# CMB-BNU/PloidyFrost

Measured on AMD Instinct MI355X. Metric: unitigs/s through superbubble+SeqAlign (k=25, z=8), higher is better.
Workload: dtype u64

## Files before the change

### include/ploidyfrost_hip.h

```cpp
#ifndef PLOIDYFROST_HIP_H_
#define PLOIDYFROST_HIP_H_

#include <stddef.h>
#include <stdint.h>

#ifdef __cplusplus
extern "C" {
#endif

#define PF_NONE 0xFFFFFFFFu

enum pf_status {
    PF_OK = 0,
    PF_ERR_ARG = 1,
    PF_ERR_HIP = 2,
    PF_ERR_NO_DEVICE = 3,
    PF_ERR_OVERFLOW = 4,
    PF_ERR_MISSING_KMER = 5
};

typedef struct pf_ctx pf_ctx;

int pf_create(int device, pf_ctx **out);
int pf_warmup(int device);
// ... 271 lines not shown
    uint32_t n_cols;
    uint32_t n_sites;
    uint32_t n_indel_len;
} pf_bubble_result;

int pf_align_bubbles(pf_ctx *, const char *text, uint64_t text_len, const pf_bubble_path *paths, uint64_t n_paths,
                     const pf_bubble_task *tasks, uint32_t n_tasks, double match, double mismatch, double gap,
                     pf_bubble_result *results, char *out_text, uint64_t text_cap, pf_bubble_site *out_sites,
                     uint64_t site_cap, uint8_t *out_groups, uint64_t group_cap, uint32_t *out_ilen, uint64_t ilen_cap,
                     uint64_t used[4]);

int pf_string_cov(pf_ctx *, const char *text, const uint64_t *str_off, uint32_t n_str, uint32_t low, uint32_t up,
                  uint64_t *sum, uint8_t *ok, uint8_t *miss);


int pf_call_set_colours(pf_ctx *, uint32_t n_colors, const uint64_t *full_mask, const uint64_t *size_total, const uint32_t *part_first,
                        const uint32_t *part_colour, const uint64_t *part_word, const uint64_t *part_bits, uint64_t n_part, uint64_t n_words);
int pf_call_set_cutoffs(pf_ctx *, uint32_t n_colors, const uint32_t *lower, const uint32_t *upper);

int pf_call_set_state(pf_ctx *, const uint8_t *flags, const uint32_t *plus, const uint32_t *minus);
int pf_call_set_format(pf_ctx *, int reference_mt);
int pf_superbubble_rows(pf_ctx *, int colored_rule, uint64_t *n_rows, uint64_t *text_len);
int pf_superbubble_fetch(pf_ctx *, char *dst, uint64_t len);
int pf_call_coverage(pf_ctx *);

typedef struct pf_call_side {
    uint32_t u;
    uint32_t exit_ov;
    uint32_t err_unitig;
    uint8_t plus_side;
    uint8_t kind;
    uint8_t aligned;
    uint8_t err;
} pf_call_side;
int pf_call_scan(pf_ctx *, uint32_t lower, uint32_t upper, uint64_t *n_sides);
int pf_call_sides(pf_ctx *, pf_call_side *out, uint64_t cap);
int pf_call_resolve(pf_ctx *, uint64_t *n_bubbles, uint32_t *err, uint32_t *err_unitig);
int pf_call_select(pf_ctx *, const uint32_t *side_index, uint64_t n_bubbles);

#define PF_CALL_STREAMS 10
enum pf_call_stream {
    PF_OUT_ALLELE_FREQUENCY = 0, PF_OUT_ALIGNSEQ = 1, PF_OUT_BIFRE = 2, PF_OUT_TRIFRE = 3, PF_OUT_TETRAFRE = 4, PF_OUT_PENTAFRE = 5,
    PF_OUT_BICOV = 6, PF_OUT_TRICOV = 7, PF_OUT_TETRACOV = 8, PF_OUT_PENTACOV = 9
};
typedef struct pf_call_result {
    uint64_t text_len[PF_CALL_STREAMS];
    uint64_t allele[4];
    uint64_t core_cov, core_num;
    uint64_t n_called;
    uint64_t align_jobs, site_strings, n_branching;
    uint64_t snp_jobs, pair_jobs, wave_jobs;
    uint64_t stack_jobs;
    uint64_t alignseq_packed_len;
    uint64_t numeric_packed;
} pf_call_result;
#define PF_CALL_SLABS 4
#define PF_CALL_LANES 4
int pf_call_run(pf_ctx *, int slab, uint64_t t0, uint64_t t1, uint64_t var_count_base, uint32_t complex_size, double match,
                double mismatch, double gap, pf_call_result *out);
int pf_call_align(pf_ctx *, uint64_t t0, uint64_t t1, uint32_t complex_size, double match, double mismatch, double gap,
                  pf_call_result *out);
int pf_call_text(pf_ctx *, int slab, uint64_t var_count_base, pf_call_result *out);
int pf_call_set_alignseq_packed(pf_ctx *, int on);
#define PF_NUMERIC_PACKED_LEN(text_len) (((((uint64_t)(text_len)) + 1) / 2 + 15) & ~15ull)
int pf_call_set_numeric_packed(pf_ctx *, int on);
int pf_call_fetch_text(pf_ctx *, int slab, int stream, char *dst, uint64_t len);
int pf_call_reserve(pf_ctx *, uint64_t n_bubbles, uint32_t complex_size);
int pf_call_reserve_lanes(pf_ctx *, uint64_t n_bubbles, uint32_t complex_size, int n_lanes);
int pf_call_reserve_text(pf_ctx *, uint64_t piece_bubbles);
typedef struct pf_call_bubble {
    uint32_t entrance_ov, exit_ov;
    uint32_t strict, n_inner;
    uint32_t inner[4];
    double cov[4], core_mean, cov_sum;
} pf_call_bubble;
int pf_call_peek(pf_ctx *, int lane, pf_call_bubble *bubbles, pf_bubble_result *results, uint64_t *sv_off, uint64_t bubble_cap, char *text,
                 pf_bubble_site *sites, uint8_t *groups, uint32_t *ilen, double *sv, const uint64_t cap[5], uint64_t used[6]);
int pf_call_text_range(pf_ctx *, int slab, uint64_t first, uint64_t count, uint64_t var_count_base, pf_call_result *out);
int pf_call_align_lane(pf_ctx *, int lane, uint64_t t0, uint64_t t1, uint32_t complex_size, double match, double mismatch,
                       double gap, pf_call_result *out);
int pf_call_text_range_lane(pf_ctx *, int lane, int slab, uint64_t first, uint64_t count, uint64_t var_count_base,
                            pf_call_result *out);
int pf_call_text_sizes(pf_ctx *, int lane, uint64_t first, uint64_t count, uint64_t var_count_base, pf_call_result *out);
int pf_call_fetch(pf_ctx *, int slab, int stream, char *dst, uint64_t len);
int pf_call_fetch_slab(pf_ctx *, int slab, char *dst, const uint64_t *len);
int pf_call_fetch_range(pf_ctx *, int slab, uint64_t first_byte, char *dst, uint64_t len, int slot);
int pf_call_fetch_wait(pf_ctx *, int slot);
int pf_format_doubles(pf_ctx *, const double *values, uint64_t n, char *text, uint8_t *len);

int pf_side_components(pf_ctx *, int reset, const pf_bfs_record *records, uint64_t n_records, const uint32_t *pool, uint64_t pool_len,
                       const pf_bfs_record *extra, uint64_t n_extra, const uint32_t *extra_pool, uint64_t extra_pool_len);
int pf_replay_order(pf_ctx *, uint32_t n_classes, uint32_t *order, uint32_t *class_off, uint32_t *labels);

int pf_bfs_live_deferred(pf_ctx *, uint64_t cap, volatile uint64_t **list);
int pf_bfs_live_count(pf_ctx *, uint64_t *n);
int pf_bfs_candidates_resident(pf_ctx *, uint32_t u0, uint32_t u1, uint64_t *n_records, uint64_t *pool_used, uint32_t *deferred,
                               uint32_t *deferred_entrance, uint64_t deferred_cap, uint64_t *n_deferred);
int pf_find_reserve(pf_ctx *, uint64_t n_records);
int pf_replay_device(pf_ctx *, uint32_t complex_size, uint32_t small_limit, uint64_t *n_big, uint64_t *big_entries);
int pf_replay_set_colours(pf_ctx *, uint32_t n_colors, const uint64_t *full_mask, const uint64_t *size_total, const uint32_t *n_full_enc);
int pf_replay_big_fetch(pf_ctx *, uint32_t *index, pf_bfs_record *records, uint32_t *pool);
int pf_replay_finish(pf_ctx *, const uint32_t *sides, const uint32_t *links, const uint8_t *side_flags, uint64_t n_patch);
int pf_call_get_state(pf_ctx *, uint8_t *flags, uint32_t *plus, uint32_t *minus);

#define PF_MAX_COLORS_TABLE 1024
#define PF_MAX_COLORS PF_MAX_COLORS_TABLE
int pf_upload_counts_colored(pf_ctx *, uint32_t n_colors, const uint64_t *const *kmers, const uint32_t *const *counts,
                             const uint64_t *n, const uint64_t *min_count, const uint64_t *max_count, const int *both_strands);
uint32_t pf_num_colors(const pf_ctx *);
int pf_unitig_cov_colored(pf_ctx *, uint32_t u0, uint32_t u1, uint64_t *sum, uint32_t *min_count, uint32_t *max_count,
                          uint8_t *miss);
int pf_unitig_cov_colored_probe(pf_ctx *, uint32_t u0, uint32_t u1, uint64_t *sum, uint32_t *min_count, uint32_t *max_count,
                          uint8_t *miss);
int pf_string_cov_colored(pf_ctx *, const char *text, const uint64_t *str_off, uint32_t n_str, const uint32_t *low,
                          const uint32_t *up, uint64_t *sum, uint8_t *ok);

#define PF_COMM_ID_BYTES 128
int pf_comm_unique_id(unsigned char id[PF_COMM_ID_BYTES]);
int pf_comm_init(pf_ctx *, const unsigned char id[PF_COMM_ID_BYTES], int rank, int world);
int pf_gather(pf_ctx *, const uint64_t *mine, uint32_t n, uint64_t *all);
void pf_comm_destroy(pf_ctx *);

#define PF_GMM_MAX_GAUSS 16
int pf_gmm_upload(pf_ctx *, const double *values, uint64_t n);
uint64_t pf_gmm_count(const pf_ctx *);
int pf_gmm_fit(pf_ctx *, uint32_t gauss, double m_thre, double n_thre, int32_t max_iter, double max_delta, double *weights,
               double *means, double *vars, double *loglik, uint32_t *iterations);
int pf_gmm_values(pf_ctx *, double *dst, uint64_t cap);
#define PF_DENSITY_MIN_POINTS 2
#define PF_DENSITY_MAX_POINTS 4096
typedef struct pf_density_info {
    uint64_t n;
    double min, max, sd, q1, q3, bw;
    double order[4];
} pf_density_info;
int pf_gmm_density(pf_ctx *, uint32_t points, double adjust, double *x, double *density, pf_density_info *info);

enum pf_model_source { PF_MODEL_COV = 0, PF_MODEL_FRE = 1 };
int pf_call_model_begin(pf_ctx *, int source, double q);
int pf_call_model_take(pf_ctx *, int slab);
int pf_call_model_finish(pf_ctx *, uint64_t *n_values);
typedef struct pf_filter_opts {
    int simple, indel, snp;
    long long low, up;
    long long num, distance, size;
    double frequency;
} pf_filter_opts;
int pf_call_model_filter(pf_ctx *, const pf_filter_opts *);
int pf_call_model_take_text(pf_ctx *, int stream_ord, const char *host_text, uint64_t len);
typedef struct pf_filter_multi_opts {
    int simple, indel, snp;
    long long low, up;
    long long num, distance, size;
    double frequency;
    long long color;
    double cramer;
} pf_filter_multi_opts;
#define PF_MODEL_NO_ROW 0xFFFFFFFFFFFFFFFFull
int pf_call_model_filter_multi(pf_ctx *, const pf_filter_multi_opts *, int each_color);
uint32_t pf_call_model_color_count(const pf_ctx *);
int pf_call_model_color_select(pf_ctx *, int color, uint64_t *n_values);
uint64_t pf_call_fetched_bytes(const pf_ctx *);

int pf_host_alloc(pf_ctx *, size_t bytes, void **out);
int pf_fetch(pf_ctx *, void *dst_host, const void *src_dev, uint64_t bytes);
void pf_host_free(pf_ctx *, void *p);
// ... 13 lines not shown
```

### ploidyfrost_amd/csrc/host/pf_cdbg_call.cpp

```cpp
#include <fcntl.h>
#include <sys/stat.h>
#include <unistd.h>

#include <algorithm>
#include <atomic>
#include <condition_variable>
#include <cstdio>
#include <cstring>
#include <ctime>
#include <deque>
#include <memory>
#include <mutex>
#include <sstream>
#include <thread>

#include "../pf_alnpack.hpp"
#include "../pf_nibble.hpp"
#include "pf_cdbg_impl.hpp"
#include "pf_parallel.hpp"

namespace pfh {

namespace {
const char *kStreamSuffix[PF_CALL_STREAMS] = {"_allele_frequency.txt", "_alignseq.txt", "_bifre.txt",    "_trifre.txt",   "_tetrafre.txt",
// ... 202 lines not shown
    model_n_ = 0;
    color_fits_.clear();
    color_none_.clear();
    color_empty_.clear();
    color_no_density_.clear();
    density_done_ = false;
    pooled_values_.clear();
    last_each_ = false;
    const uint64_t fetched_before = pf_call_fetched_bytes(ctx_);
    const unsigned T = threads_ ? threads_ : (unsigned)std::max<size_t>(thr, 1);
    times_.cov_device_s = times_.tasks_s = times_.align_s = times_.sites_s = times_.format_s = times_.write_s = 0;
    times_.tasks = times_.align_jobs = times_.site_strings = 0;
    times_.snp_jobs = times_.pair_jobs = times_.wave_jobs = times_.stack_jobs = 0;
    times_.align_build_s = times_.align_device_s = times_.align_post_s = times_.align_choose_s = times_.scan_s = 0;
    allele_[0] = allele_[1] = allele_[2] = allele_[3] = 0;
    core_cov_ = core_num_ = 0;
    const bool trace = getenv("PF_TRACE_PLOIDY") != nullptr;
    auto tp = [&](const char *what) { if (trace) fprintf(stderr, "[ploidy] %-28s %.2f ms\n", what, since(t_all) * 1e3); };

    struct OutFile {
        std::string name;
        uint64_t bytes = 0;
        int rc = 0;
    };
    std::vector<OutFile> files(PF_CALL_STREAMS);
    for (int s = 0; s < PF_CALL_STREAMS; ++s) files[(size_t)s].name = outpre + kStreamSuffix[s];
    MappedOut *maps = out_maps_.get();
    int open_failed = -1;
    std::thread opener;
    if (write_ten)
        opener = std::thread([&] {
            for (size_t i = 0; i < files.size(); ++i)
                if (maps[i].open_for(outdir_ + "/" + files[i].name)) { open_failed = (int)i; return; }
        });
    struct OpenerGuard {
        std::thread &t;
        ~OpenerGuard() { if (t.joinable()) t.join(); }
    } opener_guard{opener};

    uint64_t n_tasks = 0;
    if (call_select(cutoff, n_tasks)) return status_;
    tp("scan + selection done");
    if (opener.joinable()) opener.join();
    if (open_failed >= 0) return fail(PF_ERR_ARG, "CDBG:: Open " + files[(size_t)open_failed].name + " file error");
    last_allfre_.clear();
    last_allfre_file_.clear();
    std::thread prefault0;
    std::atomic<bool> prefault0_stop{false};
    struct Prefault0Guard {
        std::thread &t;
        std::atomic<bool> &stop;
        ~Prefault0Guard() { stop.store(true); if (t.joinable()) t.join(); }
    } prefault0_guard{prefault0, prefault0_stop};
    if (write_ten && n_tasks) {
        const double nbub = 1.1 * (double)n_tasks;
        const double per_bubble[PF_CALL_STREAMS] = {20, 2.0 * (2 * g_.k + 26), 20, 0.5, 0.25, 0, 34, 0.75, 0.25, 0};
        std::vector<std::pair<int, uint64_t>> fresh;
        for (int s = 0; s < PF_CALL_STREAMS; ++s) {
            const uint64_t est = (uint64_t)(per_bubble[s] * nbub);
            if (est >= (1u << 20) && maps[s].reserve(est) == 0) fresh.push_back({s, est});
        }
        if (!fresh.empty())
            prefault0 = std::thread([maps, fresh, T, &prefault0_stop] {
                constexpr uint64_t STEP = 4u << 20;
                std::vector<std::pair<int, uint64_t>> spans;
                uint64_t longest = 0;
                for (auto &f : fresh) longest = std::max(longest, f.second);
                for (uint64_t at = 0; at < longest; at += STEP)
                    for (auto &f : fresh)
                        if (at < f.second) spans.push_back({f.first, at});
                parallel_chunks(spans.size(), 1, std::max(2u, T), [&](size_t i, size_t, size_t) {
                    if (prefault0_stop.load(std::memory_order_relaxed)) return;
                    const int s = spans[i].first;
                    uint64_t end = spans[i].second + STEP;
                    for (auto &f : fresh) if (f.first == s) end = std::min(end, f.second);
                    maps[s].populate(spans[i].second, end);
                });
            });
    }

    const bool aln_packed = !getenv("PF_ALIGNSEQ_ASCII");
    if (pf_call_set_alignseq_packed(ctx_, aln_packed ? 1 : 0) != PF_OK) return fail(PF_ERR_HIP, std::string(tag_) + "::PloidyEstimation(): " + pf_last_error(ctx_));
    const bool num_packed = !getenv("PF_NUMERIC_ASCII");
    if (pf_call_set_numeric_packed(ctx_, num_packed ? 1 : 0) != PF_OK) return fail(PF_ERR_HIP, std::string(tag_) + "::PloidyEstimation(): " + pf_last_error(ctx_));
    if (model_.on && (pf_call_model_begin(ctx_, model_.source, model_.q) != PF_OK || (filter_on_ && pf_call_model_filter(ctx_, &filter_) != PF_OK) ||
                      (multi_on_ && pf_call_model_filter_multi(ctx_, &multi_, multi_each_ ? 1 : 0) != PF_OK)))
        return fail(PF_ERR_ARG, std::string(tag_) + "::PloidyEstimation(): " + pf_last_error(ctx_));
    struct PackGuard {
        pf_ctx *c;
        ~PackGuard() { (void)pf_call_set_alignseq_packed(c, 0); (void)pf_call_set_numeric_packed(c, 0); }
    } pack_guard{ctx_};
    auto slab_len = [](const pf_call_result &r, int s) -> uint64_t {
        const uint64_t aln = (s == PF_OUT_ALIGNSEQ && r.alignseq_packed_len) ? r.alignseq_packed_len : r.text_len[s];
        if (!r.numeric_packed) return aln;
        return s == PF_OUT_ALIGNSEQ ? ((aln + 15) & ~15ull) : PF_NUMERIC_PACKED_LEN(r.text_len[s]);
    };

    const size_t batch_env = [] { const char *e = getenv("PF_BATCH_BUBBLES"); return e ? (size_t)std::max(1, atoi(e)) : (size_t)0; }();
    const size_t batch_now = batch_env ? batch_env : batch_bubbles_;
    const size_t CHUNK = std::min<size_t>(std::max<size_t>(batch_now ? batch_now * 4 : 1, 1), (size_t)1 << 24);
    struct Done {
        pf_call_result res;
        int slab;
        int hslab;
        std::shared_ptr<std::vector<std::vector<char>>> plain;
    };
    std::mutex mu;
    std::condition_variable cv;
    std::deque<Done> ready, towrite;
    size_t fetched = 0;
    size_t written = 0;
    bool fetcher_done = false;
    bool stop = false, producer_done = false;
    int wst = PF_OK;
    std::string werr;
    double write_s = 0;
    auto thread_failed = [&](const char *who, const std::exception &e) {
        {
            std::lock_guard<std::mutex> lk(mu);
            wst = PF_ERR_HIP;
            werr = std::string(who) + ": " + e.what();
            stop = true;
            fetcher_done = true;
        }
        cv.notify_all();
    };
    std::thread fetcher([&] {
        try {
        size_t b = 0;
        for (;;) {
            Done d;
            {
                std::unique_lock<std::mutex> lk(mu);
                cv.wait(lk, [&] { return stop || !ready.empty() || producer_done; });
                if (stop || ready.empty()) { fetcher_done = true; lk.unlock(); cv.notify_all(); return; }
                d = ready.front();
                ready.pop_front();
                cv.wait(lk, [&] { return stop || b < written + 2; });
                if (stop) { fetcher_done = true; lk.unlock(); cv.notify_all(); return; }
            }
            uint64_t total = 0, fetch_len[PF_CALL_STREAMS];
            for (int s = 0; s < PF_CALL_STREAMS; ++s) { fetch_len[s] = slab_len(d.res, s); total += fetch_len[s]; }
            PinnedBuf<char> &hb = cx_.slab[d.hslab];
            hb.ensure(ctx_, std::max<uint64_t>(total, 1) + 16);
            int st = pf_call_fetch_slab(ctx_, d.slab, hb.p, fetch_len);
            if (st == PF_OK && d.res.numeric_packed) {
                uint32_t flagged = 0;
                memcpy(&flagged, hb.p + total, 4);
                if (flagged) {
                    d.plain = std::make_shared<std::vector<std::vector<char>>>((size_t)PF_CALL_STREAMS);
                    for (int s = 0; s < PF_CALL_STREAMS && st == PF_OK; ++s)
                        if (((flagged >> s) & 1) && d.res.text_len[s]) {
                            (*d.plain)[(size_t)s].resize(d.res.text_len[s]);
                            st = pf_call_fetch_text(ctx_, d.slab, s, (*d.plain)[(size_t)s].data(), d.res.text_len[s]);
                        }
                }
            }
            {
                std::lock_guard<std::mutex> lk(mu);
                fetched = b + 1;
                if (st != PF_OK) { wst = st; werr = "copy of a text slab failed"; stop = true; fetcher_done = true; }
                else towrite.push_back(d);
            }
            cv.notify_all();
            if (st != PF_OK) return;
            if (trace) fprintf(stderr, "[ploidy]   batch %zu fetched (%.1f MB) %.2f ms\n", b, total / 1e6, since(t_all) * 1e3);
            ++b;
        }
        } catch (const std::exception &e) { thread_failed("copy of a text slab", e); }
    });
    std::thread writer([&] {
        try {
        size_t b = 0;
        for (;;) {
            Done d;
            {
                std::unique_lock<std::mutex> lk(mu);
                cv.wait(lk, [&] { return stop || !towrite.empty() || fetcher_done; });
                if (stop || towrite.empty()) return;
                d = towrite.front();
                towrite.pop_front();
            }
            const auto tw = clk::now();
            uint64_t total = 0, off[PF_CALL_STREAMS + 1];
            for (int s = 0; s < PF_CALL_STREAMS; ++s) { off[s] = total; total += slab_len(d.res, s); }
            PinnedBuf<char> &hb = cx_.slab[d.hslab];
            if (write_ten) {
                CopySpan spans[PF_CALL_STREAMS];
                bool nib_span[PF_CALL_STREAMS] = {};
                size_t n_spans = 0;
                pf::AlnPackPiece packed;
                char *packed_dst = nullptr;
                std::vector<char> packed_tmp;
                for (int s = 0; s < PF_CALL_STREAMS; ++s) {
                    if (!d.res.text_len[s]) continue;
                    char *dst = maps[s].prepare(files[(size_t)s].bytes, d.res.text_len[s]);
                    if (s == PF_OUT_ALIGNSEQ && d.res.alignseq_packed_len) {
                        if (!packed.parse(reinterpret_cast<const uint8_t *>(hb.p + off[s]), d.res.alignseq_packed_len)) { files[(size_t)s].rc = 1; continue; }
                        if (!dst) { packed_tmp.resize(d.res.text_len[s]); dst = packed_tmp.data(); }
                        packed_dst = dst;
                        continue;
                    }
                    const char *src = hb.p + off[s];
                    bool nib = d.res.numeric_packed != 0 && s != PF_OUT_ALIGNSEQ;
                    if (nib && d.plain && !(*d.plain)[(size_t)s].empty()) { src = (*d.plain)[(size_t)s].data(); nib = false; }
                    if (dst) {
                        nib_span[n_spans] = nib;
                        spans[n_spans++] = CopySpan{dst, src, d.res.text_len[s]};
                    } else if (nib) {
                        std::vector<char> tmp(d.res.text_len[s]);
                        pf::nibble_expand(tmp.data(), reinterpret_cast<const uint8_t *>(src), d.res.text_len[s]);
                        if (maps[s].write(files[(size_t)s].bytes, tmp.data(), tmp.size(), T)) files[(size_t)s].rc = 1;
                    } else if (maps[s].write(files[(size_t)s].bytes, src, d.res.text_len[s], T)) files[(size_t)s].rc = 1;
                }
                constexpr uint64_t PIECE = 1u << 20;
                std::vector<CopySpan> cut;
                std::vector<char> cut_nib;
                constexpr uint64_t NIB_PIECE = 128u << 10;
                for (size_t i = 0; i < n_spans; ++i) {
                    const uint64_t step = nib_span[i] ? NIB_PIECE : PIECE;
                    for (uint64_t at = 0; at < spans[i].len; at += step) {
                        cut.push_back(CopySpan{spans[i].dst + at, spans[i].src + (nib_span[i] ? at / 2 : at), std::min<uint64_t>(step, spans[i].len - at)});
                        cut_nib.push_back(nib_span[i] ? 1 : 0);
                    }
                }
                constexpr uint64_t GROUPS_PER_TASK = 16;
                const size_t n_aln = packed_dst ? (size_t)((packed.n_groups + GROUPS_PER_TASK - 1) / GROUPS_PER_TASK) : 0;
                std::atomic<int> bad{0};
                parallel_chunks(n_aln + cut.size(), 1, T, [&](size_t i, size_t, size_t) {
                    if (i >= n_aln) {
                        const CopySpan &c = cut[i - n_aln];
                        if (cut_nib[i - n_aln]) pf::nibble_expand(c.dst, reinterpret_cast<const uint8_t *>(c.src), c.len);
                        else memcpy(c.dst, c.src, (size_t)c.len);
                        return;
                    }
                    const uint64_t g0 = (uint64_t)i * GROUPS_PER_TASK, g1 = std::min<uint64_t>(packed.n_groups, g0 + GROUPS_PER_TASK);
                    uint64_t t0_, r0_, t1_, r1_;
                    packed.entry(g0, t0_, r0_);
                    packed.entry(g1, t1_, r1_);
                    if (t1_ > d.res.text_len[PF_OUT_ALIGNSEQ] || t0_ > t1_ || r0_ > r1_ ||
                        (uint64_t)(packed.records - packed.base) + r1_ > d.res.alignseq_packed_len) { bad = 1; return; }
                    char *end = pf::alnpack_expand(packed.records + r0_, packed.records + r1_, packed_dst + t0_, packed_dst + t1_);
                    if (end != packed_dst + t1_) bad = 1;
                });
                if (bad) files[PF_OUT_ALIGNSEQ].rc = 1;
                if (!packed_tmp.empty() && maps[PF_OUT_ALIGNSEQ].write(files[PF_OUT_ALIGNSEQ].bytes, packed_tmp.data(), packed_tmp.size(), T)) files[PF_OUT_ALIGNSEQ].rc = 1;
            }
            if (!write_files_) {
                if (d.plain && !(*d.plain)[0].empty()) last_allfre_.append((*d.plain)[0].data(), d.res.text_len[0]);
                else if (d.res.numeric_packed) {
                    const size_t at0 = last_allfre_.size();
                    last_allfre_.resize(at0 + d.res.text_len[0]);
                    pf::nibble_expand(&last_allfre_[at0], reinterpret_cast<const uint8_t *>(hb.p + off[0]), d.res.text_len[0]);
                } else last_allfre_.append(hb.p + off[0], d.res.text_len[0]);
            }
            for (int s = 0; s < PF_CALL_STREAMS; ++s) files[(size_t)s].bytes += d.res.text_len[s];
            write_s += since(tw);
            if (trace) fprintf(stderr, "[ploidy]   batch %zu written %.2f ms\n", b, since(t_all) * 1e3);
            ++b;
            { std::lock_guard<std::mutex> lk(mu); written = b; }
            cv.notify_all();
        }
        } catch (const std::exception &e) { thread_failed("writing the result files", e); }
    });
    struct WriterGuard {
        std::thread &t, &t2;
        std::mutex &mu;
        std::condition_variable &cv;
        bool &stop;
        ~WriterGuard() {
            if (!t.joinable() && !t2.joinable()) return;
            { std::lock_guard<std::mutex> lk(mu); stop = true; }
            cv.notify_all();
            if (t.joinable()) t.join();
            if (t2.joinable()) t2.join();
        }
    } writer_guard{fetcher, writer, mu, cv, stop};

    int rc = PF_OK;
    std::string rc_err;
    std::thread prefault;
    struct PrefaultGuard {
        std::thread &t;
        ~PrefaultGuard() { if (t.joinable()) t.join(); }
    } prefault_guard{prefault};
    const auto t_dev = clk::now();
    uint64_t ALIGN = std::min<uint64_t>((uint64_t)CHUNK * std::max<size_t>(align_pieces_, 1), (uint64_t)1 << 24);
    {
        const int ranges_env = [] { const char *e = getenv("PF_ALIGN_RANGES"); return e ? atoi(e) : 0; }();
        const uint64_t pieces = (n_tasks + CHUNK - 1) / CHUNK;
        const uint64_t n_ranges = ranges_env > 0 ? (uint64_t)ranges_env : (pieces >= 4 ? 2 : 1);
        if (n_ranges > 1) ALIGN = std::min<uint64_t>(ALIGN, std::max<uint64_t>(1, (pieces + n_ranges - 1) / n_ranges) * CHUNK);
    }
    int first_env = 0;
    constexpr int LANES = PF_CALL_LANES;
    const int aligners_wanted = [&] { const char *e = getenv("PF_ALIGN_THREADS"); return e ? std::max(1, std::min(LANES, atoi(e))) : std::min(2, LANES); }();
    {
        const uint64_t pieces = (n_tasks + CHUNK - 1) / CHUNK;
        if (first_env <= 0 && !getenv("PF_ALIGN_RANGES") && pieces >= 4)
            first_env = (int)std::min<uint64_t>(aligners_wanted >= 2 ? (pieces + 1) / 2 : (pieces * 5 + 7) / 8, ((uint64_t)1 << 24) / CHUNK);
    }
    struct Range {
        uint64_t a0 = 0, a1 = 0;
        int lane = 0;
        bool aligned = false;
        uint64_t n_called = 0;
    };
    std::vector<Range> ranges;
    for (uint64_t a0 = 0, a1 = 0; a0 < n_tasks; a0 = a1) {
        a1 = std::min<uint64_t>(n_tasks, a0 + (first_env > 0 && ranges.empty() ? (uint64_t)first_env * CHUNK : ALIGN));
        Range r;
        r.a0 = a0; r.a1 = a1; r.lane = (int)(ranges.size() % (size_t)LANES);
        ranges.push_back(r);
    }
    const int aligners = (int)std::min<size_t>(ranges.size(), (size_t)aligners_wanted);
    size_t next_range = 0;
    size_t ranges_formatted = 0;
    std::thread formatter([&] {
        struct Last {
            std::mutex &mu;
            std::condition_variable &cv;
            bool &producer_done;
            ~Last() {
                { std::lock_guard<std::mutex> lk(mu); producer_done = true; }
                cv.notify_all();
            }
        } last{mu, cv, producer_done};
        try {
        size_t b = 0;
        uint64_t var_base = 0;
        for (size_t ri = 0; ri < ranges.size(); ++ri) {
            Range r;
            {
                std::unique_lock<std::mutex> lk(mu);
                cv.wait(lk, [&] { return stop || ranges[ri].aligned; });
                if (stop) return;
                r = ranges[ri];
            }
            const uint64_t rn = r.a1 - r.a0;
            for (uint64_t p0 = 0; p0 < rn; p0 += CHUNK, ++b) {
                const uint64_t count = std::min<uint64_t>(CHUNK, rn - p0);
                {
                    std::unique_lock<std::mutex> lk(mu);
                    cv.wait(lk, [&] { return stop || model_.only || b < fetched + PF_CALL_SLABS; });
                    if (stop) return;
                }
                Done d;
                d.slab = (int)(b % PF_CALL_SLABS);
                d.hslab = (int)(b & 1);
                int st = pf_call_text_range_lane(ctx_, r.lane, d.slab, p0, count, var_base, &d.res);
                if (st == PF_OK && model_.on) st = pf_call_model_take(ctx_, d.slab);
                if (st != PF_OK) {
                    { std::lock_guard<std::mutex> lk(mu); if (rc == PF_OK) { rc = st; rc_err = pf_last_error(ctx_); } stop = true; }
                    cv.notify_all();
                    return;
                }
                if (trace) fprintf(stderr, "[ploidy]   piece %zu formatted on the device %.2f ms\n", b, since(t_all) * 1e3);
                if (b == 0 && write_ten) {
                    const double scale = 1.05 * (double)n_tasks / (double)std::max<uint64_t>(1, count);
                    std::vector<std::pair<int, uint64_t>> fresh;
                    for (int s = 0; s < PF_CALL_STREAMS; ++s) {
                        const uint64_t est = (uint64_t)((double)d.res.text_len[s] * scale) + 4096;
                        if (d.res.text_len[s] && maps[s].reserve(est) == 0) fresh.push_back({s, est});
                    }
                    if (!fresh.empty())
                        prefault = std::thread([maps, fresh, T] {
                            constexpr uint64_t STEP = 4u << 20;
                            std::vector<std::pair<int, uint64_t>> spans;
                            uint64_t longest = 0;
                            for (auto &f : fresh) longest = std::max(longest, f.second);
                            for (uint64_t at = 0; at < longest; at += STEP)
                                for (auto &f : fresh)
                                    if (at < f.second) spans.push_back({f.first, at});
                            parallel_chunks(spans.size(), 1, std::max(2u, T / 2), [&](size_t i, size_t, size_t) {
                                const int s = spans[i].first;
                                uint64_t end = spans[i].second + STEP;
                                for (auto &f : fresh) if (f.first == s) end = std::min(end, f.second);
                                maps[s].populate(spans[i].second, end);
                            });
                        });
                }
                for (int a = 0; a < 4; ++a) allele_[a] += d.res.allele[a];
                core_cov_ += d.res.core_cov;
                core_num_ += d.res.core_num;
                if (!model_.only) {
                    { std::lock_guard<std::mutex> lk(mu); ready.push_back(d); }
                    cv.notify_all();
                }
            }
            var_base += r.n_called;
            { std::lock_guard<std::mutex> lk(mu); ++ranges_formatted; }
            cv.notify_all();
        }
        } catch (const std::exception &e) { thread_failed("formatting the result rows", e); }
    });
    struct FormatterGuard {
        std::thread &t;
        std::mutex &mu;
        std::condition_variable &cv;
        bool &stop;
        ~FormatterGuard() {
            if (!t.joinable()) return;
            { std::lock_guard<std::mutex> lk(mu); stop = true; }
            cv.notify_all();
            t.join();
        }
    } formatter_guard{formatter, mu, cv, stop};
    auto aligner = [&] {
        try {
        for (;;) {
            size_t ri;
            {
                std::unique_lock<std::mutex> lk(mu);
                if (stop || next_range >= ranges.size()) return;
                ri = next_range++;
                cv.wait(lk, [&] { return stop || ri < ranges_formatted + (size_t)LANES; });
                if (stop) return;
            }
            const Range r = ranges[ri];
            pf_call_result ar;
            const int st = pf_call_align_lane(ctx_, r.lane, r.a0, r.a1, (uint32_t)std::min<size_t>(complex_size_, 1u << 20), sc_.match, sc_.mismatch, sc_.gap, &ar);
            if (st != PF_OK) {
                { std::lock_guard<std::mutex> lk(mu); if (rc == PF_OK) { rc = st; rc_err = pf_last_error(ctx_); } stop = true; }
                cv.notify_all();
                return;
            }
            if (trace) fprintf(stderr, "[ploidy]   range %zu: %llu bubbles aligned on the device %.2f ms\n", ri, (unsigned long long)(r.a1 - r.a0), since(t_all) * 1e3);
            {
                std::lock_guard<std::mutex> lk(mu);
                times_.tasks += r.a1 - r.a0;
                times_.align_jobs += ar.align_jobs;
                times_.snp_jobs += ar.snp_jobs; times_.pair_jobs += ar.pair_jobs; times_.wave_jobs += ar.wave_jobs; times_.stack_jobs += ar.stack_jobs;
                times_.site_strings += ar.site_strings;
                ranges[ri].n_called = ar.n_called;
                ranges[ri].aligned = true;
            }
            cv.notify_all();
        }
        } catch (const std::exception &e) { thread_failed("aligning the bubbles", e); }
    };
    {
        std::vector<std::thread> extra;
        struct ExtraGuard {
            std::vector<std::thread> &v;
            ~ExtraGuard() { for (auto &t : v) if (t.joinable()) t.join(); }
        } extra_guard{extra};
        for (int a = 1; a < aligners; ++a) extra.emplace_back(aligner);
        aligner();
    }
    formatter.join();
    times_.align_s = since(t_dev);
    fetcher.join();
    writer.join();
    if (prefault.joinable()) prefault.join();
    prefault0_stop.store(true);
    if (prefault0.joinable()) prefault0.join();
    tp("pipeline done");
    if (rc != PF_OK) {
        return fail(rc, rc_err.rfind("CDBG::", 0) == 0 ? rc_err : std::string(tag_) + "::PloidyEstimation(): " + rc_err);
    }
    if (wst != PF_OK) return fail(wst, std::string(tag_) + "::PloidyEstimation(): " + werr);
    auto t0 = clk::now();
    if (join_pending_write() || join_pending_ids()) return status_;
    tp("super_bubble.txt joined");
    for (size_t i = 0; i < files.size(); ++i) {
        OutFile &of = files[i];
        out_bytes_ += of.bytes;
// ... 104 lines not shown
```

### ploidyfrost_amd/csrc/pf_alnpack.hpp

```cpp
#pragma once
#include <cstdint>
#include <cstring>

#ifdef __HIPCC__
#define PF_ALNPACK_HD __host__ __device__
#else
#define PF_ALNPACK_HD
#endif

namespace pf {

constexpr uint32_t ALNPACK_GROUP = 256;
constexpr uint32_t ALNPACK_HEADER = 24;

PF_ALNPACK_HD inline uint32_t alnpack_row_bytes(uint32_t n_cols) { return 3u * ((n_cols + 7u) >> 3); }
PF_ALNPACK_HD inline uint64_t alnpack_index_bytes(uint64_t n_bubbles) { return 16 + ((n_bubbles + ALNPACK_GROUP - 1) / ALNPACK_GROUP + 1) * 16; }
PF_ALNPACK_HD inline uint32_t alnpack_code(char c) { return c == '-' ? 0u : c == 'A' ? 1u : c == 'C' ? 2u : c == 'G' ? 3u : 4u; }

#ifndef __HIP_DEVICE_COMPILE__
struct AlnPackTables {
    uint32_t four[4096];
    AlnPackTables() {
        static const char letter[8] = {'-', 'A', 'C', 'G', 'T', '?', '?', '?'};
        for (uint32_t v = 0; v < 4096; ++v)
            four[v] = (uint32_t)(uint8_t)letter[v & 7] | (uint32_t)(uint8_t)letter[(v >> 3) & 7] << 8 | (uint32_t)(uint8_t)letter[(v >> 6) & 7] << 16 |
                      (uint32_t)(uint8_t)letter[(v >> 9) & 7] << 24;
    }
};
inline const AlnPackTables &alnpack_tables() {
    static const AlnPackTables t;
    return t;
}

inline char *alnpack_put_uint(char *p, uint64_t x) {
    char tmp[24];
    int n = 0;
    do { tmp[n++] = (char)('0' + x % 10); x /= 10; } while (x);
    while (n) *p++ = tmp[--n];
    return p;
}

struct AlnPackPiece {
    const uint8_t *base = nullptr;
    uint64_t n_groups = 0, group_bubbles = 0;
    const uint8_t *index = nullptr, *records = nullptr;
    bool parse(const uint8_t *p, uint64_t len) {
        if (len < 32) return false;
        memcpy(&n_groups, p, 8);
        memcpy(&group_bubbles, p + 8, 8);
        if (n_groups > (len - 16) / 16 - 1) return false;
        base = p;
        index = p + 16;
        records = index + (n_groups + 1) * 16;
        return true;
    }
    void entry(uint64_t g, uint64_t &text_off, uint64_t &rec_off) const {
        memcpy(&text_off, index + g * 16, 8);
        memcpy(&rec_off, index + g * 16 + 8, 8);
    }
};

inline char *alnpack_expand(const uint8_t *rec, const uint8_t *rec_end, char *dst, const char *dst_end) {
    const AlnPackTables &T = alnpack_tables();
    char prefix[96];
    while (rec < rec_end) {
        if ((size_t)(rec_end - rec) < ALNPACK_HEADER) return nullptr;
        uint64_t vc;
        uint32_t ent, ext, L, R;
        memcpy(&vc, rec, 8);
        memcpy(&ent, rec + 8, 4);
        memcpy(&ext, rec + 12, 4);
        memcpy(&L, rec + 16, 4);
        memcpy(&R, rec + 20, 4);
        const bool strict = (R >> 31) != 0;
        R &= 0x7FFFFFFFu;
        rec += ALNPACK_HEADER;
        char *q = alnpack_put_uint(prefix, vc);
        *q++ = '\t'; *q++ = strict ? '1' : '0'; *q++ = '\t';
        q = alnpack_put_uint(q, ent);
        *q++ = '\t';
        q = alnpack_put_uint(q, ext);
        *q++ = '\t';
        const size_t np = (size_t)(q - prefix);
        const uint32_t rb = alnpack_row_bytes(L);
        if ((uint64_t)R * rb > (uint64_t)(rec_end - rec) || (uint64_t)R * (np + L + 1) > (uint64_t)(dst_end - dst)) return nullptr;
        for (uint32_t r = 0; r < R; ++r, rec += rb) {
            memcpy(dst, prefix, np);
            dst += np;
            uint32_t x = 0;
            const uint8_t *s = rec;
            for (; x + 8 <= L; x += 8, s += 3) {
                const uint32_t v = (uint32_t)s[0] | (uint32_t)s[1] << 8 | (uint32_t)s[2] << 16;
                const uint32_t a = T.four[v & 4095], b = T.four[v >> 12];
                memcpy(dst + x, &a, 4);
                memcpy(dst + x + 4, &b, 4);
            }
            if (x < L) {
                const uint32_t v = (uint32_t)s[0] | (uint32_t)s[1] << 8 | (uint32_t)s[2] << 16;
                char tail[8];
                const uint32_t a = T.four[v & 4095], b = T.four[v >> 12];
                memcpy(tail, &a, 4);
                memcpy(tail + 4, &b, 4);
                memcpy(dst + x, tail, L - x);
            }
            dst += L;
            *dst++ = '\n';
        }
    }
    return dst;
}
#endif

}
```

### ploidyfrost_amd/csrc/pf_call.hip

```cpp
#include "pf_call_kernels.hpp"
#include "pf_scan.hpp"

using namespace pf;

#define PF_HIP(call)                                                                         \
    do {                                                                                     \
        hipError_t e_ = (call);                                                              \
        if (e_ != hipSuccess) {                                                              \
            pf::CtxErr{ctx} = std::string(#call) + ": " + hipGetErrorString(e_);                   \
            return PF_ERR_HIP;                                                               \
        }                                                                                    \
    } while (0)

#define PF_TRY(call) do { const int s_ = (call); if (s_ != PF_OK) return s_; } while (0)

using namespace pf_call;

struct Need { DevBuf *buf; size_t bytes; };
static int need(pf_ctx *ctx, const char *who, std::initializer_list<Need> list) {
    for (const Need &n : list)
        if (!n.buf->ensure(n.bytes)) { pf::CtxErr{ctx} = std::string(who) + ": out of device memory"; return PF_ERR_HIP; }
    return PF_OK;
}

namespace pf {

void call_state_create(pf_ctx *ctx) { (void)state_of(ctx); }
void call_destroy(pf_ctx *ctx) {
    if (!ctx->call) return;
    ctx->call->release_all();
    delete ctx->call;
    ctx->call = nullptr;
}
void call_invalidate(pf_ctx *ctx) {
    if (!ctx->call) return;
    ctx->call->have_cov = false;
    ctx->call->have_state = false;
    ctx->call->n_sides = ctx->call->n_tasks = 0;
}

}

namespace pf {
int call_state_arrays(pf_ctx *ctx, uint8_t **flags, uint32_t **plus, uint32_t **minus) {
    if (!ctx->d_seq || !ctx->has_adj) { pf::CtxErr{ctx} = "T1 state: graph and adjacency first"; return PF_ERR_ARG; }
    CallState *S = state_of(ctx);
    const size_t N = ctx->N;
    if (!S->flags.ensure(N + 1) || !S->plus.ensure(N * 4) || !S->minus.ensure(N * 4)) { pf::CtxErr{ctx} = "T1 state: out of device memory"; return PF_ERR_HIP; }
    *flags = S->flags.as<uint8_t>();
    *plus = S->plus.as<uint32_t>();
    *minus = S->minus.as<uint32_t>();
    S->have_state = false;
    return PF_OK;
}
void call_state_resident(pf_ctx *ctx) {
    CallState *S = state_of(ctx);
    S->have_state = true;
    S->n_sides = S->n_tasks = 0;
}
}

extern "C" {

int pf_format_doubles(pf_ctx *ctx, const double *values, uint64_t n, char *text, uint8_t *len) {
    if (!ctx || (n && (!values || !text || !len))) return PF_ERR_ARG;
    if (n == 0) return PF_OK;
    PF_HIP(hipSetDevice(ctx->device));
    DevTmp<double> dx;
    DevTmp<char> dt;
    DevTmp<uint8_t> dl;
    PF_HIP(dx.alloc(n * 8));
    PF_HIP(dt.alloc(n * 32));
    PF_HIP(dl.alloc(n));
    PF_HIP(hipMemcpyAsync(dx.p, values, n * 8, hipMemcpyDefault, ctx->stream));
    k_format_doubles<<<(unsigned)((n + 255) / 256), 256, 0, ctx->stream>>>(dx.p, n, dt.p, dl.p);
    PF_HIP(hipGetLastError());
    PF_HIP(hipMemcpyAsync(text, dt.p, n * 32, hipMemcpyDefault, ctx->stream));
    PF_HIP(hipMemcpyAsync(len, dl.p, n, hipMemcpyDefault, ctx->stream));
    PF_HIP(hipStreamSynchronize(ctx->stream));
    return PF_OK;
}

// ... 632 lines not shown
        PF_HIP(scan_inclusive_u32(W.has.as<uint32_t>(), O.vc.as<uint32_t>(), nb, W.scan_tmp.p, st));
        PF_HIP(hipMemcpyAsync(&n_called, O.vc.as<uint32_t>() + (nb - 1), 4, hipMemcpyDeviceToHost, st));
        return PF_OK;
    }

    SiteArgs site_args(uint32_t ks, uint64_t rows_cap, uint64_t per_wave, uint64_t sv_cap) const {
        SiteArgs sa;
        sa.batch = batch; sa.blist = lists.blist; sa.res = pools.res; sa.otext = pools.otext; sa.osites = pools.osites; sa.ogroups = pools.ogroups;
        sa.k = ctx->k; sa.tab = ctx->d_tab; sa.mask = ctx->tab_cap - 1; sa.one_strand = ctx->tab_one_strand; sa.tab_exact = ctx->tab_exact;
        sa.low = S->low; sa.up = S->up; sa.ks = ks; sa.rows_cap = (uint32_t)rows_cap;
        sa.scratch = W.sites_scr.as<uint8_t>(); sa.scratch_per_wave = per_wave; sa.sv_off = O.sv_off.as<uint64_t>();
        sa.sv = O.sv.as<double>(); sa.sv_cap = sv_cap; sa.cnt = d_cnt; sa.prof = nullptr;
        sa.n_colors = S->n_colors;
        sa.ctab = CTab{ctx->d_ctab, ctx->ctab_cap - 1, ctx->ctab_line_bytes}; sa.c_one_strand = ctx->ctab_one_strand; sa.unread = ctx->d_unread;
        sa.clow = S->col_low.as<uint32_t>(); sa.cup = S->col_up.as<uint32_t>(); sa.full = S->col_full.as<uint64_t>(); sa.cwords = S->col_words;
        sa.part_first = S->part_first.as<uint32_t>(); sa.part_colour = S->part_colour.as<uint32_t>(); sa.part_word = S->part_word.as<uint64_t>();
        sa.part_bits = S->part_bits.as<uint64_t>(); sa.walk_pool = W.walk_pool.as<uint32_t>(); sa.walk_off = W.walk_off.as<uint64_t>();
        sa.graph = graph;
        return sa;
    }

    int launch_sites(SiteArgs &sa, int grid) {
        static const bool sites_stats = getenv("PF_SITES_STATS") != nullptr;
        DevTmp<unsigned long long> prof;
        if (sites_stats) PF_TRY(stats_begin(ctx, prof, (size_t)grid * 6, st, &sa.prof));
        PF_HIP(hipMemsetAsync(&d_cnt->sites_next, 0, 4, st));
        PF_HIP(hipMemsetAsync(&d_cnt->sv_head, 0, 8, st));
        PF_HIP(hipMemsetAsync(&d_cnt->site_strings, 0, 8, st));
        tbegin(PF_K_CALL_SITES, st);
        if (sa.n_colors) k_call_sites<true><<<grid, 64, 0, st>>>(sa);
        else k_call_sites<false><<<grid, 64, 0, st>>>(sa);
        tend(st);
        ctx_units(ctx, PF_K_CALL_SITES, hc.n_branching);
        if (sites_stats) { PF_HIP(hipGetLastError()); PF_TRY(print_sites_stats(ctx, prof, grid, st)); }
        return read_counters();
    }

    int run_sites() {
        uint32_t KS = std::max<uint32_t>(first_site_string(ctx->k), S->sites_ks.load());
        const uint32_t C = S->n_colors;
        const uint64_t rows_cap = sites_rows_cap(hc.max_rows);
        for (int sv_attempt = 0, ks_attempt = 0;;) {
            const uint64_t per_wave = sites_per_wave(rows_cap, KS, C, S->col_words);
            const int grid = call_sites_grid(hc.n_branching, grids, per_wave);
            const uint64_t sv_cap = site_values_cap(C, hc.n_branching, grid, S->sv_pool);
            PF_TRY(need(ctx, who, {{&W.sites_scr, per_wave * grid}, {&O.sv, sv_cap * 8}}));
            SiteArgs sa = site_args(KS, rows_cap, per_wave, sv_cap);
            PF_TRY(launch_sites(sa, grid));
            if (hc.err & ERR_SITE_LONG) {
                if (++ks_attempt > 3 || hc.ks_need <= KS) { pf::CtxErr{ctx} = "pf_call_run: the room for a site string does not converge"; return PF_ERR_OVERFLOW; }
                KS = grown_site_string(hc.ks_need);
                amax(S->sites_ks, KS);
                hc.err = 0; hc.ks_need = 0;
                PF_HIP(hipMemsetAsync(&d_cnt->err, 0, 4, st));
                PF_HIP(hipMemsetAsync(&d_cnt->ks_need, 0, 4, st));
                continue;
            }
            if (hc.err & ERR_MISSING_KMER) { pf::CtxErr{ctx} = "CDBG::readCov(): a kmer of a site string can not found ."; return PF_ERR_MISSING_KMER; }
            if (hc.err & ERR_SITE_ROW) { pf::CtxErr{ctx} = "CDBG::PloidyEstimation(): a site string runs past the end of an aligned row (the reference terminates here: std::out_of_range from substr, src/CDBG.cpp:1478-1590)"; return PF_ERR_ARG; }
            if (hc.err & ERR_SITE_UNITIG) { pf::CtxErr{ctx} = "CCDBG::PloidyEstimation(): a site string does not start on a unitig of its bubble"; return PF_ERR_ARG; }
            if (hc.sv_head > sv_cap) {
                if (sv_attempt++ >= 2) { pf::CtxErr{ctx} = "pf_call_run: site value pool does not converge"; return PF_ERR_OVERFLOW; }
                amax(S->sv_pool, grown(hc.sv_head, 1024));
                continue;
            }
            amax(S->sv_pool, sv_cap);
            return PF_OK;
        }
    }
};

}

extern "C" {

int pf_call_align_lane(pf_ctx *ctx, int lane, uint64_t t0, uint64_t t1, uint32_t complex_size, double match, double mismatch, double gap,
                       pf_call_result *out) {
    if (!ctx || !out || lane < 0 || lane >= PF_CALL_LANES) return PF_ERR_ARG;
    CallState *S = ctx->call;
    if (!S || t0 > t1 || t1 > S->n_tasks) { pf::CtxErr{ctx} = "pf_call_align: range outside the selection"; return PF_ERR_ARG; }
    memset(out, 0, sizeof(*out));
    CallState::AlignOut &O = S->lane[lane];
    O.nb = 0;
    O.t0 = t0;
    O.cur = pf_call_result{};
    if (t1 == t0) return PF_OK;
    if (t1 - t0 > (1u << 24)) { pf::CtxErr{ctx} = "pf_call_align: at most 2^24 bubbles per batch"; return PF_ERR_ARG; }
    PF_HIP(hipSetDevice(ctx->device));
    AlignCall A(ctx, lane, t0, (uint32_t)(t1 - t0), complex_size, match, mismatch, gap);
    PF_TRY(A.prepare());
    for (A.attempt = 0;; ++A.attempt) {
        if (A.attempt > 5) { pf::CtxErr{ctx} = "pf_call_align: pools do not converge"; return PF_ERR_OVERFLOW; }
        bool retry = false;
        PF_TRY(A.size_pools());
        PF_TRY(A.launch_tiers());
        PF_TRY(A.read_counters());
        A.trace.stage("K-PREP .. K-STACK done");
        PF_TRY(A.launch_pair_tier2());
        A.note_units();
        PF_TRY(A.launch_paths_big(&retry));
        if (!retry) PF_TRY(A.accept_walks(&retry));
        if (!retry) PF_TRY(A.run_bubble(&retry));
        if (!retry) break;
    }
    const CallCounters &hc = A.hc;
    out->n_branching = hc.n_branching;
    out->align_jobs = A.n_jobs + hc.n_snp_done + hc.n_pair_done + hc.n_pair2_done + hc.n_stack_done;
    out->snp_jobs = hc.n_snp_done; out->pair_jobs = hc.n_pair_done + hc.n_pair2_done; out->wave_jobs = A.n_jobs; out->stack_jobs = hc.n_stack_done;
    PF_TRY(A.number_called());
    if (hc.n_branching) {
        PF_TRY(A.run_sites());
    } else {
        PF_TRY(need(ctx, A.who, {{&O.sv, 16}}));
        PF_HIP(hipStreamSynchronize(A.st));
    }
    out->site_strings = hc.site_strings;
    A.trace.stage("K-SITES done");
    out->n_called = A.n_called;
    O.nb = A.nb;
    O.cur = *out;
    for (int x = 0; x < 4; ++x) O.used[x] = A.heads[x];
    O.used[4] = hc.n_branching ? hc.sv_head : 0;
    return PF_OK;
}

int pf_call_peek(pf_ctx *ctx, int lane, pf_call_bubble *bubbles, pf_bubble_result *results, uint64_t *sv_off, uint64_t bubble_cap, char *text,
                 pf_bubble_site *sites, uint8_t *groups, uint32_t *ilen, double *sv, const uint64_t cap[5], uint64_t used[6]) {
    if (!ctx || lane < 0 || lane >= PF_CALL_LANES || !used) return PF_ERR_ARG;
    CallState *S = ctx->call;
    if (!S) { pf::CtxErr{ctx} = "pf_call_peek: pf_call_align first"; return PF_ERR_ARG; }
    if (S->n_colors) { pf::CtxErr{ctx} = "pf_call_peek: the single-sample path's view (a colored site holds one value per colour and group)"; return PF_ERR_ARG; }
    const CallState::AlignOut &O = S->lane[lane];
    used[0] = O.nb;
    for (int x = 0; x < 5; ++x) used[x + 1] = O.used[x];
    if (!O.nb) return PF_OK;
    if (!bubbles && !results && !text && !sites && !groups && !ilen && !sv && !sv_off) return PF_OK;
    if (bubble_cap < O.nb || !cap) return PF_ERR_ARG;
    for (int x = 0; x < 5; ++x)
        if (cap[x] < O.used[x]) return PF_ERR_ARG;
    PF_HIP(hipSetDevice(ctx->device));
    if (bubbles) {
        std::vector<uint32_t> kept(O.nb);
        PF_HIP(hipMemcpy(kept.data(), S->kept.as<uint32_t>() + O.t0, (size_t)O.nb * 4, hipMemcpyDeviceToHost));
        std::vector<CallTask> ct(S->n_sides);
        if (S->n_sides) PF_HIP(hipMemcpy(ct.data(), S->ctask.p, (size_t)S->n_sides * sizeof(CallTask), hipMemcpyDeviceToHost));
        for (uint32_t j = 0; j < O.nb; ++j) {
            const CallTask &t = ct[kept[j]];
            pf_call_bubble &b = bubbles[j];
            b.entrance_ov = t.entrance_ov; b.exit_ov = t.exit_ov; b.strict = t.strict; b.n_inner = t.n_inner;
            for (int x = 0; x < 4; ++x) { b.inner[x] = t.inner[x]; b.cov[x] = t.cov[x]; }
            b.core_mean = t.core_mean; b.cov_sum = t.cov_sum;
        }
    }
    if (results) PF_HIP(hipMemcpy(results, O.res.p, (size_t)O.nb * sizeof(pf_bubble_result), hipMemcpyDeviceToHost));
    if (sv_off) PF_HIP(hipMemcpy(sv_off, O.sv_off.p, (size_t)O.nb * 8, hipMemcpyDeviceToHost));
    if (text && O.used[0]) PF_HIP(hipMemcpy(text, O.otext.p, O.used[0], hipMemcpyDeviceToHost));
    if (sites && O.used[1]) PF_HIP(hipMemcpy(sites, O.osites.p, O.used[1] * sizeof(pf_bubble_site), hipMemcpyDeviceToHost));
    if (groups && O.used[2]) PF_HIP(hipMemcpy(groups, O.ogroups.p, O.used[2], hipMemcpyDeviceToHost));
    if (ilen && O.used[3]) PF_HIP(hipMemcpy(ilen, O.oilen.p, O.used[3] * 4, hipMemcpyDeviceToHost));
    if (sv && O.used[4]) PF_HIP(hipMemcpy(sv, O.sv.p, O.used[4] * 8, hipMemcpyDeviceToHost));
    return PF_OK;
}

int pf_call_reserve_lanes(pf_ctx *ctx, uint64_t nb64, uint32_t complex_size, int n_lanes) {
    if (!ctx || nb64 == 0 || n_lanes < 1 || n_lanes > PF_CALL_LANES) return PF_ERR_ARG;
    CallState *S = state_of(ctx);
    PF_HIP(hipSetDevice(ctx->device));
    const uint32_t nb = (uint32_t)std::min<uint64_t>(nb64, 1u << 24);
    const char *who = "pf_call_reserve";
    const CallGrids grids = call_grids(ctx->n_cu);
    DevLoadTrace trace;
    for (int lane = 0; lane < n_lanes; ++lane) {
        CallState::AlignWork &W = S->work[lane];
        CallState::AlignOut &O = S->lane[lane];
        PF_TRY(ensure_batch_buffers(ctx, who, W, O, nb));
        PF_TRY(ensure_wave_scratch(ctx, who, W, grids, depth_cap(complex_size), true, true));
        PF_TRY(ensure_pools(ctx, who, W, O, nb, batch_pools(nb, grids, LearntPools{}, false)));
        PF_TRY(need(ctx, who, {{&W.scan_tmp2, reserve_job_index_bytes(nb)}, {&W.sites_scr, sites_per_wave(256, first_site_string(31), 0, 1) * grids.sites},
                               {&O.sv, reserve_site_values(nb, grids) * 8}}));
        trace.mark("reserve: a lane's buffers");
        PF_TRY(ensure_lane_streams(ctx, W, lane));
        trace.mark("reserve: a lane's streams and events");
        PF_TRY(bubble_reserve(ctx, nb, lane));
        trace.mark("reserve: K-BUBBLE's workspaces and first launches");
    }
    return PF_OK;
}

int pf_call_reserve(pf_ctx *ctx, uint64_t nb64, uint32_t complex_size) { return pf_call_reserve_lanes(ctx, nb64, complex_size, 2); }

int pf_call_align(pf_ctx *ctx, uint64_t t0, uint64_t t1, uint32_t complex_size, double match, double mismatch, double gap,
                  pf_call_result *out) {
    return pf_call_align_lane(ctx, 0, t0, t1, complex_size, match, mismatch, gap, out);
}

static int text_work_of(pf_ctx *ctx, pf::CallState *S, int which, uint32_t nb) {
    pf::CallState::TextWork &T = S->text[which];
    if (!T.stream) {
        int least = 0, greatest = 0;
        PF_HIP(hipDeviceGetStreamPriorityRange(&least, &greatest));
        PF_HIP(hipStreamCreateWithPriority(&T.stream, hipStreamNonBlocking, greatest));
    }
    return need(ctx, "pf_call_text", {{&T.sizes, (size_t)N_INT * (nb + 1) * 4}, {&T.offs, ((size_t)N_INT * (nb + 1) + 1) * 8}, {&T.totals, 16 * 8},
                                      {&T.tcounters, sizeof(CallCounters)}, {&T.tscan, scan_scratch_bytes((uint64_t)N_INT * (nb + 1))}});
}

int pf_call_reserve_text(pf_ctx *ctx, uint64_t piece_bubbles) {
    if (!ctx || piece_bubbles == 0) return PF_ERR_ARG;
    pf::CallState *S = state_of(ctx);
    PF_HIP(hipSetDevice(ctx->device));
    const uint32_t nb = (uint32_t)std::min<uint64_t>(piece_bubbles, 1u << 24);
    for (int which = 0; which < 2; ++which) { const int ts = text_work_of(ctx, S, which, nb); if (ts != PF_OK) return ts; }
    for (int slab = 0; slab < PF_CALL_SLABS; ++slab) PF_TRY(need(ctx, "pf_call_text", {{&S->out[slab], (11ull * 31 + 40) * nb}}));
    for (int which = 0; which < 2; ++which) {
        pf::CallState::TextWork &T = S->text[which];
        FmtArgs fa;
        memset(&fa, 0, sizeof(fa));
        fa.sizes = T.sizes.as<uint32_t>(); fa.offs = T.offs.as<uint64_t>(); fa.cnt = T.tcounters.as<CallCounters>();
        if (S->n_colors) { k_call_format<false, true><<<1, FMT_BLOCK, 0, T.stream>>>(fa); k_call_format<true, true><<<1, FMT_BLOCK, 0, T.stream>>>(fa); }
        else { k_call_format<false, false><<<1, FMT_BLOCK, 0, T.stream>>>(fa); k_call_format<true, false><<<1, FMT_BLOCK, 0, T.stream>>>(fa); }
        PF_HIP(hipGetLastError());
        PF_HIP(hipStreamSynchronize(T.stream));
    }
    return PF_OK;
}

static int call_text_impl(pf_ctx *ctx, int lane, int slab, uint64_t first, uint64_t count, uint64_t var_count_base, pf_call_result *out, bool sizes_only) {
    if (!ctx || !out || slab < 0 || slab >= PF_CALL_SLABS || lane < 0 || lane >= PF_CALL_LANES) return PF_ERR_ARG;
    CallState *S = ctx->call;
    if (!S) return PF_ERR_ARG;
    CallState::AlignOut &O = S->lane[lane];
    if (first + count > O.nb) { pf::CtxErr{ctx} = "pf_call_text_range: range outside the aligned batch"; return PF_ERR_ARG; }
    if (S->n_colors && S->mt_format) { pf::CtxErr{ctx} = "pf_call_text_range: the -t > 1 format is the single-sample path's"; return PF_ERR_ARG; }
    if (!sizes_only)
        for (int s = 0; s < N_STREAMS; ++s) S->out_len[slab][s] = 0;
    *out = O.cur;
    out->n_called = 0;
    if (count == 0) return PF_OK;
    PF_HIP(hipSetDevice(ctx->device));
    const bool trace_stages = getenv("PF_TRACE_ALIGN") != nullptr;
    const auto t_enter = std::chrono::steady_clock::now();
    auto ta = [&](const char *what) {
        if (trace_stages) fprintf(stderr, "[pf_call_text]    %-34s %.2f ms\n", what, std::chrono::duration<double>(std::chrono::steady_clock::now() - t_enter).count() * 1e3);
    };
    const uint32_t nb = (uint32_t)count;
    const int which = sizes_only ? 0 : (slab & 1);
    { const int ts = text_work_of(ctx, S, which, nb); if (ts != PF_OK) return ts; }
    CallState::TextWork &T = S->text[which];
    hipStream_t st = T.stream;
    const uint64_t t0 = O.t0;
    uint32_t vc_edge[2] = {0, 0};
    PF_HIP(hipMemcpyAsync(&vc_edge[1], O.vc.as<uint32_t>() + (first + count - 1), 4, hipMemcpyDeviceToHost, st));
    if (first) PF_HIP(hipMemcpyAsync(&vc_edge[0], O.vc.as<uint32_t>() + (first - 1), 4, hipMemcpyDeviceToHost, st));
    CallCounters *d_cnt = T.tcounters.as<CallCounters>();
    CallCounters hc;
    const size_t n_sizes = (size_t)N_INT * (nb + 1);
    ta("stream and size tables");
    PF_HIP(hipMemsetAsync(&d_cnt->allele[0], 0, 6 * 8, st));
    FmtArgs fa;
    fa.ct = S->ctask.as<CallTask>(); fa.kept = S->kept.as<uint32_t>(); fa.t0 = t0; fa.j0 = (uint32_t)first; fa.nb = nb;
    fa.res = O.res.as<pf_bubble_result>();
    fa.otext = O.otext.as<char>(); fa.osites = O.osites.as<pf_bubble_site>(); fa.ogroups = O.ogroups.as<uint8_t>();
    fa.oilen = O.oilen.as<uint32_t>(); fa.sv_off = O.sv_off.as<uint64_t>(); fa.sv = O.sv.as<double>(); fa.vc = O.vc.as<uint32_t>();
    fa.vc_base = var_count_base; fa.mt = S->mt_format ? 1 : 0; fa.len = ctx->d_len; fa.sizes = T.sizes.as<uint32_t>(); fa.offs = T.offs.as<uint64_t>(); fa.cnt = d_cnt;
    for (int s = 0; s < N_INT; ++s) fa.out[s] = nullptr;
    fa.packed = S->pack_alignseq ? 1 : 0;
    size_t at = 0;
    ctx_begin_at(ctx, PF_K_CALL_FORMAT, st, &at);
    fa.n_colors = S->n_colors; fa.N = ctx->N; fa.k = ctx->k; fa.full = S->col_full.as<uint64_t>(); fa.cwords = S->col_words; fa.ccov_sum = S->ccov_sum.as<uint64_t>();
    if (S->n_colors) k_call_format<false, true><<<(nb + 1 + FMT_BLOCK - 1) / FMT_BLOCK, FMT_BLOCK, 0, st>>>(fa);
    else k_call_format<false, false><<<(nb + 1 + FMT_BLOCK - 1) / FMT_BLOCK, FMT_BLOCK, 0, st>>>(fa);
    ctx_end_at(ctx, at, st);
    PF_HIP(scan_exclusive_u32_u64(T.sizes.as<uint32_t>(), T.offs.as<uint64_t>(), n_sizes, T.tscan.p, st));
    k_call_totals<<<1, 64, 0, st>>>(T.offs.as<uint64_t>(), T.sizes.as<uint32_t>(), nb, T.totals.as<uint64_t>());
    uint64_t totals[N_INT + 1] = {};
    PF_HIP(hipMemcpyAsync(totals, T.totals.p, N_INT * 8, hipMemcpyDeviceToHost, st));
    PF_HIP(hipMemcpyAsync(&hc, d_cnt, sizeof(hc), hipMemcpyDeviceToHost, st));
    PF_HIP(hipStreamSynchronize(st));
    out->n_called = vc_edge[1] - vc_edge[0];
    const uint64_t packed_len = (fa.packed && totals[PF_OUT_ALIGNSEQ]) ? alnpack_index_bytes(nb) + totals[S_PACK] : 0;
    auto slab_len = [&](int s) { return (s == PF_OUT_ALIGNSEQ && fa.packed) ? packed_len : totals[s]; };
    out->alignseq_packed_len = packed_len;
    uint64_t all = 0;
    for (int s = 0; s < N_STREAMS; ++s) all += slab_len(s);
    if (sizes_only) {
        for (int s = 0; s < N_STREAMS; ++s) out->text_len[s] = totals[s];
        for (int x = 0; x < 4; ++x) out->allele[x] = hc.allele[x];
        out->core_cov = hc.core_cov;
        out->core_num = hc.core_num;
        return PF_OK;
    }
    ta("sizes counted");
    PF_TRY(need(ctx, "pf_call_text", {{&S->out[slab], std::max<uint64_t>(all, 16)}}));
    ta("slab taken");
    all = 0;
    for (int s = 0; s < N_STREAMS; ++s) {
        fa.out[s] = S->out[slab].as<char>() + all;
        S->out_off[slab][s] = all;
        S->out_len[slab][s] = slab_len(s);
        out->text_len[s] = totals[s];
        all += slab_len(s);
    }
    if (fa.packed) { fa.out[S_PACK] = fa.out[PF_OUT_ALIGNSEQ]; fa.out[PF_OUT_ALIGNSEQ] = nullptr; }
    if (S->model.read_ev[slab]) PF_HIP(hipStreamWaitEvent(st, S->model.read_ev[slab], 0));
    ctx_begin_at(ctx, PF_K_CALL_FORMAT, st, &at);
    if (S->n_colors) k_call_format<true, true><<<(nb + FMT_BLOCK - 1) / FMT_BLOCK, FMT_BLOCK, 0, st>>>(fa);
    else k_call_format<true, false><<<(nb + FMT_BLOCK - 1) / FMT_BLOCK, FMT_BLOCK, 0, st>>>(fa);
    ctx_end_at(ctx, at, st);
    ctx_units(ctx, PF_K_CALL_FORMAT, nb);
    PF_HIP(hipGetLastError());
    S->fetch_base[slab] = S->out[slab].as<char>();
    S->nib[slab] = false;
    out->numeric_packed = 0;
    for (int s = 0; s < N_STREAMS; ++s) { S->txt_off[slab][s] = S->out_off[slab][s]; S->txt_len[slab][s] = S->out_len[slab][s]; }
    if (S->pack_numeric) {
        uint64_t foff[N_STREAMS], flen[N_STREAMS], fall = 0;
        for (int s = 0; s < N_STREAMS; ++s) {
            flen[s] = s == PF_OUT_ALIGNSEQ ? ((slab_len(s) + 15) & ~15ull) : PF_NUMERIC_PACKED_LEN(totals[s]);
            foff[s] = fall;
            fall += flen[s];
        }
        PF_TRY(need(ctx, "pf_call_text", {{&S->outp[slab], fall + 16}}));
        char *pb = S->outp[slab].as<char>();
        PF_HIP(hipMemsetAsync(pb + fall, 0, 16, st));
        if (slab_len(PF_OUT_ALIGNSEQ))
            PF_HIP(hipMemcpyAsync(pb + foff[PF_OUT_ALIGNSEQ], S->out[slab].as<char>() + S->txt_off[slab][PF_OUT_ALIGNSEQ], (size_t)slab_len(PF_OUT_ALIGNSEQ), hipMemcpyDeviceToDevice, st));
        NibArgs na;
        int x = 0;
        uint64_t units = 0;
        for (int s = 0; s < N_STREAMS; ++s) {
            if (s == PF_OUT_ALIGNSEQ) continue;
            na.src[x] = S->out[slab].as<char>() + S->txt_off[slab][s];
            na.dst[x] = reinterpret_cast<uint8_t *>(pb + foff[s]);
            na.len[x] = totals[s];
            na.unit0[x] = units;
            na.stream[x] = (uint32_t)s;
            units += (totals[s] + 15) / 16;
            ++x;
        }
        na.unit0[NIB_STREAMS] = units;
        na.flag = reinterpret_cast<uint32_t *>(pb + fall);
        if (units) k_text_nibbles<<<(unsigned)((units + 255) / 256), 256, 0, st>>>(na);
        PF_HIP(hipGetLastError());
        for (int s = 0; s < N_STREAMS; ++s) { S->out_off[slab][s] = foff[s]; S->out_len[slab][s] = flen[s]; }
        S->fetch_base[slab] = pb;
        S->nib[slab] = true;
        out->numeric_packed = 1;
    }
    if (!S->text_ev[slab]) PF_HIP(hipEventCreateWithFlags(&S->text_ev[slab], hipEventDisableTiming));
    PF_HIP(hipEventRecord(S->text_ev[slab], st));
    if (!O.read_ev[which]) PF_HIP(hipEventCreateWithFlags(&O.read_ev[which], hipEventDisableTiming));
    PF_HIP(hipEventRecord(O.read_ev[which], st));
    for (int x = 0; x < 4; ++x) out->allele[x] = hc.allele[x];
    out->core_cov = hc.core_cov;
    out->core_num = hc.core_num;
    return PF_OK;
}

int pf_call_set_numeric_packed(pf_ctx *ctx, int on) {
    if (!ctx) return PF_ERR_ARG;
    CallState *S = state_of(ctx);
    if (!S) return PF_ERR_HIP;
    S->pack_numeric = on != 0;
    return PF_OK;
}

int pf_call_fetch_text(pf_ctx *ctx, int slab, int stream, char *dst, uint64_t len) {
    if (!ctx || !ctx->call || slab < 0 || slab >= PF_CALL_SLABS || stream < 0 || stream >= N_STREAMS) return PF_ERR_ARG;
    CallState *S = ctx->call;
    if (len > S->txt_len[slab][stream] || (len && !dst)) return PF_ERR_ARG;
    if (len == 0) return PF_OK;
    if (hipSetDevice(ctx->device) != hipSuccess || !S->copy_stream) return PF_ERR_HIP;
    if (S->text_ev[slab] && hipStreamWaitEvent(S->copy_stream, S->text_ev[slab], 0) != hipSuccess) return PF_ERR_HIP;
    if (hipMemcpyAsync(dst, S->out[slab].as<char>() + S->txt_off[slab][stream], (size_t)len, hipMemcpyDeviceToHost, S->copy_stream) != hipSuccess) return PF_ERR_HIP;
    if (hipStreamSynchronize(S->copy_stream) != hipSuccess) return PF_ERR_HIP;
    S->fetched_bytes.fetch_add(len, std::memory_order_relaxed);
    return PF_OK;
}

int pf_call_set_alignseq_packed(pf_ctx *ctx, int on) {
    if (!ctx) return PF_ERR_ARG;
    CallState *S = state_of(ctx);
    if (!S) return PF_ERR_HIP;
    S->pack_alignseq = on != 0;
    return PF_OK;
}

int pf_call_text_range_lane(pf_ctx *ctx, int lane, int slab, uint64_t first, uint64_t count, uint64_t var_count_base, pf_call_result *out) {
    return call_text_impl(ctx, lane, slab, first, count, var_count_base, out, false);
}

int pf_call_text_sizes(pf_ctx *ctx, int lane, uint64_t first, uint64_t count, uint64_t var_count_base, pf_call_result *out) {
    return call_text_impl(ctx, lane, 0, first, count, var_count_base, out, true);
}

int pf_call_text_range(pf_ctx *ctx, int slab, uint64_t first, uint64_t count, uint64_t var_count_base, pf_call_result *out) {
    return pf_call_text_range_lane(ctx, 0, slab, first, count, var_count_base, out);
}

int pf_call_text(pf_ctx *ctx, int slab, uint64_t var_count_base, pf_call_result *out) {
    if (!ctx || !ctx->call) return PF_ERR_ARG;
    const int st = pf_call_text_range(ctx, slab, 0, ctx->call->lane[0].nb, var_count_base, out);
    if (st == PF_OK) out->n_called = ctx->call->lane[0].cur.n_called;
    return st;
}

int pf_call_run(pf_ctx *ctx, int slab, uint64_t t0, uint64_t t1, uint64_t var_count_base, uint32_t complex_size, double match,
                double mismatch, double gap, pf_call_result *out) {
    const int st = pf_call_align(ctx, t0, t1, complex_size, match, mismatch, gap, out);
    if (st != PF_OK) return st;
    return pf_call_text(ctx, slab, var_count_base, out);
}

int pf_call_fetch(pf_ctx *ctx, int slab, int stream, char *dst, uint64_t len) {
    if (!ctx || !ctx->call || slab < 0 || slab >= PF_CALL_SLABS || stream < 0 || stream >= N_STREAMS) return PF_ERR_ARG;
    CallState *S = ctx->call;
    if (len > S->out_len[slab][stream] || (len && !dst)) return PF_ERR_ARG;
    if (len == 0) return PF_OK;
    if (hipSetDevice(ctx->device) != hipSuccess) return PF_ERR_HIP;
    if (!S->copy_stream) return PF_ERR_HIP;
    if (S->text_ev[slab] && hipStreamWaitEvent(S->copy_stream, S->text_ev[slab], 0) != hipSuccess) return PF_ERR_HIP;
    if (hipMemcpyAsync(dst, S->fetch_base[slab] + S->out_off[slab][stream], (size_t)len, hipMemcpyDeviceToHost, S->copy_stream) != hipSuccess) return PF_ERR_HIP;
    if (hipStreamSynchronize(S->copy_stream) != hipSuccess) return PF_ERR_HIP;
    S->fetched_bytes.fetch_add(len, std::memory_order_relaxed);
    return PF_OK;
}

int pf_call_fetch_slab(pf_ctx *ctx, int slab, char *dst, const uint64_t *len) {
    if (!ctx || !ctx->call || slab < 0 || slab >= PF_CALL_SLABS || !len) return PF_ERR_ARG;
    CallState *S = ctx->call;
    if (hipSetDevice(ctx->device) != hipSuccess) return PF_ERR_HIP;
    if (!S->copy_stream) return PF_ERR_HIP;
    if (S->text_ev[slab] && hipStreamWaitEvent(S->copy_stream, S->text_ev[slab], 0) != hipSuccess) return PF_ERR_HIP;
    uint64_t at = 0;
    bool whole = true;
    for (int s = 0; s < N_STREAMS; ++s) {
        if (len[s] > S->out_len[slab][s] || (len[s] && !dst)) return PF_ERR_ARG;
        whole = whole && len[s] == S->out_len[slab][s];
        at += len[s];
    }
    size_t tl_at = (size_t)-1;
    (void)ctx_begin_at(ctx, PF_K_COPY_TEXT, S->copy_stream, &tl_at);
    if (whole) {
        const uint64_t tail = S->nib[slab] ? 16 : 0;
        if (at + tail && hipMemcpyAsync(dst, S->fetch_base[slab], (size_t)(at + tail), hipMemcpyDeviceToHost, S->copy_stream) != hipSuccess) return PF_ERR_HIP;
    } else {
        at = 0;
        for (int s = 0; s < N_STREAMS; ++s) {
            if (len[s] && hipMemcpyAsync(dst + at, S->fetch_base[slab] + S->out_off[slab][s], (size_t)len[s], hipMemcpyDeviceToHost, S->copy_stream) != hipSuccess)
                return PF_ERR_HIP;
            at += len[s];
        }
    }
    ctx_end_at(ctx, tl_at, S->copy_stream);
    if (hipStreamSynchronize(S->copy_stream) != hipSuccess) return PF_ERR_HIP;
    S->fetched_bytes.fetch_add(at, std::memory_order_relaxed);
    return PF_OK;
// ... 28 lines not shown
```

### ploidyfrost_amd/csrc/pf_call_kernels.hpp

```cpp
#pragma once

#include <hip/hip_runtime.h>

#include <algorithm>
#include <atomic>
#include <chrono>
#include <cmath>
#include <cstddef>
#include <cstdio>
#include <cstdlib>
#include <cstring>
#include <string>
#include <vector>

#include "pf_bubble_launch.hpp"
#include "pf_alnpack.hpp"
#include "pf_call_dev.hpp"
#include "pf_call_plan.hpp"
#include "pf_colored_dev.hpp"
#include "pf_cov_stream.hpp"
#include "pf_ctx.hpp"
#include "pf_device_common.hpp"
#include "pf_filter_rows.hpp"
#include "pf_format_dev.hpp"
// ... 20 lines not shown
    bool ensure(size_t bytes) {
        if (bytes <= cap && p) return true;
        if (p) (void)hipFree(p);
        p = nullptr;
        cap = 0;
        const size_t want = bytes + bytes / 4 + 256;
        if (hipMalloc(&p, want) != hipSuccess) { (void)hipGetLastError(); p = nullptr; return false; }
        cap = want;
        return true;
    }
    void release() {
        if (p) (void)hipFree(p);
        p = nullptr;
        cap = 0;
    }
};

template <typename T, typename V>
inline void amax(std::atomic<T> &a, V v) {
    T cur = a.load(std::memory_order_relaxed);
    while (cur < (T)v && !a.compare_exchange_weak(cur, (T)v, std::memory_order_relaxed)) {}
}

enum CallErr : unsigned int {
    ERR_MANY_PATHS = 1u,
    ERR_MISSING_KMER = 2u,
    ERR_SITE_ROW = 4u,
    ERR_PATH_POOL = 8u,
    ERR_SITE_LONG = 16u,
    ERR_TOO_DEEP = 32u,
    ERR_SITE_UNITIG = 64u,
    ERR_WALK = ERR_MANY_PATHS | ERR_TOO_DEEP,
};

struct CallCounters {
    unsigned int q_n[NQ];
    unsigned int n_branching;
    unsigned int n_snp, n_snp_done;
    unsigned int n_pair, n_pair_done;
    unsigned int n_pair2, n_pair2_done;
    unsigned int n_stack, n_stack_b, n_stack_done;
    unsigned int paths_next, sites_next;
    unsigned int n_many, max_rows;
    unsigned int ks_need;
    unsigned int err;
    unsigned int err_entrance, err_exit;
    unsigned long long path_head, text_head, sv_head, walk_head;
    unsigned long long max_need, retry_need;
    unsigned long long allele[4], core_cov, core_num, n_called, site_strings;
};

static_assert(offsetof(CallCounters, core_cov) == offsetof(CallCounters, allele) + 32 && offsetof(CallCounters, core_num) == offsetof(CallCounters, allele) + 40, "allele[4], core_cov, core_num are contiguous");

}

namespace pf {
using namespace pf_call;

struct CallState {
    DevBuf flags, plus, minus;
    bool have_state = false;
    DevBuf cov_sum, cov_min, cov_miss;
    bool have_cov = false, per_strand = false;
    uint32_t n_colors = 0, col_words = 1;
    DevBuf col_low, col_up, col_full, col_size, part_first, part_colour, part_word, part_bits;
    DevBuf ccov_sum, ccov_min, ccov_max, ccov_miss;
    std::atomic<uint32_t> sites_ks{0};
    bool pack_alignseq = false;
    bool pack_numeric = false;
    DevBuf side_cnt, side_base, sides, ctask, scan_tmp, target, pending, killed, rstate, rflag, rsmall;
    uint64_t n_sides = 0;
    uint32_t low = 0, up = 0;
    DevBuf kept;
    DevBuf sb_cnt, sb_base, sb_sizes, sb_offs, sb_out;
    uint64_t sb_len = 0;
    uint64_t n_tasks = 0;
    struct AlignOut {
        DevBuf res, otext, osites, ogroups, oilen, sv_off, sv, vc;
        uint64_t t0 = 0;
        uint32_t nb = 0;
        pf_call_result cur = {};
        uint64_t used[5] = {};
        hipEvent_t read_ev[2] = {nullptr, nullptr};
    } lane[PF_CALL_LANES];
    struct AlignWork {
        DevBuf counters, btask, bpath, ptext, queues, blist, slist, plist, plist2, klist, klist_b, stack_scr, pair_scr, pair_scr2, has, scan_tmp, scan_tmp2, paths_scr, sites_scr;
        DevBuf mlist, paths_big_scr;
        uint32_t mlist_cap = 0;
        DevBuf walk_off, walk_pool;
        uint64_t walk_cap = 0;
        hipStream_t stream = nullptr;
        bool own_stream = false;
        hipStream_t side_stream = nullptr;
        hipEvent_t ev_prep = nullptr, ev_paths = nullptr;
    } work[PF_CALL_LANES];
    struct TextWork {
        DevBuf sizes, offs, totals, tcounters, tscan;
        hipStream_t stream = nullptr;
    } text[2];
    std::atomic<uint64_t> path_pool{0}, text_pool{0}, sv_pool{0};
    std::atomic<uint64_t> otext_cap{0}, osites_cap{0}, ogroups_cap{0}, oilen_cap{0};
    DevBuf out[PF_CALL_SLABS];
    uint64_t out_len[PF_CALL_SLABS][N_STREAMS] = {}, out_off[PF_CALL_SLABS][N_STREAMS] = {};
    DevBuf outp[PF_CALL_SLABS];
    const char *fetch_base[PF_CALL_SLABS] = {};
    bool nib[PF_CALL_SLABS] = {};
    uint64_t txt_len[PF_CALL_SLABS][N_STREAMS] = {}, txt_off[PF_CALL_SLABS][N_STREAMS] = {};
    hipStream_t copy_stream = nullptr;
    hipEvent_t fetch_ev[2] = {nullptr, nullptr};
    hipEvent_t text_ev[PF_CALL_SLABS] = {};
    bool mt_format = false;
    std::atomic<uint64_t> fetched_bytes{0};
    struct ModelWork {
        bool active = false;
        int source = 0;
        double q = 0;
        hipStream_t stream = nullptr;
        DevBuf state, flags, ends, nvals, voff, n_rows, scan;
        DevBuf vals[14];
        uint64_t bound[14] = {};
        bool filter = false, taken = false;
        pf::FilterRule rule = {};
        DevBuf cflag, coff, upload, tokens;
        bool each = false, each_done = false;
        DevBuf keys[14], tkeys, ctok;
        uint64_t pooled_n = 0;
        uint32_t color_count = 0;
        uint8_t color_kept[1024] = {};
        hipEvent_t read_ev[PF_CALL_SLABS] = {};
    } model;
    void release_all() {
        for (DevBuf *b : {&model.state, &model.flags, &model.ends, &model.nvals, &model.voff, &model.n_rows, &model.scan, &model.cflag, &model.coff, &model.upload, &model.tokens, &model.tkeys, &model.ctok}) b->release();
        for (DevBuf &b : model.vals) b.release();
        for (DevBuf &b : model.keys) b.release();
        model.each_done = false;
        if (model.stream) { (void)hipStreamDestroy(model.stream); model.stream = nullptr; }
        for (hipEvent_t &e : model.read_ev)
            if (e) { (void)hipEventDestroy(e); e = nullptr; }
        model.active = false;
        DevBuf *all[] = {&col_low, &col_up, &col_full, &col_size, &part_first, &part_colour, &part_word, &part_bits, &ccov_sum, &ccov_min, &ccov_max, &ccov_miss,
                         &flags, &plus, &minus, &cov_sum, &cov_min, &cov_miss, &side_cnt, &side_base, &sides, &ctask, &scan_tmp, &target, &pending, &killed, &rstate, &rflag, &rsmall, &kept, &sb_cnt, &sb_base, &sb_sizes, &sb_offs, &sb_out,
                         };
        for (DevBuf *b : all) b->release();
        for (TextWork &t : text) {
            for (DevBuf *b : {&t.sizes, &t.offs, &t.totals, &t.tcounters, &t.tscan}) b->release();
            if (t.stream) { (void)hipStreamDestroy(t.stream); t.stream = nullptr; }
        }
        for (AlignOut &o : lane) {
            for (DevBuf *b : {&o.res, &o.otext, &o.osites, &o.ogroups, &o.oilen, &o.sv_off, &o.sv, &o.vc}) b->release();
            for (hipEvent_t &e : o.read_ev) if (e) { (void)hipEventDestroy(e); e = nullptr; }
        }
        for (AlignWork &w : work) {
            for (DevBuf *b : {&w.counters, &w.btask, &w.bpath, &w.ptext, &w.queues, &w.blist, &w.slist, &w.plist, &w.plist2, &w.klist, &w.klist_b, &w.stack_scr,
                              &w.pair_scr, &w.pair_scr2, &w.has, &w.scan_tmp, &w.scan_tmp2, &w.paths_scr, &w.sites_scr, &w.mlist, &w.paths_big_scr, &w.walk_off, &w.walk_pool})
                b->release();
            if (w.own_stream && w.stream) (void)hipStreamDestroy(w.stream);
            w.stream = nullptr; w.own_stream = false;
            if (w.side_stream) { (void)hipStreamDestroy(w.side_stream); w.side_stream = nullptr; }
            if (w.ev_prep) { (void)hipEventDestroy(w.ev_prep); w.ev_prep = nullptr; }
            if (w.ev_paths) { (void)hipEventDestroy(w.ev_paths); w.ev_paths = nullptr; }
        }
        for (DevBuf &b : out) b.release();
        for (DevBuf &b : outp) b.release();
        if (copy_stream) { (void)hipStreamDestroy(copy_stream); copy_stream = nullptr; }
        for (hipEvent_t &e : fetch_ev)
            if (e) { (void)hipEventDestroy(e); e = nullptr; }
        for (hipEvent_t &e : text_ev)
            if (e) { (void)hipEventDestroy(e); e = nullptr; }
    }
};
}

namespace pf_call {

__device__ inline bool colour_in(const uint64_t *__restrict__ full, uint32_t words, uint32_t u, uint32_t c) {
    return (full[(size_t)u * words + (c >> 6)] >> (c & 63)) & 1;
}

inline CallState *state_of(pf_ctx *ctx) {
    if (!ctx->call) {
        ctx->call = new CallState();
        if (hipStreamCreateWithFlags(&ctx->call->copy_stream, hipStreamNonBlocking) != hipSuccess) { (void)hipGetLastError(); ctx->call->copy_stream = nullptr; }
    }
    return ctx->call;
}

struct ScanArgs {
    const uint8_t *flags;
    const uint32_t *plus, *minus, *succ, *pred;
    const uint64_t *seq, *off;
    const uint32_t *len;
    uint32_t N;
    int k;
    const uint64_t *cov_sum;
    const uint32_t *cov_min;
    const uint8_t *cov_miss;
    int per_strand;
    uint32_t low, up;
    const uint32_t *side_base;
    pf_call_side *sides;
    CallTask *tasks;
    uint32_t *target;
    uint32_t n_colors;
    const uint64_t *ccov_sum;
    const uint32_t *ccov_min, *ccov_max;
    const uint8_t *ccov_miss;
    const uint32_t *clow, *cup;
    const uint64_t *full, *size_total;
    uint32_t cwords;
};

struct ResolveArgs {
    const pf_call_side *sides;
    const uint32_t *target;
    uint32_t n;
    int *pending;
    uint8_t *killed;
    uint8_t *state;
    uint32_t *flag;
    unsigned int *undecided;
    unsigned int *first_err;
};

struct CallLists {
    uint32_t *queues;
    uint32_t *blist, *slist, *plist, *plist2, *klist, *klist_b;
    uint32_t nb;
};
__device__ inline void wave_append(int key, uint32_t val, const CallLists &L, CallCounters *cnt) {
    unsigned long long todo = __ballot(key != KEY_NONE);
    while (todo) {
        const int x = __shfl(key, __ffsll((long long)todo) - 1, WAVE);
        const unsigned long long m = __ballot(key == x);
// ... 132 lines not shown
    const uint32_t *blist;
    const uint32_t *succ;
    GraphSeq graph;
    int k;
    uint32_t depth_cap;
    uint8_t *scratch;
    uint64_t scratch_per_wave;
    int force_scratch;
    uint32_t max_paths;
    const unsigned int *n_list;
    uint32_t *mlist;
    uint32_t mlist_cap;
    uint32_t *walk_pool;
    uint64_t *walk_off;
    uint64_t walk_cap;
    pf_bubble_task *btask;
    pf_bubble_path *bpath;
    uint64_t path_cap;
    char *text;
    uint64_t text_cap;
    uint32_t *queues;
    uint32_t *klist;
    int stack_ok;
    CallCounters *cnt;
};

constexpr uint32_t MAX_PATHS = 255;
constexpr uint32_t PATHS_BIG = 65535;

struct SiteArgs {
    BatchRef batch;
    const uint32_t *blist;
    const pf_bubble_result *res;
    const char *otext;
    pf_bubble_site *osites;
    const uint8_t *ogroups;
    int k;
    const CountLine *tab;
    uint64_t mask;
    int one_strand, tab_exact;
    uint32_t low, up;
    uint32_t ks;
    uint32_t rows_cap;
    uint8_t *scratch;
    uint64_t scratch_per_wave;
    uint64_t *sv_off;
    double *sv;
    uint64_t sv_cap;
    CallCounters *cnt;
    unsigned long long *prof;
    uint32_t n_colors;
    CTab ctab;
    int c_one_strand;
    const uint8_t *unread;
    const uint32_t *clow, *cup;
    const uint64_t *full;
    uint32_t cwords;
    const uint32_t *part_first, *part_colour;
    const uint64_t *part_word, *part_bits;
    const uint32_t *walk_pool;
    const uint64_t *walk_off;
    GraphSeq graph;
};

struct FmtArgs {
    const CallTask *ct;
    const uint32_t *kept;
    uint64_t t0;
    uint32_t j0;
    uint32_t nb;
    const pf_bubble_result *res;
    const char *otext;
    const pf_bubble_site *osites;
    const uint8_t *ogroups;
    const uint32_t *oilen;
    const uint64_t *sv_off;
    const double *sv;
    const uint32_t *vc;
    uint64_t vc_base;
    int mt;
    const uint32_t *len;
    uint32_t *sizes;
    const uint64_t *offs;
    char *out[N_INT];
    int packed;
    CallCounters *cnt;
    uint32_t n_colors, N, cwords;
    int k;
    const uint64_t *full, *ccov_sum;
};

constexpr uint32_t FMT_BLOCK = 64;

constexpr int NIB_STREAMS = N_STREAMS - 1;
struct NibArgs {
    const char *src[NIB_STREAMS];
    uint8_t *dst[NIB_STREAMS];
    uint64_t len[NIB_STREAMS];
    uint64_t unit0[NIB_STREAMS + 1];
    uint32_t stream[NIB_STREAMS];
    uint32_t *flag;
};

struct SbArgs {
    const uint8_t *flags;
    const uint32_t *plus, *minus;
    uint32_t N;
    int colored;
    uint32_t first_id;
    const uint32_t *row_base;
    uint32_t *sizes;
    const uint64_t *offs;
    char *out;
};

__global__ void k_call_count_sides(const uint8_t *, uint32_t, uint32_t *);
template <bool COLORED> __global__ void k_call_sides(ScanArgs);
__global__ void k_call_pending(ResolveArgs);
__global__ void k_call_resolve(ResolveArgs);
__global__ void k_call_prep(PrepArgs);
__global__ void k_call_snp(SnpArgs);
__global__ void k_call_pair2_reroute(PairArgs);
template <int NMAX, bool INTEGRAL> __global__ void k_call_pair(PairArgs);
__global__ void k_call_stack(StackArgs);
template <bool BIG> __global__ void k_call_paths(PathArgs);
template <bool COLORED> __global__ void k_call_sites(SiteArgs);
__global__ void k_call_has(const pf_bubble_result *, uint32_t, uint32_t *);
template <bool W, bool COLORED> __global__ void k_call_format(FmtArgs);
__global__ void k_call_totals(const uint64_t *, const uint32_t *, uint32_t, uint64_t *);
__global__ void k_sb_count(SbArgs, uint32_t *);
template <bool W> __global__ void k_sb_format(SbArgs);
__global__ void k_format_doubles(const double *, uint64_t, char *, uint8_t *);
__global__ void k_text_nibbles(NibArgs);

}
```

### ploidyfrost_amd/csrc/pf_call_plan.hpp

```cpp
#pragma once

#include <algorithm>
#include <cstdint>

namespace pf_call {

constexpr uint32_t FIRST_ROW_TEXT = 384, FIRST_SITES = 4, FIRST_GROUPS = 12, FIRST_ILEN = 2, FIRST_PATH_TEXT = 64;

constexpr int paths_per_cu = 16, sites_per_cu = 16, pair_per_cu = 12, pair2_per_cu = 4, stack_per_cu = 8;

struct CallGrids {
    int paths, sites, pair, pair2, stack;
};
inline CallGrids call_grids(int n_cu) { return {n_cu * paths_per_cu, n_cu * sites_per_cu, n_cu * pair_per_cu, n_cu * pair2_per_cu, n_cu * stack_per_cu}; }

inline uint64_t round_up(uint64_t x, uint64_t to) { return (x + to - 1) & ~(to - 1); }
inline uint64_t grown(uint64_t need, uint64_t slack) { return need + need / 8 + slack; }

inline uint32_t depth_cap(uint32_t complex_size) { return std::max<uint32_t>(complex_size + 4, 16); }
inline uint64_t paths_stack_bytes(uint32_t depth) { return (10ull * depth + 4) * 4; }
inline uint64_t paths_per_wave(uint32_t depth) { return round_up(256 * 8 + 256 * 4 + paths_stack_bytes(depth), 256); }
inline uint64_t paths_big_per_wave(uint32_t depth, uint32_t max_paths) { return round_up(round_up(paths_stack_bytes(depth), 8) + ((uint64_t)max_paths + 1) * 12, 256); }
inline int paths_big_grid(uint32_t n_many) { return (int)std::min<uint32_t>(n_many, 32); }
constexpr uint32_t MANY_LIST_MIN = 4096;
inline uint32_t grown_many(uint32_t n_many) { return n_many + n_many / 8 + 64; }

inline int call_pair2_grid(uint32_t n_pair2, const CallGrids &g) { return (int)std::min<uint32_t>((n_pair2 + 63) / 64, (uint32_t)g.pair2); }
inline uint32_t pair2_min(int n_cu) { return (uint32_t)n_cu * 32u; }

inline uint32_t first_site_string(int k) { return (uint32_t)(2 * k + 64); }
inline uint32_t grown_site_string(uint32_t ks_need) { return (ks_need + 63u) & ~63u; }
inline uint64_t sites_rows_cap(uint32_t max_rows) { return std::max<uint64_t>(256, round_up(max_rows, 64)); }
inline uint64_t sites_per_wave(uint64_t rows_cap, uint64_t ks, uint32_t n_colors, uint32_t col_words) {
    return round_up(2 * rows_cap * ks + rows_cap * (4 + 4 + 4 + 1 + 1 + 8) + (n_colors ? rows_cap * (16ull * col_words + 8ull * n_colors + 1) : 0), 256);
}
inline int call_sites_grid(uint32_t n_branching, const CallGrids &g, uint64_t per_wave) {
    return (int)std::max<uint64_t>(1, std::min<uint64_t>(std::min<uint32_t>(n_branching, (uint32_t)g.sites), (2ull << 30) / per_wave));
}
inline uint64_t site_values_cap(uint32_t n_colors, uint32_t n_branching, int sites_grid, uint64_t learnt) {
    return std::max<uint64_t>(learnt, 8ull * std::max<uint32_t>(n_colors, 1) * n_branching + 1024ull * sites_grid + 1024);
}

struct LearntPools {
    uint64_t path_pool = 0, path_text = 0, row_text = 0, sites = 0, groups = 0, ilen = 0, walk = 0;
};
struct BatchPools {
    uint64_t path_pool;
    uint64_t path_text;
    uint64_t row_text, sites, groups, ilen;
    uint64_t walk;
    uint64_t path_entries(uint32_t nb) const { return 4ull * nb + path_pool; }
};
inline BatchPools batch_pools(uint32_t nb, const CallGrids &g, const LearntPools &l, bool colored) {
    BatchPools p;
    p.path_pool = std::max<uint64_t>(l.path_pool, (uint64_t)nb / 2 + 128ull * g.paths + 1024);
    p.path_text = std::max<uint64_t>(l.path_text, (uint64_t)nb * FIRST_PATH_TEXT + (1u << 16));
    p.row_text = std::max<uint64_t>(l.row_text, (uint64_t)FIRST_ROW_TEXT * nb + (1u << 16));
    p.sites = std::max<uint64_t>(l.sites, (uint64_t)FIRST_SITES * nb + 64);
    p.groups = std::max<uint64_t>(l.groups, (uint64_t)FIRST_GROUPS * nb + 64);
    p.ilen = std::max<uint64_t>(l.ilen, (uint64_t)FIRST_ILEN * nb + 64);
    p.walk = colored ? std::max<uint64_t>(l.walk, (uint64_t)nb * 2 + 256ull * g.paths + 1024) : 0;
    return p;
}
inline uint64_t row_text_need(uint64_t path_text_used, uint32_t n_branching, uint32_t nb) { return 3 * path_text_used + 128ull * n_branching + 160ull * nb; }

inline uint64_t reserve_job_index_bytes(uint32_t nb) { return (uint64_t)nb / 4 * 4 + 4096; }
inline uint64_t reserve_site_values(uint32_t nb, const CallGrids &g) { return (uint64_t)nb / 4 + 1024ull * g.sites + 1024; }

}
```

### ploidyfrost_amd/csrc/pf_call_text.hip

```cpp
#include "pf_call_kernels.hpp"

namespace pf_call {

__device__ __forceinline__ uint32_t open_run_len(const uint32_t *ilen, uint32_t i, uint32_t n_ilen, uint32_t n_cols, uint32_t col) {
    return i < n_ilen ? ilen[i] : n_cols - col;
}


template <class Val>
__device__ inline double cramer_v_dev(const Val &val, uint32_t ca, uint32_t cb, uint32_t n_alleles) {
#pragma clang fp contract(off)
    double n = 0, nA = 0, nB = 0, chi = 0;
    uint32_t count = 0;
    for (uint32_t i = 0; i < n_alleles; ++i) {
        const double A = val(ca, i), B = val(cb, i), p = A + B;
        nA += A;
        nB += B;
        n = n + p;
        if (p != 0) ++count;
    }
    if ((count & 255u) < 2) return 0;
    for (uint32_t i = 0; i < n_alleles; ++i) {
        const double A = val(ca, i), B = val(cb, i), p = A + B;
        if (p == 0) continue;
        const double exA = nA * p / n, exB = nB * p / n;
        const double dA = A - exA, dB = B - exB;
        chi += dA * dA / exA;
        chi += dB * dB / exB;
    }
    return sqrt(chi / n);
}
template <class Val>
__device__ inline double max_cramer_v_dev(const Val &val, uint32_t n_colors, uint32_t n_alleles) {
    double c = 0;
    for (uint32_t ci = 0; ci + 1 < n_colors; ++ci)
        for (uint32_t cj = ci + 1; cj < n_colors; ++cj) {
            const double v = cramer_v_dev(val, ci, cj, n_alleles);
            c = c < v ? v : c;
        }
    return c;
}

template <bool W>
struct Row {
    char *p;
    uint32_t n;
    __device__ inline void put(char c) { if (W) *p++ = c; else ++n; }
};

template <bool W>
struct Tee {
    Row<W> &a, &b;
    __device__ inline void put(char c) { a.put(c); b.put(c); }
};

__global__ void k_call_has(const pf_bubble_result *__restrict__ res, uint32_t nb, uint32_t *__restrict__ has) {
    const uint32_t j = blockIdx.x * blockDim.x + threadIdx.x;
    if (j < nb) has[j] = (res[j].n_rows != 0 && res[j].n_rows != 0xFFFFFFFFu) ? 1u : 0u;
}

constexpr uint32_t FMT_STAGE[4] = {8192, 1536, 1536, 2048};
constexpr int FMT_STAGED_STREAM[4] = {1, 0, 2, 6};

template <bool W, bool COLORED>
__global__ __launch_bounds__(FMT_BLOCK, W ? 3 : 4) void k_call_format(FmtArgs a) {
    const uint32_t jj = blockIdx.x * blockDim.x + threadIdx.x;
    const uint32_t j = a.j0 + jj;
    unsigned long long allele[4] = {0, 0, 0, 0}, core_cov = 0, core_num = 0;
    __shared__ __attribute__((aligned(16))) char s_stage[W ? (FMT_BLOCK / 64) * (FMT_STAGE[0] + FMT_STAGE[1] + FMT_STAGE[2] + FMT_STAGE[3]) : 4];
    bool staged[4] = {false, false, false, false};
    uint64_t span0[4] = {0, 0, 0, 0};
    uint32_t span_len[4] = {0, 0, 0, 0};
    char *stage[4] = {nullptr, nullptr, nullptr, nullptr};
    char *cp_dst = nullptr;
    const char *cp_src = nullptr;
    uint32_t cp_L = 0, cp_R = 0, cp_step = 0;
    if (W) {
        const size_t stride = (size_t)a.nb + 1;
        const uint32_t w_first = jj & ~63u;
        if (w_first < a.nb) {
            const uint32_t w_end = w_first + 64 < a.nb ? w_first + 64 : a.nb;
            char *base = s_stage + (threadIdx.x >> 6) * (FMT_STAGE[0] + FMT_STAGE[1] + FMT_STAGE[2] + FMT_STAGE[3]);
            uint32_t acc = 0;
#pragma unroll
            for (int q = 0; q < 4; ++q) {
                const int st_ = (q == 0 && a.packed) ? S_PACK : FMT_STAGED_STREAM[q];
                span0[q] = a.offs[st_ * stride + w_first];
                span_len[q] = (uint32_t)(a.offs[st_ * stride + w_end] - span0[q]);
                staged[q] = span_len[q] <= FMT_STAGE[q];
                stage[q] = base + acc;
                acc += FMT_STAGE[q];
            }
        }
    }
    if (jj < a.nb) {
        const size_t stride = (size_t)a.nb + 1;
        Row<W> s_all{nullptr, 0}, s_aln{nullptr, 0}, s_fre[4], s_cov[4];
        for (int x = 0; x < 4; ++x) { s_fre[x] = Row<W>{nullptr, 0}; s_cov[x] = Row<W>{nullptr, 0}; }
        if (W) {
            s_all.p = a.out[0] + (a.offs[0 * stride + jj] - a.offs[0 * stride]);
            if (!a.packed) s_aln.p = a.out[1] + (a.offs[1 * stride + jj] - a.offs[1 * stride]);
#pragma unroll
            for (int x = 0; x < 4; ++x) {
                s_fre[x].p = a.out[2 + x] + (a.offs[(2 + x) * stride + jj] - a.offs[(2 + x) * stride]);
                s_cov[x].p = a.out[6 + x] + (a.offs[(6 + x) * stride + jj] - a.offs[(6 + x) * stride]);
            }
            if (staged[0] && !a.packed) s_aln.p = stage[0] + (a.offs[1 * stride + jj] - span0[0]);
            if (staged[1]) s_all.p = stage[1] + (a.offs[0 * stride + jj] - span0[1]);
            if (staged[2]) s_fre[0].p = stage[2] + (a.offs[2 * stride + jj] - span0[2]);
            if (staged[3]) s_cov[0].p = stage[3] + (a.offs[6 * stride + jj] - span0[3]);
        }
        const pf_bubble_result r = a.res[j];
        if (r.n_rows != 0 && r.n_rows != 0xFFFFFFFFu) {
            const CallTask &t = a.ct[a.kept[a.t0 + j]];
            const uint32_t R = r.n_rows, L = r.n_cols;
            const char *rows = a.otext + r.rows_off;
            const uint64_t my_vc = a.vc_base + a.vc[j] - (a.mt ? 1 : 0);
            char *fre_start[4] = {s_fre[0].p, s_fre[1].p, s_fre[2].p, s_fre[3].p};
            const uint32_t fre_n0[4] = {s_fre[0].n, s_fre[1].n, s_fre[2].n, s_fre[3].n};
            if (W && a.packed) {
                char *rec = staged[0] ? stage[0] + (a.offs[(size_t)S_PACK * stride + jj] - span0[0])
                                      : a.out[S_PACK] + alnpack_index_bytes(a.nb) + (a.offs[(size_t)S_PACK * stride + jj] - a.offs[(size_t)S_PACK * stride]);
                const uint64_t vc64 = my_vc;
                const uint32_t h[4] = {t.u + 1, (t.exit_ov >> 1) + 1, L, R | (t.strict ? 0x80000000u : 0u)};
                __builtin_memcpy(rec, &vc64, 8);
                __builtin_memcpy(rec + 8, h, 16);
                cp_dst = rec + ALNPACK_HEADER; cp_src = rows; cp_L = L; cp_R = R;
            }
            for (uint32_t p = 0; p < R && !(W && a.packed); ++p) {
                char *const row_start = s_aln.p;
                put_uint(s_aln, my_vc);
                s_aln.put('\t'); s_aln.put(t.strict ? '1' : '0'); s_aln.put('\t');
                put_uint(s_aln, (uint64_t)t.u + 1);
                s_aln.put('\t');
                put_uint(s_aln, (uint64_t)(t.exit_ov >> 1) + 1);
                s_aln.put('\t');
                if (W) { if (p == 0) { cp_dst = s_aln.p; cp_src = rows; cp_L = L; cp_R = R; } s_aln.p += L; }
                else s_aln.n += L;
                s_aln.put('\n');
                if (W && p == 0) cp_step = (uint32_t)(s_aln.p - row_start);
            }
            core_cov = (unsigned long long)t.core_mean;
            core_num = 1;
            const pf_bubble_site *sites = a.osites + r.site_off;
            const uint32_t *ilen = a.oilen + r.ilen_off;
            const size_t usize = a.len[t.u], esize = a.len[t.exit_ov >> 1];
            const uint32_t ns = r.n_sites;
            uint32_t indel = 0;
            uint64_t vcur = t.strict ? 0 : a.sv_off[j];
            for (uint32_t i = 0; i < ns; ++i) {
                const pf_bubble_site sr = sites[i];
                const uint8_t *grp = a.ogroups + r.group_off + (uint64_t)i * R;
                uint32_t vd;
                if (i == 0) {
                    if (ns != 1) vd = (uint32_t)std::min((size_t)(uint32_t)(sites[1].col - sites[0].col - 1), usize);
                    else vd = (uint32_t)std::min(usize, esize);
                } else if (i == ns - 1) {
                    vd = (uint32_t)std::min((size_t)(uint32_t)(sites[i].col - sites[i - 1].col - 1), esize);
                } else {
                    vd = std::min((uint32_t)(sites[i].col - sites[i - 1].col - 1), (uint32_t)(sites[i + 1].col - sites[i].col - 1));
                }
                const uint32_t maxnum = sr.maxnum;
                if (sr.is_indel) ++indel;
                if (COLORED) {
                    const uint32_t C = a.n_colors;
                    const double *cvals = nullptr;
                    if (!t.strict) {
                        cvals = a.sv + vcur;
                        vcur += (uint64_t)C * maxnum + 1;
                        if (!sr.pad_) continue;
                    }
                    uint32_t wu[4] = {0, 0, 0, 0}, lk[4] = {1, 1, 1, 1};
                    if (t.strict)
                        for (uint32_t p = 0; p < R && p < 4; ++p) {
                            wu[p] = t.inner[p] >> 1;
                            lk[p] = a.len[wu[p]] - (uint32_t)a.k + 1;
                        }
                    auto m_at = [&](uint32_t c, uint32_t p) -> double {
                        const uint32_t q = p < 4 ? p : 3;
                        return colour_in(a.full, a.cwords, wu[q], c) ? (double)a.ccov_sum[(size_t)c * a.N + wu[q]] / (double)lk[q] : 0.0;
                    };
                    auto gc_at = [&](uint32_t c, uint32_t x) -> double {
                        if (!t.strict) return cvals[(size_t)c * maxnum + x];
                        double tc = 0.0;
                        for (uint32_t p = 0; p < R; ++p)
                            if ((uint32_t)grp[p] - 1 == x) tc += m_at(c, p);
                        return tc;
                    };
                    const double coefficient = t.strict ? max_cramer_v_dev(m_at, C, R) : max_cramer_v_dev(gc_at, C, maxnum);
                    for (uint32_t c = 0; c < C; ++c) {
                        uint32_t n_res = 0;
                        double sum = 0;
                        for (uint32_t x = 0; x < maxnum; ++x) {
                            const double v = gc_at(c, x);
                            if (v > 0.0) { ++n_res; sum += v; }
                        }
                        if (n_res < 2) continue;
                        const int ar = (int)n_res - 2;
                        Row<W> cov = ar == 0 ? s_cov[0] : ar == 1 ? s_cov[1] : ar == 2 ? s_cov[2] : s_cov[3];
                        Row<W> fre = ar == 0 ? s_fre[0] : ar == 1 ? s_fre[1] : ar == 2 ? s_fre[2] : s_fre[3];
                        const bool filed = ar <= 3;
                        for (uint32_t x = 0; x < maxnum; ++x) {
                            const double v = gc_at(c, x);
                            if (!(v > 0.0)) continue;
                            if (filed) { put_double(cov, v); cov.put('\t'); }
// ... 17 lines not shown
                            put_uint(cov, my_vc);
                            cov.put('\t');
                            put_uint(cov, ns);
                            cov.put('\t');
                            put_double(cov, coefficient);
                            cov.put('\t');
                            put_uint(cov, vd);
                            cov.put('\t'); cov.put('\n');
                            ++allele[ar];
                            if (ar == 0) { s_cov[0] = cov; s_fre[0] = fre; }
                            else if (ar == 1) { s_cov[1] = cov; s_fre[1] = fre; }
                            else if (ar == 2) { s_cov[2] = cov; s_fre[2] = fre; }
                            else { s_cov[3] = cov; s_fre[3] = fre; }
                        }
                    }
                    continue;
                }
                double denom;
                const double *vals = nullptr;
                if (t.strict) {
                    denom = t.cov_sum;
                } else {
                    vals = a.sv + vcur;
                    vcur += maxnum + 1;
                    if (!sr.pad_) continue;
                    denom = vals[maxnum];
                }
                const int ar = (int)maxnum - 2;
                Row<W> cov = ar == 0 ? s_cov[0] : ar == 1 ? s_cov[1] : ar == 2 ? s_cov[2] : s_cov[3];
                Row<W> fre = ar == 0 ? s_fre[0] : ar == 1 ? s_fre[1] : ar == 2 ? s_fre[2] : s_fre[3];
                const bool filed = ar >= 0 && ar <= 3;
                for (uint32_t x = 0; x < maxnum; ++x) {
                    double tc;
                    if (t.strict) {
                        tc = 0.0;
                        for (uint32_t p = 0; p < R; ++p)
                            if ((uint32_t)grp[p] - 1 == x) tc += t.cov[p < 4 ? p : 3];
                    } else {
                        tc = vals[x];
                    }
                    if (filed) { put_double(cov, tc); cov.put('\t'); }
                    const double fr = tc / denom;
                    if (filed) {
                        if (!a.mt) {
                            Tee<W> both{fre, s_all};
                            put_double(both, fr);
                            both.put('\n');
                        } else {
                            put_double(fre, fr);
                            fre.put('\n');
                        }
                    } else if (!a.mt) {
                        put_double(s_all, fr);
                        s_all.put('\n');
                    }
                }
                if (filed) {
                    cov.put(t.strict ? '1' : '0'); cov.put('\t');
                    if (sr.is_indel) put_uint(cov, open_run_len(ilen, indel - 1, r.n_indel_len, r.n_cols, sr.col));
                    else cov.put('0');
                    cov.put('\t');
                    put_uint(cov, my_vc);
                    cov.put('\t');
                    put_uint(cov, ns);
                    cov.put('\t');
                    put_uint(cov, vd);
                    cov.put('\t'); cov.put('\n');
                    ++allele[ar];
                    if (ar == 0) { s_cov[0] = cov; s_fre[0] = fre; }
                    else if (ar == 1) { s_cov[1] = cov; s_fre[1] = fre; }
                    else if (ar == 2) { s_cov[2] = cov; s_fre[2] = fre; }
                    else { s_cov[3] = cov; s_fre[3] = fre; }
                }
            }
            if (a.mt) {
                const int n_ar = t.strict ? 4 : 3;
                for (int x = 0; x < n_ar; ++x) {
                    if (W) { for (char *c = fre_start[x]; c < s_fre[x].p; ++c) *s_all.p++ = *c; }
                    else s_all.n += s_fre[x].n - fre_n0[x];
                }
            }
        }
        if (!W) {
            a.sizes[0 * stride + jj] = s_all.n;
            a.sizes[1 * stride + jj] = s_aln.n;
            a.sizes[(size_t)S_PACK * stride + jj] = (a.packed && s_aln.n) ? ALNPACK_HEADER + r.n_rows * alnpack_row_bytes(r.n_cols) : 0u;
#pragma unroll
            for (int x = 0; x < 4; ++x) {
                a.sizes[(2 + x) * stride + jj] = s_fre[x].n;
                a.sizes[(6 + x) * stride + jj] = s_cov[x].n;
            }
        }
    }
    if (W) {
        {
            unsigned long long todo = __ballot(cp_R != 0);
            const int lane = lane_id();
            while (todo) {
                const int b = __ffsll((long long)todo) - 1;
                todo &= todo - 1;
                const uint32_t Lb = read_lane(cp_L, b), Rb = read_lane(cp_R, b), step = read_lane(cp_step, b);
                const uint64_t d64 = (uint64_t)(uintptr_t)cp_dst, s64 = (uint64_t)(uintptr_t)cp_src;
                char *dst = reinterpret_cast<char *>((uintptr_t)(((uint64_t)read_lane((uint32_t)(d64 >> 32), b) << 32) | read_lane((uint32_t)d64, b)));
                const char *src = reinterpret_cast<const char *>((uintptr_t)(((uint64_t)read_lane((uint32_t)(s64 >> 32), b) << 32) | read_lane((uint32_t)s64, b)));
                if (a.packed) {
                    const uint32_t rb = alnpack_row_bytes(Lb);
                    for (uint32_t p = 0; p < Rb; ++p)
                        for (uint32_t x0 = 0; x0 < Lb; x0 += WAVE) {
                            const uint32_t x = x0 + (uint32_t)lane;
                            uint32_t v = x < Lb ? alnpack_code(src[(size_t)p * Lb + x]) << (3 * (lane & 7)) : 0u;
                            v |= (uint32_t)__shfl_xor((int)v, 1, WAVE);
                            v |= (uint32_t)__shfl_xor((int)v, 2, WAVE);
                            v |= (uint32_t)__shfl_xor((int)v, 4, WAVE);
                            const uint32_t g = x >> 3, byte = (uint32_t)lane & 7;
                            if (byte < 3 && (g << 3) < Lb) dst[(size_t)p * rb + 3 * (size_t)g + byte] = (char)(v >> (8 * byte));
                        }
                    continue;
                }
                for (uint32_t p = 0; p < Rb; ++p)
                    for (uint32_t x = (uint32_t)lane; x < Lb; x += WAVE) dst[(size_t)p * step + x] = src[(size_t)p * Lb + x];
            }
        }
        if (a.packed && jj < a.nb && (jj % ALNPACK_GROUP == 0 || jj + 1 == a.nb)) {
            const size_t stride = (size_t)a.nb + 1;
            char *idx = a.out[S_PACK];
            auto entry = [&](uint64_t g, uint32_t at) {
                const uint64_t e[2] = {a.offs[1 * stride + at] - a.offs[1 * stride], a.offs[(size_t)S_PACK * stride + at] - a.offs[(size_t)S_PACK * stride]};
                __builtin_memcpy(idx + 16 + 16 * g, e, 16);
            };
            if (jj % ALNPACK_GROUP == 0) entry(jj / ALNPACK_GROUP, jj);
            if (jj + 1 == a.nb) {
                const uint64_t n_groups = ((uint64_t)a.nb + ALNPACK_GROUP - 1) / ALNPACK_GROUP;
                const uint64_t head[2] = {n_groups, ALNPACK_GROUP};
                __builtin_memcpy(idx, head, 16);
                entry(n_groups, a.nb);
            }
        }
        __builtin_amdgcn_fence(__ATOMIC_SEQ_CST, "workgroup");
        __builtin_amdgcn_wave_barrier();
        const size_t stride = (size_t)a.nb + 1;
#pragma unroll
        for (int q = 0; q < 4; ++q) {
            if (!staged[q]) continue;
            const bool pk = q == 0 && a.packed;
            const int st_ = pk ? S_PACK : FMT_STAGED_STREAM[q];
            char *dst = a.out[st_] + (pk ? alnpack_index_bytes(a.nb) : 0) + (span0[q] - a.offs[st_ * stride]);
            const uint32_t n_words = span_len[q] >> 2;
            for (uint32_t x = lane_id(); x < n_words; x += WAVE) {
                const uint32_t w = reinterpret_cast<const uint32_t *>(stage[q])[x];
                __builtin_memcpy(dst + 4 * (size_t)x, &w, 4);
            }
            for (uint32_t x = (n_words << 2) + lane_id(); x < span_len[q]; x += WAVE) dst[x] = stage[q][x];
        }
    }
    if (!W) {
        unsigned long long v[7] = {allele[0], allele[1], allele[2], allele[3], core_cov, core_num, 0};
        for (int x = 0; x < 6; ++x) {
            const unsigned long long s = wave_sum_u64(v[x]);
            if (lane_id() == 0 && s) atomicAdd(reinterpret_cast<unsigned long long *>(reinterpret_cast<char *>(a.cnt) + offsetof(CallCounters, allele)) + x, s);
        }
        if (jj == a.nb) {
            const size_t stride = (size_t)a.nb + 1;
            for (int s = 0; s < N_INT; ++s) a.sizes[s * stride + a.nb] = 0;
        }
    }
}

__global__ void k_call_totals(const uint64_t *__restrict__ offs, const uint32_t *__restrict__ sizes, uint32_t nb, uint64_t *__restrict__ totals) {
    const int s = threadIdx.x;
    const size_t stride = (size_t)nb + 1;
    if (s < N_INT) totals[s] = offs[s * stride + nb] - offs[s * stride];
    (void)sizes;
}


__device__ inline uint32_t sb_rows_of(const SbArgs &a, uint32_t u, bool &p_row, bool &m_row) {
    const uint8_t f = a.flags[u];
    p_row = m_row = false;
    if ((f & 3) == 0) return 0;
    if (a.colored) { p_row = a.plus[u] != 0; m_row = a.minus[u] != 0; }
    else { p_row = (f & B_PLUS) != 0; m_row = (f & B_MINUS) != 0; }
    return (uint32_t)p_row + (uint32_t)m_row;
}

__global__ void k_sb_count(SbArgs a, uint32_t *cnt) {
    const uint32_t u = blockIdx.x * blockDim.x + threadIdx.x;
    if (u > a.N) return;
    bool p, m;
    cnt[u] = u < a.N ? sb_rows_of(a, u, p, m) : 0u;
}

constexpr uint32_t SB_STAGE = 4096;

template <bool W>
__global__ __launch_bounds__(256) void k_sb_format(SbArgs a) {
    const uint32_t u = blockIdx.x * blockDim.x + threadIdx.x;
    __shared__ __attribute__((aligned(16))) char s_stage[W ? 4 * SB_STAGE : 4];
    char *stage = s_stage + (threadIdx.x >> 6) * SB_STAGE;
    uint64_t span0 = 0;
    uint32_t span_len = 0;
    bool staged = false;
    if (W) {
        const uint32_t w_first = u & ~63u;
        if (w_first < a.N) {
            const uint32_t w_end = w_first + 64 < a.N ? w_first + 64 : a.N;
            span0 = a.offs[w_first];
            span_len = (uint32_t)(a.offs[w_end] - span0);
            staged = span_len <= SB_STAGE;
        }
    }
    if (u < a.N) {
        bool rows[2];
        const uint32_t n = sb_rows_of(a, u, rows[0], rows[1]);
        Row<W> o{W ? (staged ? stage + (a.offs[u] - span0) : a.out + a.offs[u]) : nullptr, 0};
        if (n) {
            const uint8_t f = a.flags[u];
            uint64_t nb = (uint64_t)a.row_base[u] + a.first_id;
            for (int side = 0; side < 2; ++side) {
                if (!rows[side]) continue;
                const bool ps = side == 0;
                put_uint(o, nb++);
                o.put('\t');
                put_uint(o, (uint64_t)u + 1);
                o.put('\t'); o.put(ps ? '+' : '-'); o.put('\t');
                put_uint(o, ps ? a.plus[u] : a.minus[u]);
                o.put('\t'); o.put((f & (ps ? B_STRICT_P : B_STRICT_M)) ? '1' : '0');
                o.put('\t'); o.put((f & (ps ? B_COMPLEX_P : B_COMPLEX_M)) ? '1' : '0');
                o.put('\n');
            }
        }
        if (!W) a.sizes[u] = o.n;
    } else if (u == a.N && !W) {
        a.sizes[u] = 0;
    }
    if (W && staged) {
        __builtin_amdgcn_fence(__ATOMIC_SEQ_CST, "workgroup");
        __builtin_amdgcn_wave_barrier();
        char *dst = a.out + span0;
        const uint32_t n_words = span_len >> 2;
        for (uint32_t x = lane_id(); x < n_words; x += WAVE) {
            const uint32_t w = reinterpret_cast<const uint32_t *>(stage)[x];
            __builtin_memcpy(dst + 4 * (size_t)x, &w, 4);
        }
        for (uint32_t x = (n_words << 2) + lane_id(); x < span_len; x += WAVE) dst[x] = stage[x];
    }
}


__global__ void k_format_doubles(const double *__restrict__ x, uint64_t n, char *__restrict__ out, uint8_t *__restrict__ len) {
    const uint64_t i = (uint64_t)blockIdx.x * blockDim.x + threadIdx.x;
    if (i >= n) return;
    BufSink s{out + i * 32};
    put_double(s, x[i]);
    len[i] = (uint8_t)(s.p - (out + i * 32));
}
// ... 45 lines not shown
```

### ploidyfrost_amd/csrc/pf_nibble.hpp

```cpp
#pragma once
#include <stdint.h>
#include <string.h>

namespace pf {

constexpr char kNibbleAlphabet[17] = "0123456789.\t\n-e+";

inline unsigned nibble_code(char c) {
    for (unsigned i = 0; i < 16; ++i)
        if (kNibbleAlphabet[i] == c) return i;
    return 16;
}

inline void nibble_expand(char *dst, const uint8_t *src, uint64_t n) {
    static const struct Lut {
        uint16_t two[256];
        Lut() {
            for (int b = 0; b < 256; ++b) two[b] = (uint16_t)((uint8_t)kNibbleAlphabet[b & 15] | ((uint16_t)(uint8_t)kNibbleAlphabet[b >> 4] << 8));
        }
    } lut;
    uint64_t i = 0;
    for (; i + 16 <= n; i += 16) {
        uint64_t in;
        memcpy(&in, src + (i >> 1), 8);
        uint16_t w[8];
        for (int x = 0; x < 8; ++x) w[x] = lut.two[(in >> (8 * x)) & 0xFF];
        memcpy(dst + i, w, 16);
    }
    for (; i + 2 <= n; i += 2) {
        const uint16_t w = lut.two[src[i >> 1]];
        memcpy(dst + i, &w, 2);
    }
    if (i < n) dst[i] = (char)(lut.two[src[i >> 1]] & 0xFF);
}

}
```

### ploidyfrost_amd/hipapi.py

```python
from __future__ import annotations

import ctypes as C
import os

import numpy as np

PKG = os.path.dirname(os.path.abspath(__file__))
LIB_PATH = os.path.join(PKG, "csrc", "libploidyfrost_hip.so")

NONE = 0xFFFFFFFF
PF_OK, PF_ERR_ARG, PF_ERR_HIP, PF_ERR_NO_DEVICE, PF_ERR_OVERFLOW, PF_ERR_MISSING_KMER = range(6)
KERNELS = ["k_table_build", "k_adj_insert", "k_adj_probe", "k_cov", "k_bfs", "k_bfs_big", "k_align", "k_align_big",
           "k_strcov", "k_bubble", "k_bubble_big", "k_cov_colored", "k_strcov_colored", "k_gmm", "k_kmc_decode", "k_minz_count", "k_cov_join",
           "k_call_sides", "k_call_prep", "k_call_paths", "k_call_sites", "k_call_format", "k_call_snp", "k_bfs_thread", "k_call_pair", "k_call_stack", "k_cov_join_rest", "copy_text_to_host", "k_call_model"]

K_DENSITY = len(KERNELS)
K_HIST = K_DENSITY + 1
HIST_MAX_BINS = 1 << 20
K_MASK = K_HIST + 1
MASK_STATS = np.dtype([(f, "<u8") for f in ("reads", "reads_changed", "bases", "bases_masked", "kmers", "kmers_bad")])
MASK_NO_UPPER = 0xFFFFFFFF
K_COUNT = K_MASK + 1
COUNT_STATS = np.dtype([(f, "<u8") for f in ("reads", "bases", "kmers", "kmers_bad", "unique", "below_min", "above_max", "written")])
K_TRIM = K_COUNT + 1
# ... 86 lines not shown
        "pf_bfs_candidates_resident": (i, [vp, C.c_uint32, C.c_uint32, C.POINTER(u64), C.POINTER(u64), vp, vp, u64, C.POINTER(u64)]),
        "pf_replay_device": (i, [vp, C.c_uint32, C.c_uint32, C.POINTER(u64), C.POINTER(u64)]),
        "pf_replay_big_fetch": (i, [vp, vp, vp, vp]),
        "pf_replay_set_colours": (i, [vp, C.c_uint32, vp, vp, vp]),
        "pf_replay_finish": (i, [vp, vp, vp, vp, u64]),
        "pf_call_get_state": (i, [vp, vp, vp, vp]),
        "pf_gfa_ingest": (i, [vp, vp, u64, i, i, C.POINTER(C.c_uint32), C.POINTER(C.c_uint32)]),
        "pf_gfa_parse": (i, [vp, vp, u64, i, i, C.POINTER(C.c_uint32), C.POINTER(C.c_uint32)]),
        "pf_gfa_upload": (i, [vp]),
        "pf_gfa_error": (C.c_char_p, [vp]),
        "pf_gfa_segments": (i, [vp, vp, vp, vp, vp, vp, C.POINTER(C.c_int)]),
        "pf_replay_order": (i, [vp, C.c_uint32, vp, vp, vp]),
        "pf_kernel_name": (C.c_char_p, [i]),
        "pf_upload_graph": (i, [vp, vp, vp, vp, u32, i]),
        "pf_build_adjacency": (i, [vp, vp, vp]),
        "pf_upload_counts": (i, [vp, vp, vp, u64, u32, u64, u64, i]),
        "pf_join_counts": (i, [vp]),
        "pf_join_counts_begin": (i, [vp]),
        "pf_join_counts_end": (i, [vp]),
        "pf_lookup_kmers": (i, [vp, vp, u64, vp, vp]),
        "pf_unitig_cov": (i, [vp, u32, u32, vp, vp, vp]),
        "pf_unitig_cov_probe": (i, [vp, u32, u32, vp, vp, vp]),
        "pf_count_candidates": (i, [vp, u32, u32, C.POINTER(u64)]),
        "pf_bfs_candidates": (i, [vp, u32, u32, vp, u64, vp, u64, C.POINTER(u64), C.POINTER(u64)]),
        "pf_align_batch": (i, [vp, vp, u64, vp, u32, C.c_double, C.c_double, C.c_double, vp, vp, vp, u64, vp, u64, vp, u64,
                               C.POINTER(u64)]),
        "pf_align_bubbles": (i, [vp, vp, u64, vp, u64, vp, u32, C.c_double, C.c_double, C.c_double, vp, vp, u64, vp, u64, vp, u64,
                                 vp, u64, C.POINTER(u64)]),
        "pf_string_cov": (i, [vp, vp, vp, u32, u32, u32, vp, vp, vp]),
        "pf_host_alloc": (i, [vp, C.c_size_t, C.POINTER(vp)]),
        "pf_selftest_scan": (i, [vp, u64, C.c_uint32]),
        "pf_call_set_numeric_packed": (i, [vp, i]),
        "pf_call_fetch_text": (i, [vp, i, i, vp, u64]),
        "pf_host_free": (None, [vp, vp]),
        "pf_device_name": (i, [vp, C.c_char_p, C.c_size_t]),
        "pf_device_pci_bus_id": (i, [vp, C.c_char_p, C.c_size_t]),
        "pf_table_capacity": (u64, [vp]),
        "pf_num_kmers": (u64, [vp]),
        "pf_upload_counts_colored": (i, [vp, u32, vp, vp, vp, vp, vp, vp]),
        "pf_num_colors": (u32, [vp]),
        "pf_unitig_cov_colored": (i, [vp, u32, u32, vp, vp, vp, vp]),
        "pf_unitig_cov_colored_probe": (i, [vp, u32, u32, vp, vp, vp, vp]),
        "pf_string_cov_colored": (i, [vp, vp, vp, u32, vp, vp, vp, vp]),
        "pf_unitig_cov_exact": (i, [vp, u32, u32, i, vp, vp, vp]),
        "pf_minimizer_table_slots": (u64, [u64]),
        "pf_minimizer_crowding": (i, [vp, i, u32, vp, vp, vp]),
        "pf_minimizer_replay_inputs": (i, [vp, i, C.c_uint32, vp, vp]),
        "pf_kmc_decode": (i, [vp, vp, u64, u32, u32, vp, u64, u32, u32, vp, vp]),
        "pf_device_free": (None, [vp, vp]),
        "pf_copy_to_host": (i, [vp, vp, vp, C.c_size_t]),
        "pf_gmm_upload": (i, [vp, vp, u64]),
        "pf_gmm_count": (u64, [vp]),
        "pf_gmm_fit": (i, [vp, u32, C.c_double, C.c_double, C.c_int32, C.c_double, vp, vp, vp, vp, vp]),
        "pf_call_set_state": (i, [vp, vp, vp, vp]),
        "pf_call_coverage": (i, [vp]),
        "pf_call_set_format": (i, [vp, i]),
        "pf_superbubble_rows": (i, [vp, i, C.POINTER(u64), C.POINTER(u64)]),
        "pf_superbubble_fetch": (i, [vp, vp, u64]),
        "pf_call_scan": (i, [vp, u32, u32, C.POINTER(u64)]),
        "pf_call_sides": (i, [vp, vp, u64]),
        "pf_call_resolve": (i, [vp, C.POINTER(u64), C.POINTER(u32), C.POINTER(u32)]),
        "pf_call_select": (i, [vp, vp, u64]),
        "pf_call_run": (i, [vp, i, u64, u64, u64, u32, C.c_double, C.c_double, C.c_double, vp]),
        "pf_call_align": (i, [vp, u64, u64, u32, C.c_double, C.c_double, C.c_double, vp]),
        "pf_call_text": (i, [vp, i, u64, vp]),
        "pf_call_set_alignseq_packed": (i, [vp, i]),
        "pf_comm_unique_id": (i, [vp]),
        "pf_comm_init": (i, [vp, vp, i, i]),
        "pf_gather": (i, [vp, vp, C.c_uint32, vp]),
        "pf_comm_destroy": (None, [vp]),
        "pf_call_peek": (i, [vp, i, vp, vp, vp, u64, vp, vp, vp, vp, vp, vp, vp]),
        "pf_call_reserve": (i, [vp, u64, C.c_uint32]),
        "pf_call_reserve_lanes": (i, [vp, u64, C.c_uint32, C.c_int]),
        "pf_timing_select": (i, [vp, u64]),
        "pf_kernel_busy": (i, [vp, u64, C.POINTER(C.c_double)]),
        "pf_call_reserve_text": (i, [vp, u64]),
        "pf_find_reserve": (i, [vp, u64]),
        "pf_call_set_colours": (i, [vp, u32, vp, vp, vp, vp, vp, vp, u64, u64]),
        "pf_call_set_cutoffs": (i, [vp, u32, vp, vp]),
        "pf_call_text_range": (i, [vp, i, u64, u64, u64, vp]),
        "pf_call_align_lane": (i, [vp, i, u64, u64, u32, C.c_double, C.c_double, C.c_double, vp]),
        "pf_call_text_range_lane": (i, [vp, i, i, u64, u64, u64, vp]),
        "pf_call_text_sizes": (i, [vp, i, u64, u64, u64, vp]),
        "pf_bfs_live_deferred": (i, [vp, u64, vp]),
        "pf_bfs_live_count": (i, [vp, vp]),
        "pf_call_fetch": (i, [vp, i, i, vp, u64]),
        "pf_call_fetch_slab": (i, [vp, i, vp, vp]),
        "pf_call_fetch_range": (i, [vp, i, u64, vp, u64, i]),
        "pf_call_fetch_wait": (i, [vp, i]),
        "pf_format_doubles": (i, [vp, vp, u64, vp, vp]),
        "pf_gmm_values": (i, [vp, vp, u64]),
        "pf_call_model_begin": (i, [vp, i, C.c_double]),
        "pf_call_model_take": (i, [vp, i]),
        "pf_call_model_finish": (i, [vp, C.POINTER(u64)]),
        "pf_call_fetched_bytes": (u64, [vp]),
        "pf_call_model_filter": (i, [vp, vp]),
        "pf_call_model_take_text": (i, [vp, i, C.c_char_p, u64]),
        "pf_call_model_filter_multi": (i, [vp, vp, i]),
        "pf_call_model_color_count": (C.c_uint32, [vp]),
        "pf_call_model_color_select": (i, [vp, i, C.POINTER(u64)]),
        "pf_gmm_density": (i, [vp, u32, C.c_double, vp, vp, vp]),
        "pf_count_histogram": (i, [vp, vp, u64, u64, u64, u32, vp]),
        "pf_mask_reads": (i, [vp, vp, u64, vp, vp, u64, u32, u32, vp, vp]),
        "pf_mask_fastq": (i, [vp, vp, u64, i, u32, u32, vp, C.POINTER(u64), vp, C.POINTER(u64)]),
        "pf_count_begin": (i, [vp, u32, i, u64]),
        "pf_count_reads": (i, [vp, vp, u64, vp, vp, u64, vp]),
        "pf_count_fastq": (i, [vp, vp, u64, i, C.POINTER(u64), vp, C.POINTER(u64)]),
        "pf_count_finish": (i, [vp, u64, u64, u64, C.POINTER(vp), C.POINTER(vp), C.POINTER(u64), vp]),
        "pf_count_abort": (i, [vp]),
        "pf_kmc_encode": (i, [vp, vp, vp, u64, u32, u32, u32, vp, vp]),
        "pf_unitig_build": (i, [vp, vp, u64, u32, u32, i, i, vp]),
        "pf_unitig_fetch": (i, [vp, u64, u64, vp]),
        "pf_unitig_release": (i, [vp]),
        "pf_unitig_text": (i, [vp, C.POINTER(vp), C.POINTER(u64)]),
        "pf_maskcount_reads": (i, [vp, vp, u64, vp, vp, u64, u32, u32, vp]),
        "pf_maskcount_fastq": (i, [vp, vp, u64, i, u32, u32, C.POINTER(u64), vp, C.POINTER(u64)]),
        "pf_unitig_build_colored": (i, [vp, vp, u64, u32, u32, i, i, u32, vp, C.POINTER(u64)]),
        "pf_color_begin": (i, [vp, u32]),
        "pf_color_reads": (i, [vp, u32, vp, u64, vp, vp, u64, vp]),
        "pf_color_fastq": (i, [vp, u32, vp, u64, i, C.POINTER(u64), vp, C.POINTER(u64)]),
        "pf_color_finish": (i, [vp, vp]),
        "pf_color_kmers": (i, [vp, u32, vp, u64, vp]),
        "pf_release_counts": (i, [vp]),
        "pf_kmer_union": (i, [vp, u32, vp, vp, C.POINTER(vp), C.POINTER(u64)]),
        "pf_color_fetch": (i, [vp, vp, vp, vp, vp, vp]),
        "pf_trim_fastq": (i, [vp, vp, u64, i, vp, u32, u32, vp, C.POINTER(u64), C.POINTER(u64), vp, vp, C.POINTER(u64), vp, C.POINTER(u64)]),
        "pf_trim_fastq_pair": (i, [vp, vp, u64, vp, u64, i, vp, u32, u32, C.POINTER(vp), C.POINTER(u64), C.POINTER(u64), C.POINTER(vp), C.POINTER(vp),
                                   C.POINTER(u64), vp, C.POINTER(u64)]),
        "pf_trim_table_fastq": (i, [vp, vp, u64, i, vp, vp, vp, C.POINTER(u64), C.POINTER(u64), C.POINTER(u64), vp, C.POINTER(u64)]),
        "pf_trim_table_fastq_pair": (i, [vp, vp, u64, vp, u64, i, vp, C.POINTER(vp), C.POINTER(vp), C.POINTER(u64), C.POINTER(u64), C.POINTER(u64), vp,
                                         C.POINTER(u64)]),
        "pf_count_fastq_trimmed": (i, [vp, vp, u64, i, vp, C.POINTER(u64), vp, vp, C.POINTER(u64)]),
        "pf_count_fastq_pair_trimmed": (i, [vp, vp, u64, vp, u64, i, vp, C.POINTER(u64), vp, vp, C.POINTER(u64)]),
        "pf_maskcount_fastq_trimmed": (i, [vp, vp, u64, i, vp, u32, u32, C.POINTER(u64), vp, vp, C.POINTER(u64)]),
        "pf_maskcount_fastq_pair_trimmed": (i, [vp, vp, u64, vp, u64, i, vp, u32, u32, C.POINTER(u64), vp, vp, C.POINTER(u64)]),
    }
    for name, (res, args) in sig.items():
        fn = getattr(L, name)
        fn.restype = res
        fn.argtypes = args
    _lib = L
    return L


DECLARED_SYMBOLS = ["pf_create", "pf_warmup", "pf_destroy", "pf_last_error", "pf_set_stream", "pf_synchronize", "pf_enable_timing",
                    "pf_kernel_time", "pf_reset_timing", "pf_device_busy", "pf_kernel_units", "pf_side_components", "pf_replay_order", "pf_bfs_candidates_begin", "pf_bfs_candidates_end", "pf_fetch", "pf_bfs_candidates_resident", "pf_bfs_live_deferred", "pf_bfs_live_count", "pf_replay_device", "pf_replay_big_fetch", "pf_replay_set_colours", "pf_replay_finish", "pf_call_get_state", "pf_gfa_ingest", "pf_gfa_segments", "pf_gfa_parse", "pf_gfa_upload", "pf_gfa_error", "pf_kernel_name", "pf_upload_graph", "pf_build_adjacency",
                    "pf_upload_counts", "pf_join_counts", "pf_join_counts_begin", "pf_join_counts_end", "pf_lookup_kmers", "pf_unitig_cov", "pf_count_candidates", "pf_bfs_candidates",
                    "pf_align_batch", "pf_align_bubbles", "pf_string_cov", "pf_host_alloc", "pf_host_free", "pf_device_name", "pf_device_pci_bus_id", "pf_table_capacity", "pf_num_kmers",
                    "pf_upload_counts_colored", "pf_num_colors", "pf_unitig_cov_colored", "pf_string_cov_colored",
                    "pf_gmm_upload", "pf_gmm_count", "pf_gmm_fit", "pf_kmc_decode", "pf_device_free", "pf_copy_to_host",
                    "pf_minimizer_table_slots", "pf_minimizer_crowding", "pf_minimizer_replay_inputs", "pf_bfs_candidates_split", "pf_unitig_cov_exact", "pf_unitig_cov_probe", "pf_unitig_cov_colored_probe",
                    "pf_call_set_state", "pf_call_set_format", "pf_superbubble_rows", "pf_superbubble_fetch", "pf_call_coverage", "pf_call_scan", "pf_call_sides", "pf_call_resolve", "pf_call_select", "pf_call_run", "pf_call_align",
                    "pf_call_text", "pf_call_set_alignseq_packed", "pf_comm_unique_id", "pf_comm_init", "pf_gather", "pf_comm_destroy", "pf_call_reserve", "pf_call_reserve_lanes", "pf_timing_select", "pf_kernel_busy", "pf_call_reserve_text", "pf_selftest_scan", "pf_call_set_numeric_packed", "pf_call_fetch_text", "pf_find_reserve", "pf_call_set_colours", "pf_call_set_cutoffs", "pf_call_peek", "pf_call_text_range", "pf_call_align_lane", "pf_call_text_range_lane", "pf_call_text_sizes", "pf_call_fetch", "pf_call_fetch_slab", "pf_call_fetch_range", "pf_call_fetch_wait", "pf_format_doubles",
                    "pf_gmm_values", "pf_call_model_begin", "pf_call_model_take", "pf_call_model_finish", "pf_call_fetched_bytes",
                    "pf_call_model_filter", "pf_call_model_take_text",
                    "pf_call_model_filter_multi", "pf_call_model_color_count", "pf_call_model_color_select",
                    "pf_gmm_density", "pf_count_histogram", "pf_mask_reads", "pf_mask_fastq",
                    "pf_count_begin", "pf_count_reads", "pf_count_fastq", "pf_count_finish", "pf_count_abort", "pf_kmc_encode",
                    "pf_trim_fastq", "pf_trim_fastq_pair", "pf_unitig_build", "pf_unitig_fetch", "pf_unitig_release",
                    "pf_unitig_build_colored", "pf_color_begin", "pf_color_reads", "pf_color_fastq", "pf_color_finish", "pf_color_fetch",
                    "pf_maskcount_reads", "pf_maskcount_fastq", "pf_unitig_text",
                    "pf_kmer_union", "pf_color_kmers", "pf_release_counts",
                    "pf_trim_table_fastq", "pf_trim_table_fastq_pair", "pf_count_fastq_trimmed", "pf_count_fastq_pair_trimmed",
                    "pf_maskcount_fastq_trimmed", "pf_maskcount_fastq_pair_trimmed"]


class TrimPlan(C.Structure):
    _fields_ = [("steps", C.c_void_p), ("n_steps", C.c_uint32), ("phred", C.c_uint32)]


def trim_steps(steps) -> np.ndarray:
    if isinstance(steps, np.ndarray) and steps.dtype == TRIM_STEP:
        return np.ascontiguousarray(steps)
    if isinstance(steps, str):
        steps = steps.split()
    out = np.zeros(len(steps), dtype=TRIM_STEP)
    for j, s in enumerate(steps):
        if isinstance(s, str):
            name, *fields = s.split(":")
            s = (TRIM_KINDS[name],) + tuple(int(x) for x in fields)
        out[j] = tuple(s) + (0,) * (3 - len(s))
    return out


def density_dict(x: np.ndarray, density: np.ndarray, info: np.ndarray) -> dict:
    r = info[0]
    return {"x": x, "density": density, "bw": float(r["bw"]), "n": int(r["n"]), "min": float(r["min"]), "max": float(r["max"]),
            "sd": float(r["sd"]), "q1": float(r["q1"]), "q3": float(r["q3"]), "order": np.array(r["order"], dtype=np.float64)}


def call_peek(ctx_handle, lane: int = 0):
    L = load_library()
    h = C.c_void_p(ctx_handle)
    used = (C.c_uint64 * 6)()
    st = L.pf_call_peek(h, lane, None, None, None, 0, None, None, None, None, None, None, used)
    if st != PF_OK:
        raise DeviceError(st, L.pf_last_error(h).decode())
    nb = int(used[0])
    if nb == 0:
        return []
    cap = (C.c_uint64 * 5)(*[int(used[x + 1]) for x in range(5)])
    bub = np.zeros(nb, dtype=CALL_BUBBLE)
    res = np.zeros(nb, dtype=BUBBLE_RESULT)
    sv_off = np.zeros(nb, dtype=np.uint64)
    text = np.zeros(max(1, cap[0]), dtype=np.uint8)
    sites = np.zeros(max(1, cap[1]), dtype=BUBBLE_SITE)
    groups = np.zeros(max(1, cap[2]), dtype=np.uint8)
    ilen = np.zeros(max(1, cap[3]), dtype=np.uint32)
    sv = np.zeros(max(1, cap[4]), dtype=np.float64)
    st = L.pf_call_peek(h, lane, bub.ctypes.data, res.ctypes.data, sv_off.ctypes.data, nb, text.ctypes.data, sites.ctypes.data,
                        groups.ctypes.data, ilen.ctypes.data, sv.ctypes.data, cap, used)
    if st != PF_OK:
        raise DeviceError(st, L.pf_last_error(h).decode())
    tb = text.tobytes()
    out = []
    for j in range(nb):
        b, r = bub[j], res[j]
        d = dict(entrance_ov=int(b["entrance_ov"]), exit_ov=int(b["exit_ov"]), strict=bool(b["strict"]),
                 inner=[int(x) for x in b["inner"][: int(b["n_inner"])]], cov=[float(x) for x in b["cov"][: int(b["n_inner"])]],
                 core_mean=float(b["core_mean"]), cov_sum=float(b["cov_sum"]), rows=None)
        R, Lc = int(r["n_rows"]), int(r["n_cols"])
        if R:
            o = int(r["rows_off"])
            d["rows"] = [tb[o + i * Lc: o + (i + 1) * Lc] for i in range(R)]
            d["sites"] = []
            d["site_cov"] = []
            v = int(sv_off[j])
            for i in range(int(r["n_sites"])):
                srec = sites[int(r["site_off"]) + i]
                g0 = int(r["group_off"]) + i * R
                mx = int(srec["maxnum"])
                d["sites"].append((int(srec["col"]), int(srec["is_indel"]), mx, groups[g0: g0 + R].tolist(), int(srec["pad"])))
                if not d["strict"]:
                    d["site_cov"].append((sv[v: v + mx].tolist(), float(sv[v + mx])))
                    v += mx + 1
            d["indel_len"] = ilen[int(r["ilen_off"]): int(r["ilen_off"]) + int(r["n_indel_len"])].tolist()
# ... 780 lines not shown
```

Before: 247.1 million.

## Size text once per lane range on device and vectorise host expansion with AVX2

Text output sizing moves from a per-chunk size-then-write call to one device sizing pass per lane range, on a dedicated size stream with precomputed bound rows. Each chunk then only writes, and allele and core-coverage totals are taken from that single sizing pass. Separately, the host nibble and alignment-pack expansion gain AVX2 paths and a two-digit integer formatter. This is meant to cut repeated sizing launches and host expansion cost, but it adds reserve-time warmup work and a lot of new code paths.

Measured after the change: 253.6 million, median of 6. 1.03x the previous value.

```diff
diff --git a/include/ploidyfrost_hip.h b/include/ploidyfrost_hip.h
--- a/include/ploidyfrost_hip.h
+++ b/include/ploidyfrost_hip.h
@@ -377,6 +377,8 @@
 int pf_call_text_range_lane(pf_ctx *, int lane, int slab, uint64_t first, uint64_t count, uint64_t var_count_base,
                             pf_call_result *out);
 int pf_call_text_sizes(pf_ctx *, int lane, uint64_t first, uint64_t count, uint64_t var_count_base, pf_call_result *out);
+int pf_call_text_size_lane(pf_ctx *, int lane, uint64_t var_count_base, uint64_t piece_bubbles, pf_call_result *out);
+int pf_call_text_write_lane(pf_ctx *, int lane, int slab, uint64_t first, uint64_t count, pf_call_result *out);
 int pf_call_fetch(pf_ctx *, int slab, int stream, char *dst, uint64_t len);
 int pf_call_fetch_slab(pf_ctx *, int slab, char *dst, const uint64_t *len);
 int pf_call_fetch_range(pf_ctx *, int slab, uint64_t first_byte, char *dst, uint64_t len, int slot);
diff --git a/ploidyfrost_amd/csrc/host/pf_cdbg_call.cpp b/ploidyfrost_amd/csrc/host/pf_cdbg_call.cpp
--- a/ploidyfrost_amd/csrc/host/pf_cdbg_call.cpp
+++ b/ploidyfrost_amd/csrc/host/pf_cdbg_call.cpp
@@ -308,6 +308,7 @@
     const bool aln_packed = !getenv("PF_ALIGNSEQ_ASCII");
     if (pf_call_set_alignseq_packed(ctx_, aln_packed ? 1 : 0) != PF_OK) return fail(PF_ERR_HIP, std::string(tag_) + "::PloidyEstimation(): " + pf_last_error(ctx_));
     const bool num_packed = !getenv("PF_NUMERIC_ASCII");
+    const bool expand_simd = pf::expand_simd_available() && !getenv("PF_EXPAND_SCALAR");
     if (pf_call_set_numeric_packed(ctx_, num_packed ? 1 : 0) != PF_OK) return fail(PF_ERR_HIP, std::string(tag_) + "::PloidyEstimation(): " + pf_last_error(ctx_));
     if (model_.on && (pf_call_model_begin(ctx_, model_.source, model_.q) != PF_OK || (filter_on_ && pf_call_model_filter(ctx_, &filter_) != PF_OK) ||
                       (multi_on_ && pf_call_model_filter_multi(ctx_, &multi_, multi_each_ ? 1 : 0) != PF_OK)))
@@ -435,7 +436,7 @@
                         spans[n_spans++] = CopySpan{dst, src, d.res.text_len[s]};
                     } else if (nib) {
                         std::vector<char> tmp(d.res.text_len[s]);
-                        pf::nibble_expand(tmp.data(), reinterpret_cast<const uint8_t *>(src), d.res.text_len[s]);
+                        pf::nibble_expand(tmp.data(), reinterpret_cast<const uint8_t *>(src), d.res.text_len[s], expand_simd);
                         if (maps[s].write(files[(size_t)s].bytes, tmp.data(), tmp.size(), T)) files[(size_t)s].rc = 1;
                     } else if (maps[s].write(files[(size_t)s].bytes, src, d.res.text_len[s], T)) files[(size_t)s].rc = 1;
                 }
@@ -456,7 +457,7 @@
                 parallel_chunks(n_aln + cut.size(), 1, T, [&](size_t i, size_t, size_t) {
                     if (i >= n_aln) {
                         const CopySpan &c = cut[i - n_aln];
-                        if (cut_nib[i - n_aln]) pf::nibble_expand(c.dst, reinterpret_cast<const uint8_t *>(c.src), c.len);
+                        if (cut_nib[i - n_aln]) pf::nibble_expand(c.dst, reinterpret_cast<const uint8_t *>(c.src), c.len, expand_simd);
                         else memcpy(c.dst, c.src, (size_t)c.len);
                         return;
                     }
@@ -466,7 +467,7 @@
                     packed.entry(g1, t1_, r1_);
                     if (t1_ > d.res.text_len[PF_OUT_ALIGNSEQ] || t0_ > t1_ || r0_ > r1_ ||
                         (uint64_t)(packed.records - packed.base) + r1_ > d.res.alignseq_packed_len) { bad = 1; return; }
-                    char *end = pf::alnpack_expand(packed.records + r0_, packed.records + r1_, packed_dst + t0_, packed_dst + t1_);
+                    char *end = pf::alnpack_expand(packed.records + r0_, packed.records + r1_, packed_dst + t0_, packed_dst + t1_, expand_simd);
                     if (end != packed_dst + t1_) bad = 1;
                 });
                 if (bad) files[PF_OUT_ALIGNSEQ].rc = 1;
@@ -477,7 +478,7 @@
                 else if (d.res.numeric_packed) {
                     const size_t at0 = last_allfre_.size();
                     last_allfre_.resize(at0 + d.res.text_len[0]);
-                    pf::nibble_expand(&last_allfre_[at0], reinterpret_cast<const uint8_t *>(hb.p + off[0]), d.res.text_len[0]);
+                    pf::nibble_expand(&last_allfre_[at0], reinterpret_cast<const uint8_t *>(hb.p + off[0]), d.res.text_len[0], expand_simd);
                 } else last_allfre_.append(hb.p + off[0], d.res.text_len[0]);
             }
             for (int s = 0; s < PF_CALL_STREAMS; ++s) files[(size_t)s].bytes += d.res.text_len[s];
@@ -564,6 +565,19 @@
                 r = ranges[ri];
             }
             const uint64_t rn = r.a1 - r.a0;
+            {
+                pf_call_result rr;
+                const int st = pf_call_text_size_lane(ctx_, r.lane, var_base, CHUNK, &rr);
+                if (st != PF_OK) {
+                    { std::lock_guard<std::mutex> lk(mu); if (rc == PF_OK) { rc = st; rc_err = pf_last_error(ctx_); } stop = true; }
+                    cv.notify_all();
+                    return;
+                }
+                for (int a = 0; a < 4; ++a) allele_[a] += rr.allele[a];
+                core_cov_ += rr.core_cov;
+                core_num_ += rr.core_num;
+                if (trace) fprintf(stderr, "[ploidy]   range %zu sized on the device %.2f ms\n", ri, since(t_all) * 1e3);
+            }
             for (uint64_t p0 = 0; p0 < rn; p0 += CHUNK, ++b) {
                 const uint64_t count = std::min<uint64_t>(CHUNK, rn - p0);
                 {
@@ -574,7 +588,7 @@
                 Done d;
                 d.slab = (int)(b % PF_CALL_SLABS);
                 d.hslab = (int)(b & 1);
-                int st = pf_call_text_range_lane(ctx_, r.lane, d.slab, p0, count, var_base, &d.res);
+                int st = pf_call_text_write_lane(ctx_, r.lane, d.slab, p0, count, &d.res);
                 if (st == PF_OK && model_.on) st = pf_call_model_take(ctx_, d.slab);
                 if (st != PF_OK) {
                     { std::lock_guard<std::mutex> lk(mu); if (rc == PF_OK) { rc = st; rc_err = pf_last_error(ctx_); } stop = true; }
@@ -606,9 +620,6 @@
                             });
                         });
                 }
-                for (int a = 0; a < 4; ++a) allele_[a] += d.res.allele[a];
-                core_cov_ += d.res.core_cov;
-                core_num_ += d.res.core_num;
                 if (!model_.only) {
                     { std::lock_guard<std::mutex> lk(mu); ready.push_back(d); }
                     cv.notify_all();
diff --git a/ploidyfrost_amd/csrc/pf_alnpack.hpp b/ploidyfrost_amd/csrc/pf_alnpack.hpp
--- a/ploidyfrost_amd/csrc/pf_alnpack.hpp
+++ b/ploidyfrost_amd/csrc/pf_alnpack.hpp
@@ -1,6 +1,8 @@
 #pragma once
 #include <cstdint>
 #include <cstring>
+
+#include "pf_nibble.hpp"
 
 #ifdef __HIPCC__
 #define PF_ALNPACK_HD __host__ __device__
@@ -32,11 +34,32 @@
     return t;
 }
 
+struct AlnPackDigits {
+    char two[200];
+    constexpr AlnPackDigits() : two() {
+        for (int v = 0; v < 100; ++v) { two[2 * v] = (char)('0' + v / 10); two[2 * v + 1] = (char)('0' + v % 10); }
+    }
+};
 inline char *alnpack_put_uint(char *p, uint64_t x) {
+    static constexpr AlnPackDigits D{};
     char tmp[24];
-    int n = 0;
-    do { tmp[n++] = (char)('0' + x % 10); x /= 10; } while (x);
-    while (n) *p++ = tmp[--n];
+    char *const e = tmp + 24, *q = e;
+    while (x > 0xFFFFFFFFull) {
+        const uint64_t d = x / 100;
+        q -= 2;
+        memcpy(q, D.two + 2 * (size_t)(x - d * 100), 2);
+        x = d;
+    }
+    uint32_t y = (uint32_t)x;
+    while (y >= 100) {
+        const uint32_t d = y / 100;
+        q -= 2;
+        memcpy(q, D.two + 2 * (size_t)(y - d * 100), 2);
+        y = d;
+    }
+    if (y >= 10) { q -= 2; memcpy(q, D.two + 2 * (size_t)y, 2); }
+    else *--q = (char)('0' + y);
+    while (q < e) *p++ = *q++;
     return p;
 }
 
@@ -60,9 +83,68 @@
     }
 };
 
-inline char *alnpack_expand(const uint8_t *rec, const uint8_t *rec_end, char *dst, const char *dst_end) {
+constexpr char kAlnPackLetters[17] = "-ACGT???????????";
+
+#ifdef PF_EXPAND_AVX2
+__attribute__((target("avx2"))) inline __m256i alnpack_32_avx2(const uint8_t *s) {
+    const __m256i in = _mm256_broadcastsi128_si256(_mm_loadu_si128(reinterpret_cast<const __m128i *>(s)));
+#define PF_ALN_G(b) (b), (b), (b), (b) + 1, (b), (b) + 1, (b) + 1, (b) + 1, (b) + 1, (b) + 2, (b) + 1, (b) + 2, (b) + 2, -1, (b) + 2, -1
+    const __m256i pick_a = _mm256_setr_epi8(PF_ALN_G(0), PF_ALN_G(6));
+    const __m256i pick_b = _mm256_setr_epi8(PF_ALN_G(3), PF_ALN_G(9));
+#undef PF_ALN_G
+    const __m256i mul = _mm256_setr_epi16(128, 16, 2, 64, 8, 1, 32, 4, 128, 16, 2, 64, 8, 1, 32, 4);
+    const __m256i seven = _mm256_set1_epi16(7);
+    const __m256i letters = _mm256_broadcastsi128_si256(_mm_loadu_si128(reinterpret_cast<const __m128i *>(kAlnPackLetters)));
+    const __m256i a = _mm256_and_si256(_mm256_srli_epi16(_mm256_mullo_epi16(_mm256_shuffle_epi8(in, pick_a), mul), 7), seven);
+    const __m256i b = _mm256_and_si256(_mm256_srli_epi16(_mm256_mullo_epi16(_mm256_shuffle_epi8(in, pick_b), mul), 7), seven);
+    return _mm256_shuffle_epi8(letters, _mm256_packus_epi16(a, b));
+}
+
+__attribute__((target("avx2"))) inline char *alnpack_rows_avx2(const uint8_t *rec, const uint8_t *rec_end, uint32_t rb, uint32_t R, uint32_t L,
+                                                                const char *prefix, size_t np, char *dst) {
     const AlnPackTables &T = alnpack_tables();
-    char prefix[96];
+    const bool prefix32 = np <= 32 && np + L + 1 >= 32;
+    for (uint32_t r = 0; r < R; ++r, rec += rb) {
+        if (prefix32) _mm256_storeu_si256(reinterpret_cast<__m256i *>(dst), _mm256_loadu_si256(reinterpret_cast<const __m256i *>(prefix)));
+        else memcpy(dst, prefix, np);
+        dst += np;
+        uint32_t x = 0;
+        const uint8_t *s = rec;
+        for (; x + 32 <= L && (size_t)(rec_end - s) >= 16; x += 32, s += 12)
+            _mm256_storeu_si256(reinterpret_cast<__m256i *>(dst + x), alnpack_32_avx2(s));
+        if (x < L && L - x < 32 && (size_t)(rec_end - s) >= 16 && r + 1 < R && (size_t)(L - x) + 1 + np + L + 1 >= 32) {
+            _mm256_storeu_si256(reinterpret_cast<__m256i *>(dst + x), alnpack_32_avx2(s));
+            x = L;
+        } else if (x < L && L - x < 32 && (size_t)(rec_end - s) >= 16) {
+            char tail[32];
+            _mm256_storeu_si256(reinterpret_cast<__m256i *>(tail), alnpack_32_avx2(s));
+            const uint32_t n = L - x;
+            char *d = dst + x;
+            if (n >= 16) { memcpy(d, tail, 16); memcpy(d + n - 16, tail + n - 16, 16); }
+            else if (n >= 8) { memcpy(d, tail, 8); memcpy(d + n - 8, tail + n - 8, 8); }
+            else if (n >= 4) { memcpy(d, tail, 4); memcpy(d + n - 4, tail + n - 4, 4); }
+            else for (uint32_t i = 0; i < n; ++i) d[i] = tail[i];
+            x = L;
+        }
+        for (; x < L; x += 8, s += 3) {
+            const uint32_t v = (uint32_t)s[0] | (uint32_t)s[1] << 8 | (uint32_t)s[2] << 16;
+            char eight[8];
+            const uint32_t a = T.four[v & 4095], b = T.four[v >> 12];
+            memcpy(eight, &a, 4);
+            memcpy(eight + 4, &b, 4);
+            memcpy(dst + x, eight, L - x < 8 ? L - x : 8);
+        }
+        dst += L;
+        *dst++ = '\n';
+    }
+    return dst;
+}
+#endif
+
+inline char *alnpack_expand(const uint8_t *rec, const uint8_t *rec_end, char *dst, const char *dst_end, bool simd = expand_simd_available()) {
+    const AlnPackTables &T = alnpack_tables();
+    simd = simd && expand_simd_available();
+    char prefix[96] = {};
     while (rec < rec_end) {
         if ((size_t)(rec_end - rec) < ALNPACK_HEADER) return nullptr;
         uint64_t vc;
@@ -84,6 +166,13 @@
         const size_t np = (size_t)(q - prefix);
         const uint32_t rb = alnpack_row_bytes(L);
         if ((uint64_t)R * rb > (uint64_t)(rec_end - rec) || (uint64_t)R * (np + L + 1) > (uint64_t)(dst_end - dst)) return nullptr;
+#ifdef PF_EXPAND_AVX2
+        if (simd) {
+            dst = alnpack_rows_avx2(rec, rec_end, rb, R, L, prefix, np, dst);
+            rec += (size_t)R * rb;
+            continue;
+        }
+#endif
         for (uint32_t r = 0; r < R; ++r, rec += rb) {
             memcpy(dst, prefix, np);
             dst += np;
diff --git a/ploidyfrost_amd/csrc/pf_call.hip b/ploidyfrost_amd/csrc/pf_call.hip
--- a/ploidyfrost_amd/csrc/pf_call.hip
+++ b/ploidyfrost_amd/csrc/pf_call.hip
@@ -1,3 +1,5 @@
+#include <functional>
+
 #include "pf_call_kernels.hpp"
 #include "pf_scan.hpp"
 
@@ -796,6 +798,7 @@
     memset(out, 0, sizeof(*out));
     CallState::AlignOut &O = S->lane[lane];
     O.nb = 0;
+    O.sized_nb = 0;
     O.t0 = t0;
     O.cur = pf_call_result{};
     if (t1 == t0) return PF_OK;
@@ -875,6 +878,9 @@
     if (sv && O.used[4]) PF_HIP(hipMemcpy(sv, O.sv.p, O.used[4] * 8, hipMemcpyDeviceToHost));
     return PF_OK;
 }
+
+static int lane_size_stream(pf_ctx *ctx, CallState::AlignOut &O);
+static int lane_size_tables(pf_ctx *ctx, CallState::AlignOut &O, uint32_t nb, uint64_t n_rows);
 
 int pf_call_reserve_lanes(pf_ctx *ctx, uint64_t nb64, uint32_t complex_size, int n_lanes) {
     if (!ctx || nb64 == 0 || n_lanes < 1 || n_lanes > PF_CALL_LANES) return PF_ERR_ARG;
@@ -897,6 +903,18 @@
         trace.mark("reserve: a lane's streams and events");
         PF_TRY(bubble_reserve(ctx, nb, lane));
         trace.mark("reserve: K-BUBBLE's workspaces and first launches");
+        PF_TRY(lane_size_stream(ctx, O));
+        PF_TRY(lane_size_tables(ctx, O, nb, 64));
+        {
+            FmtArgs fa;
+            memset(&fa, 0, sizeof(fa));
+            fa.sizes = O.tsizes.as<uint32_t>(); fa.offs = O.toffs.as<uint64_t>(); fa.cnt = O.tcounters.as<CallCounters>();
+            if (S->n_colors) k_call_format<false, true><<<1, FMT_BLOCK, 0, O.size_stream>>>(fa);
+            else k_call_format<false, false><<<1, FMT_BLOCK, 0, O.size_stream>>>(fa);
+            PF_HIP(hipGetLastError());
+            PF_HIP(hipStreamSynchronize(O.size_stream));
+        }
+        trace.mark("reserve: K-TEXT's tables of a range");
     }
     return PF_OK;
 }
@@ -939,106 +957,72 @@
     return PF_OK;
 }
 
-static int call_text_impl(pf_ctx *ctx, int lane, int slab, uint64_t first, uint64_t count, uint64_t var_count_base, pf_call_result *out, bool sizes_only) {
-    if (!ctx || !out || slab < 0 || slab >= PF_CALL_SLABS || lane < 0 || lane >= PF_CALL_LANES) return PF_ERR_ARG;
-    CallState *S = ctx->call;
-    if (!S) return PF_ERR_ARG;
-    CallState::AlignOut &O = S->lane[lane];
-    if (first + count > O.nb) { pf::CtxErr{ctx} = "pf_call_text_range: range outside the aligned batch"; return PF_ERR_ARG; }
-    if (S->n_colors && S->mt_format) { pf::CtxErr{ctx} = "pf_call_text_range: the -t > 1 format is the single-sample path's"; return PF_ERR_ARG; }
-    if (!sizes_only)
-        for (int s = 0; s < N_STREAMS; ++s) S->out_len[slab][s] = 0;
-    *out = O.cur;
-    out->n_called = 0;
-    if (count == 0) return PF_OK;
-    PF_HIP(hipSetDevice(ctx->device));
-    const bool trace_stages = getenv("PF_TRACE_ALIGN") != nullptr;
-    const auto t_enter = std::chrono::steady_clock::now();
-    auto ta = [&](const char *what) {
-        if (trace_stages) fprintf(stderr, "[pf_call_text]    %-34s %.2f ms\n", what, std::chrono::duration<double>(std::chrono::steady_clock::now() - t_enter).count() * 1e3);
-    };
-    const uint32_t nb = (uint32_t)count;
-    const int which = sizes_only ? 0 : (slab & 1);
-    { const int ts = text_work_of(ctx, S, which, nb); if (ts != PF_OK) return ts; }
-    CallState::TextWork &T = S->text[which];
-    hipStream_t st = T.stream;
-    const uint64_t t0 = O.t0;
-    uint32_t vc_edge[2] = {0, 0};
-    PF_HIP(hipMemcpyAsync(&vc_edge[1], O.vc.as<uint32_t>() + (first + count - 1), 4, hipMemcpyDeviceToHost, st));
-    if (first) PF_HIP(hipMemcpyAsync(&vc_edge[0], O.vc.as<uint32_t>() + (first - 1), 4, hipMemcpyDeviceToHost, st));
-    CallCounters *d_cnt = T.tcounters.as<CallCounters>();
-    CallCounters hc;
-    const size_t n_sizes = (size_t)N_INT * (nb + 1);
-    ta("stream and size tables");
-    PF_HIP(hipMemsetAsync(&d_cnt->allele[0], 0, 6 * 8, st));
+static FmtArgs fmt_args(pf_ctx *ctx, CallState *S, CallState::AlignOut &O, uint64_t var_count_base) {
     FmtArgs fa;
-    fa.ct = S->ctask.as<CallTask>(); fa.kept = S->kept.as<uint32_t>(); fa.t0 = t0; fa.j0 = (uint32_t)first; fa.nb = nb;
+    memset(&fa, 0, sizeof(fa));
+    fa.ct = S->ctask.as<CallTask>(); fa.kept = S->kept.as<uint32_t>(); fa.t0 = O.t0;
     fa.res = O.res.as<pf_bubble_result>();
     fa.otext = O.otext.as<char>(); fa.osites = O.osites.as<pf_bubble_site>(); fa.ogroups = O.ogroups.as<uint8_t>();
     fa.oilen = O.oilen.as<uint32_t>(); fa.sv_off = O.sv_off.as<uint64_t>(); fa.sv = O.sv.as<double>(); fa.vc = O.vc.as<uint32_t>();
-    fa.vc_base = var_count_base; fa.mt = S->mt_format ? 1 : 0; fa.len = ctx->d_len; fa.sizes = T.sizes.as<uint32_t>(); fa.offs = T.offs.as<uint64_t>(); fa.cnt = d_cnt;
-    for (int s = 0; s < N_INT; ++s) fa.out[s] = nullptr;
+    fa.vc_base = var_count_base; fa.mt = S->mt_format ? 1 : 0; fa.len = ctx->d_len;
     fa.packed = S->pack_alignseq ? 1 : 0;
-    size_t at = 0;
-    ctx_begin_at(ctx, PF_K_CALL_FORMAT, st, &at);
     fa.n_colors = S->n_colors; fa.N = ctx->N; fa.k = ctx->k; fa.full = S->col_full.as<uint64_t>(); fa.cwords = S->col_words; fa.ccov_sum = S->ccov_sum.as<uint64_t>();
-    if (S->n_colors) k_call_format<false, true><<<(nb + 1 + FMT_BLOCK - 1) / FMT_BLOCK, FMT_BLOCK, 0, st>>>(fa);
-    else k_call_format<false, false><<<(nb + 1 + FMT_BLOCK - 1) / FMT_BLOCK, FMT_BLOCK, 0, st>>>(fa);
-    ctx_end_at(ctx, at, st);
-    PF_HIP(scan_exclusive_u32_u64(T.sizes.as<uint32_t>(), T.offs.as<uint64_t>(), n_sizes, T.tscan.p, st));
-    k_call_totals<<<1, 64, 0, st>>>(T.offs.as<uint64_t>(), T.sizes.as<uint32_t>(), nb, T.totals.as<uint64_t>());
-    uint64_t totals[N_INT + 1] = {};
-    PF_HIP(hipMemcpyAsync(totals, T.totals.p, N_INT * 8, hipMemcpyDeviceToHost, st));
-    PF_HIP(hipMemcpyAsync(&hc, d_cnt, sizeof(hc), hipMemcpyDeviceToHost, st));
-    PF_HIP(hipStreamSynchronize(st));
-    out->n_called = vc_edge[1] - vc_edge[0];
+    return fa;
+}
+
+static int text_write_pass(pf_ctx *ctx, CallState *S, CallState::AlignOut &O, FmtArgs fa, const uint64_t *totals, int slab, pf_call_result *out,
+                           const std::function<void(const char *)> &ta) {
+    const uint32_t nb = fa.nb;
+    const int which = slab & 1;
+    hipStream_t st = S->text[which].stream;
     const uint64_t packed_len = (fa.packed && totals[PF_OUT_ALIGNSEQ]) ? alnpack_index_bytes(nb) + totals[S_PACK] : 0;
     auto slab_len = [&](int s) { return (s == PF_OUT_ALIGNSEQ && fa.packed) ? packed_len : totals[s]; };
     out->alignseq_packed_len = packed_len;
+    const bool direct = S->pack_numeric;
     uint64_t all = 0;
-    for (int s = 0; s < N_STREAMS; ++s) all += slab_len(s);
-    if (sizes_only) {
-        for (int s = 0; s < N_STREAMS; ++s) out->text_len[s] = totals[s];
-        for (int x = 0; x < 4; ++x) out->allele[x] = hc.allele[x];
-        out->core_cov = hc.core_cov;
-        out->core_num = hc.core_num;
-        return PF_OK;
-    }
-    ta("sizes counted");
+    for (int s = 0; s < N_STREAMS; ++s) all += (direct && s == PF_OUT_ALIGNSEQ) ? 0 : slab_len(s);
     PF_TRY(need(ctx, "pf_call_text", {{&S->out[slab], std::max<uint64_t>(all, 16)}}));
     ta("slab taken");
     all = 0;
     for (int s = 0; s < N_STREAMS; ++s) {
+        const uint64_t here = (direct && s == PF_OUT_ALIGNSEQ) ? 0 : slab_len(s);
         fa.out[s] = S->out[slab].as<char>() + all;
         S->out_off[slab][s] = all;
-        S->out_len[slab][s] = slab_len(s);
+        S->out_len[slab][s] = here;
         out->text_len[s] = totals[s];
-        all += slab_len(s);
+        all += here;
+    }
+    S->fetch_base[slab] = S->out[slab].as<char>();
+    S->nib[slab] = false;
+    S->aln_direct[slab] = false;
+    out->numeric_packed = 0;
+    for (int s = 0; s < N_STREAMS; ++s) { S->txt_off[slab][s] = S->out_off[slab][s]; S->txt_len[slab][s] = S->out_len[slab][s]; }
+    uint64_t foff[N_STREAMS] = {}, flen[N_STREAMS] = {}, fall = 0;
+    char *pb = nullptr;
+    if (S->pack_numeric) {
+        for (int s = 0; s < N_STREAMS; ++s) {
+            flen[s] = s == PF_OUT_ALIGNSEQ ? ((slab_len(s) + 15) & ~15ull) : PF_NUMERIC_PACKED_LEN(totals[s]);
+            foff[s] = fall;
+            fall += flen[s];
+        }
+        PF_TRY(need(ctx, "pf_call_text", {{&S->outp[slab], fall + 16}}));
+        pb = S->outp[slab].as<char>();
+        fa.out[PF_OUT_ALIGNSEQ] = pb + foff[PF_OUT_ALIGNSEQ];
+        S->txt_off[slab][PF_OUT_ALIGNSEQ] = foff[PF_OUT_ALIGNSEQ];
+        S->txt_len[slab][PF_OUT_ALIGNSEQ] = slab_len(PF_OUT_ALIGNSEQ);
+        S->aln_direct[slab] = true;
     }
     if (fa.packed) { fa.out[S_PACK] = fa.out[PF_OUT_ALIGNSEQ]; fa.out[PF_OUT_ALIGNSEQ] = nullptr; }
     if (S->model.read_ev[slab]) PF_HIP(hipStreamWaitEvent(st, S->model.read_ev[slab], 0));
+    size_t at = 0;
     ctx_begin_at(ctx, PF_K_CALL_FORMAT, st, &at);
     if (S->n_colors) k_call_format<true, true><<<(nb + FMT_BLOCK - 1) / FMT_BLOCK, FMT_BLOCK, 0, st>>>(fa);
     else k_call_format<true, false><<<(nb + FMT_BLOCK - 1) / FMT_BLOCK, FMT_BLOCK, 0, st>>>(fa);
     ctx_end_at(ctx, at, st);
     ctx_units(ctx, PF_K_CALL_FORMAT, nb);
     PF_HIP(hipGetLastError());
-    S->fetch_base[slab] = S->out[slab].as<char>();
-    S->nib[slab] = false;
-    out->numeric_packed = 0;
-    for (int s = 0; s < N_STREAMS; ++s) { S->txt_off[slab][s] = S->out_off[slab][s]; S->txt_len[slab][s] = S->out_len[slab][s]; }
     if (S->pack_numeric) {
-        uint64_t foff[N_STREAMS], flen[N_STREAMS], fall = 0;
-        for (int s = 0; s < N_STREAMS; ++s) {
-            flen[s] = s == PF_OUT_ALIGNSEQ ? ((slab_len(s) + 15) & ~15ull) : PF_NUMERIC_PACKED_LEN(totals[s]);
-            foff[s] = fall;
-            fall += flen[s];
-        }
-        PF_TRY(need(ctx, "pf_call_text", {{&S->outp[slab], fall + 16}}));
-        char *pb = S->outp[slab].as<char>();
         PF_HIP(hipMemsetAsync(pb + fall, 0, 16, st));
-        if (slab_len(PF_OUT_ALIGNSEQ))
-            PF_HIP(hipMemcpyAsync(pb + foff[PF_OUT_ALIGNSEQ], S->out[slab].as<char>() + S->txt_off[slab][PF_OUT_ALIGNSEQ], (size_t)slab_len(PF_OUT_ALIGNSEQ), hipMemcpyDeviceToDevice, st));
         NibArgs na;
         int x = 0;
         uint64_t units = 0;
@@ -1065,10 +1049,156 @@
     PF_HIP(hipEventRecord(S->text_ev[slab], st));
     if (!O.read_ev[which]) PF_HIP(hipEventCreateWithFlags(&O.read_ev[which], hipEventDisableTiming));
     PF_HIP(hipEventRecord(O.read_ev[which], st));
+    return PF_OK;
+}
+
+static int call_text_impl(pf_ctx *ctx, int lane, int slab, uint64_t first, uint64_t count, uint64_t var_count_base, pf_call_result *out, bool sizes_only) {
+    if (!ctx || !out || slab < 0 || slab >= PF_CALL_SLABS || lane < 0 || lane >= PF_CALL_LANES) return PF_ERR_ARG;
+    CallState *S = ctx->call;
+    if (!S) return PF_ERR_ARG;
+    CallState::AlignOut &O = S->lane[lane];
+    if (first + count > O.nb) { pf::CtxErr{ctx} = "pf_call_text_range: range outside the aligned batch"; return PF_ERR_ARG; }
+    if (S->n_colors && S->mt_format) { pf::CtxErr{ctx} = "pf_call_text_range: the -t > 1 format is the single-sample path's"; return PF_ERR_ARG; }
+    if (!sizes_only)
+        for (int s = 0; s < N_STREAMS; ++s) S->out_len[slab][s] = 0;
+    *out = O.cur;
+    out->n_called = 0;
+    if (count == 0) return PF_OK;
+    PF_HIP(hipSetDevice(ctx->device));
+    const bool trace_stages = getenv("PF_TRACE_ALIGN") != nullptr;
+    const auto t_enter = std::chrono::steady_clock::now();
+    auto ta = [&](const char *what) {
+        if (trace_stages) fprintf(stderr, "[pf_call_text]    %-34s %.2f ms\n", what, std::chrono::duration<double>(std::chrono::steady_clock::now() - t_enter).count() * 1e3);
+    };
+    const uint32_t nb = (uint32_t)count;
+    const int which = sizes_only ? 0 : (slab & 1);
+    { const int ts = text_work_of(ctx, S, which, nb); if (ts != PF_OK) return ts; }
+    CallState::TextWork &T = S->text[which];
+    hipStream_t st = T.stream;
+    uint32_t vc_edge[2] = {0, 0};
+    PF_HIP(hipMemcpyAsync(&vc_edge[1], O.vc.as<uint32_t>() + (first + count - 1), 4, hipMemcpyDeviceToHost, st));
+    if (first) PF_HIP(hipMemcpyAsync(&vc_edge[0], O.vc.as<uint32_t>() + (first - 1), 4, hipMemcpyDeviceToHost, st));
+    CallCounters *d_cnt = T.tcounters.as<CallCounters>();
+    CallCounters hc;
+    const size_t n_sizes = (size_t)N_INT * (nb + 1);
+    ta("stream and size tables");
+    PF_HIP(hipMemsetAsync(&d_cnt->allele[0], 0, 6 * 8, st));
+    FmtArgs fa = fmt_args(ctx, S, O, var_count_base);
+    fa.j0 = (uint32_t)first; fa.nb = nb; fa.tstride = nb + 1; fa.tj0 = 0;
+    fa.sizes = T.sizes.as<uint32_t>(); fa.offs = T.offs.as<uint64_t>(); fa.cnt = d_cnt;
+    size_t at = 0;
+    ctx_begin_at(ctx, PF_K_CALL_FORMAT, st, &at);
+    if (S->n_colors) k_call_format<false, true><<<(nb + 1 + FMT_BLOCK - 1) / FMT_BLOCK, FMT_BLOCK, 0, st>>>(fa);
+    else k_call_format<false, false><<<(nb + 1 + FMT_BLOCK - 1) / FMT_BLOCK, FMT_BLOCK, 0, st>>>(fa);
+    ctx_end_at(ctx, at, st);
+    PF_HIP(scan_exclusive_u32_u64(T.sizes.as<uint32_t>(), T.offs.as<uint64_t>(), n_sizes, T.tscan.p, st));
+    k_call_totals<<<1, 64, 0, st>>>(T.offs.as<uint64_t>(), T.sizes.as<uint32_t>(), nb, T.totals.as<uint64_t>());
+    uint64_t totals[N_INT + 1] = {};
+    PF_HIP(hipMemcpyAsync(totals, T.totals.p, N_INT * 8, hipMemcpyDeviceToHost, st));
+    PF_HIP(hipMemcpyAsync(&hc, d_cnt, sizeof(hc), hipMemcpyDeviceToHost, st));
+    PF_HIP(hipStreamSynchronize(st));
+    out->n_called = vc_edge[1] - vc_edge[0];
     for (int x = 0; x < 4; ++x) out->allele[x] = hc.allele[x];
     out->core_cov = hc.core_cov;
     out->core_num = hc.core_num;
-    return PF_OK;
+    if (sizes_only) {
+        for (int s = 0; s < N_STREAMS; ++s) out->text_len[s] = totals[s];
+        out->alignseq_packed_len = (fa.packed && totals[PF_OUT_ALIGNSEQ]) ? alnpack_index_bytes(nb) + totals[S_PACK] : 0;
+        return PF_OK;
+    }
+    ta("sizes counted");
+    return text_write_pass(ctx, S, O, fa, totals, slab, out, ta);
+}
+
+static int lane_size_stream(pf_ctx *ctx, CallState::AlignOut &O) {
+    if (O.size_stream) return PF_OK;
+    int least = 0, greatest = 0;
+    PF_HIP(hipDeviceGetStreamPriorityRange(&least, &greatest));
+    PF_HIP(hipStreamCreateWithPriority(&O.size_stream, hipStreamNonBlocking, greatest));
+    return PF_OK;
+}
+static int lane_size_tables(pf_ctx *ctx, CallState::AlignOut &O, uint32_t nb, uint64_t n_rows) {
+    const size_t n_sizes = (size_t)N_INT * ((size_t)nb + 1);
+    return need(ctx, "pf_call_text_size", {{&O.tsizes, text_sizes_bytes(nb, N_INT)}, {&O.toffs, text_offs_bytes(nb, N_INT)}, {&O.tscan, scan_scratch_bytes(n_sizes)},
+                                           {&O.tcounters, sizeof(CallCounters)}, {&O.tbounds, (size_t)n_rows * (N_INT + 1) * 8}});
+}
+
+int pf_call_text_size_lane(pf_ctx *ctx, int lane, uint64_t var_count_base, uint64_t piece_bubbles, pf_call_result *out) {
+    if (!ctx || !out || lane < 0 || lane >= PF_CALL_LANES || piece_bubbles == 0) return PF_ERR_ARG;
+    CallState *S = ctx->call;
+    if (!S) return PF_ERR_ARG;
+    CallState::AlignOut &O = S->lane[lane];
+    if (S->n_colors && S->mt_format) { pf::CtxErr{ctx} = "pf_call_text_size_lane: the -t > 1 format is the single-sample path's"; return PF_ERR_ARG; }
+    *out = O.cur;
+    out->n_called = 0;
+    O.sized_nb = 0;
+    const uint32_t nb = O.nb;
+    if (nb == 0) return PF_OK;
+    PF_HIP(hipSetDevice(ctx->device));
+    const uint32_t piece = (uint32_t)std::min<uint64_t>(piece_bubbles, 1u << 24);
+    const uint32_t n_rows = (nb + piece - 1) / piece + 1;
+    PF_TRY(lane_size_stream(ctx, O));
+    PF_TRY(lane_size_tables(ctx, O, nb, n_rows));
+    hipStream_t st = O.size_stream;
+    for (hipEvent_t e : O.read_ev) if (e) PF_HIP(hipStreamWaitEvent(st, e, 0));
+    CallCounters *d_cnt = O.tcounters.as<CallCounters>();
+    CallCounters hc;
+    PF_HIP(hipMemsetAsync(&d_cnt->allele[0], 0, 6 * 8, st));
+    FmtArgs fa = fmt_args(ctx, S, O, var_count_base);
+    fa.j0 = 0; fa.nb = nb; fa.tstride = nb + 1; fa.tj0 = 0;
+    fa.sizes = O.tsizes.as<uint32_t>(); fa.offs = O.toffs.as<uint64_t>(); fa.cnt = d_cnt;
+    size_t at = 0;
+    ctx_begin_at(ctx, PF_K_CALL_FORMAT, st, &at);
+    if (S->n_colors) k_call_format<false, true><<<(nb + 1 + FMT_BLOCK - 1) / FMT_BLOCK, FMT_BLOCK, 0, st>>>(fa);
+    else k_call_format<false, false><<<(nb + 1 + FMT_BLOCK - 1) / FMT_BLOCK, FMT_BLOCK, 0, st>>>(fa);
+    ctx_end_at(ctx, at, st);
+    const size_t n_sizes = (size_t)N_INT * ((size_t)nb + 1);
+    PF_HIP(scan_exclusive_u32_u64(O.tsizes.as<uint32_t>(), O.toffs.as<uint64_t>(), n_sizes, O.tscan.p, st));
+    const uint32_t n_vals = n_rows * (uint32_t)(N_INT + 1);
+    k_call_bounds<<<(n_vals + 255) / 256, 256, 0, st>>>(O.toffs.as<uint64_t>(), O.vc.as<uint32_t>(), nb, piece, n_rows, O.tbounds.as<uint64_t>());
+    PF_HIP(hipGetLastError());
+    O.bounds.assign(n_vals, 0);
+    PF_HIP(hipMemcpyAsync(O.bounds.data(), O.tbounds.p, (size_t)n_vals * 8, hipMemcpyDeviceToHost, st));
+    PF_HIP(hipMemcpyAsync(&hc, d_cnt, sizeof(hc), hipMemcpyDeviceToHost, st));
+    PF_HIP(hipStreamSynchronize(st));
+    const uint64_t *b0 = O.bounds.data(), *b1 = O.bounds.data() + (size_t)(n_rows - 1) * (N_INT + 1);
+    for (int s = 0; s < N_STREAMS; ++s) out->text_len[s] = b1[s] - b0[s];
+    out->alignseq_packed_len = 0;
+    out->n_called = b1[N_INT] - b0[N_INT];
+    for (int x = 0; x < 4; ++x) out->allele[x] = hc.allele[x];
+    out->core_cov = hc.core_cov;
+    out->core_num = hc.core_num;
+    O.sized_nb = nb; O.sized_piece = piece; O.sized_vc_base = var_count_base;
+    O.sized_packed = S->pack_alignseq; O.sized_mt = S->mt_format;
+    return PF_OK;
+}
+
+int pf_call_text_write_lane(pf_ctx *ctx, int lane, int slab, uint64_t first, uint64_t count, pf_call_result *out) {
+    if (!ctx || !out || slab < 0 || slab >= PF_CALL_SLABS || lane < 0 || lane >= PF_CALL_LANES) return PF_ERR_ARG;
+    CallState *S = ctx->call;
+    if (!S) return PF_ERR_ARG;
+    CallState::AlignOut &O = S->lane[lane];
+    if (!O.sized_nb || O.sized_nb != O.nb) { pf::CtxErr{ctx} = "pf_call_text_write_lane: the lane was not sized since it was aligned (pf_call_text_size_lane)"; return PF_ERR_ARG; }
+    if (first >= O.nb || first % O.sized_piece != 0 || count != std::min<uint64_t>(O.sized_piece, O.nb - first)) {
+        pf::CtxErr{ctx} = "pf_call_text_write_lane: not a piece of the sized range";
+        return PF_ERR_ARG;
+    }
+    if (O.sized_packed != S->pack_alignseq || O.sized_mt != S->mt_format) { pf::CtxErr{ctx} = "pf_call_text_write_lane: the text settings changed since the lane was sized"; return PF_ERR_ARG; }
+    for (int s = 0; s < N_STREAMS; ++s) S->out_len[slab][s] = 0;
+    *out = O.cur;
+    for (int x = 0; x < 4; ++x) out->allele[x] = 0;
+    out->core_cov = out->core_num = 0;
+    PF_HIP(hipSetDevice(ctx->device));
+    const uint32_t nb = (uint32_t)count;
+    { const int ts = text_work_of(ctx, S, slab & 1, 0); if (ts != PF_OK) return ts; }
+    const uint64_t *b0 = O.bounds.data() + (size_t)(first / O.sized_piece) * (N_INT + 1), *b1 = b0 + (N_INT + 1);
+    uint64_t totals[N_INT];
+    for (int s = 0; s < N_INT; ++s) totals[s] = b1[s] - b0[s];
+    out->n_called = b1[N_INT] - b0[N_INT];
+    FmtArgs fa = fmt_args(ctx, S, O, O.sized_vc_base);
+    fa.j0 = (uint32_t)first; fa.nb = nb; fa.tstride = O.sized_nb + 1; fa.tj0 = (uint32_t)first;
+    fa.sizes = O.tsizes.as<uint32_t>(); fa.offs = O.toffs.as<uint64_t>(); fa.cnt = O.tcounters.as<CallCounters>();
+    return text_write_pass(ctx, S, O, fa, totals, slab, out, [](const char *) {});
 }
 
 int pf_call_set_numeric_packed(pf_ctx *ctx, int on) {
@@ -1086,7 +1216,8 @@
     if (len == 0) return PF_OK;
     if (hipSetDevice(ctx->device) != hipSuccess || !S->copy_stream) return PF_ERR_HIP;
     if (S->text_ev[slab] && hipStreamWaitEvent(S->copy_stream, S->text_ev[slab], 0) != hipSuccess) return PF_ERR_HIP;
-    if (hipMemcpyAsync(dst, S->out[slab].as<char>() + S->txt_off[slab][stream], (size_t)len, hipMemcpyDeviceToHost, S->copy_stream) != hipSuccess) return PF_ERR_HIP;
+    const char *base = (stream == PF_OUT_ALIGNSEQ && S->aln_direct[slab]) ? S->outp[slab].as<char>() : S->out[slab].as<char>();
+    if (hipMemcpyAsync(dst, base + S->txt_off[slab][stream], (size_t)len, hipMemcpyDeviceToHost, S->copy_stream) != hipSuccess) return PF_ERR_HIP;
     if (hipStreamSynchronize(S->copy_stream) != hipSuccess) return PF_ERR_HIP;
     S->fetched_bytes.fetch_add(len, std::memory_order_relaxed);
     return PF_OK;
diff --git a/ploidyfrost_amd/csrc/pf_call_kernels.hpp b/ploidyfrost_amd/csrc/pf_call_kernels.hpp
--- a/ploidyfrost_amd/csrc/pf_call_kernels.hpp
+++ b/ploidyfrost_amd/csrc/pf_call_kernels.hpp
@@ -126,6 +126,12 @@
         pf_call_result cur = {};
         uint64_t used[5] = {};
         hipEvent_t read_ev[2] = {nullptr, nullptr};
+        DevBuf tsizes, toffs, tscan, tcounters, tbounds;
+        hipStream_t size_stream = nullptr;
+        std::vector<uint64_t> bounds;
+        uint32_t sized_nb = 0, sized_piece = 0;
+        uint64_t sized_vc_base = 0;
+        bool sized_packed = false, sized_mt = false;
     } lane[PF_CALL_LANES];
     struct AlignWork {
         DevBuf counters, btask, bpath, ptext, queues, blist, slist, plist, plist2, klist, klist_b, stack_scr, pair_scr, pair_scr2, has, scan_tmp, scan_tmp2, paths_scr, sites_scr;
@@ -149,6 +155,7 @@
     DevBuf outp[PF_CALL_SLABS];
     const char *fetch_base[PF_CALL_SLABS] = {};
     bool nib[PF_CALL_SLABS] = {};
+    bool aln_direct[PF_CALL_SLABS] = {};
     uint64_t txt_len[PF_CALL_SLABS][N_STREAMS] = {}, txt_off[PF_CALL_SLABS][N_STREAMS] = {};
     hipStream_t copy_stream = nullptr;
     hipEvent_t fetch_ev[2] = {nullptr, nullptr};
@@ -193,6 +200,9 @@
         for (AlignOut &o : lane) {
             for (DevBuf *b : {&o.res, &o.otext, &o.osites, &o.ogroups, &o.oilen, &o.sv_off, &o.sv, &o.vc}) b->release();
             for (hipEvent_t &e : o.read_ev) if (e) { (void)hipEventDestroy(e); e = nullptr; }
+            for (DevBuf *b : {&o.tsizes, &o.toffs, &o.tscan, &o.tcounters, &o.tbounds}) b->release();
+            if (o.size_stream) { (void)hipStreamDestroy(o.size_stream); o.size_stream = nullptr; }
+            o.sized_nb = 0;
         }
         for (AlignWork &w : work) {
             for (DevBuf *b : {&w.counters, &w.btask, &w.bpath, &w.ptext, &w.queues, &w.blist, &w.slist, &w.plist, &w.plist2, &w.klist, &w.klist_b, &w.stack_scr,
@@ -491,6 +501,7 @@
     const uint32_t *len;
     uint32_t *sizes;
     const uint64_t *offs;
+    uint32_t tstride, tj0;
     char *out[N_INT];
     int packed;
     CallCounters *cnt;
@@ -537,6 +548,7 @@
 __global__ void k_call_has(const pf_bubble_result *, uint32_t, uint32_t *);
 template <bool W, bool COLORED> __global__ void k_call_format(FmtArgs);
 __global__ void k_call_totals(const uint64_t *, const uint32_t *, uint32_t, uint64_t *);
+__global__ void k_call_bounds(const uint64_t *, const uint32_t *, uint32_t, uint32_t, uint32_t, uint64_t *);
 __global__ void k_sb_count(SbArgs, uint32_t *);
 template <bool W> __global__ void k_sb_format(SbArgs);
 __global__ void k_format_doubles(const double *, uint64_t, char *, uint8_t *);
diff --git a/ploidyfrost_amd/csrc/pf_call_plan.hpp b/ploidyfrost_amd/csrc/pf_call_plan.hpp
--- a/ploidyfrost_amd/csrc/pf_call_plan.hpp
+++ b/ploidyfrost_amd/csrc/pf_call_plan.hpp
@@ -64,6 +64,9 @@
 }
 inline uint64_t row_text_need(uint64_t path_text_used, uint32_t n_branching, uint32_t nb) { return 3 * path_text_used + 128ull * n_branching + 160ull * nb; }
 
+inline uint64_t text_sizes_bytes(uint32_t nb, int rows) { return (uint64_t)rows * ((uint64_t)nb + 1) * 4; }
+inline uint64_t text_offs_bytes(uint32_t nb, int rows) { return ((uint64_t)rows * ((uint64_t)nb + 1) + 1) * 8; }
+
 inline uint64_t reserve_job_index_bytes(uint32_t nb) { return (uint64_t)nb / 4 * 4 + 4096; }
 inline uint64_t reserve_site_values(uint32_t nb, const CallGrids &g) { return (uint64_t)nb / 4 + 1024ull * g.sites + 1024; }
 
diff --git a/ploidyfrost_amd/csrc/pf_call_text.hip b/ploidyfrost_amd/csrc/pf_call_text.hip
--- a/ploidyfrost_amd/csrc/pf_call_text.hip
+++ b/ploidyfrost_amd/csrc/pf_call_text.hip
@@ -66,6 +66,9 @@
 __global__ __launch_bounds__(FMT_BLOCK, W ? 3 : 4) void k_call_format(FmtArgs a) {
     const uint32_t jj = blockIdx.x * blockDim.x + threadIdx.x;
     const uint32_t j = a.j0 + jj;
+    const size_t stride = a.tstride;
+    const uint64_t *const offs = a.offs + a.tj0;
+    uint32_t *const sizes = a.sizes + a.tj0;
     unsigned long long allele[4] = {0, 0, 0, 0}, core_cov = 0, core_num = 0;
     __shared__ __attribute__((aligned(16))) char s_stage[W ? (FMT_BLOCK / 64) * (FMT_STAGE[0] + FMT_STAGE[1] + FMT_STAGE[2] + FMT_STAGE[3]) : 4];
     bool staged[4] = {false, false, false, false};
@@ -76,7 +79,6 @@
     const char *cp_src = nullptr;
     uint32_t cp_L = 0, cp_R = 0, cp_step = 0;
     if (W) {
-        const size_t stride = (size_t)a.nb + 1;
         const uint32_t w_first = jj & ~63u;
         if (w_first < a.nb) {
             const uint32_t w_end = w_first + 64 < a.nb ? w_first + 64 : a.nb;
@@ -85,8 +87,8 @@
 #pragma unroll
             for (int q = 0; q < 4; ++q) {
                 const int st_ = (q == 0 && a.packed) ? S_PACK : FMT_STAGED_STREAM[q];
-                span0[q] = a.offs[st_ * stride + w_first];
-                span_len[q] = (uint32_t)(a.offs[st_ * stride + w_end] - span0[q]);
+                span0[q] = offs[st_ * stride + w_first];
+                span_len[q] = (uint32_t)(offs[st_ * stride + w_end] - span0[q]);
                 staged[q] = span_len[q] <= FMT_STAGE[q];
                 stage[q] = base + acc;
                 acc += FMT_STAGE[q];
@@ -94,21 +96,20 @@
         }
     }
     if (jj < a.nb) {
-        const size_t stride = (size_t)a.nb + 1;
         Row<W> s_all{nullptr, 0}, s_aln{nullptr, 0}, s_fre[4], s_cov[4];
         for (int x = 0; x < 4; ++x) { s_fre[x] = Row<W>{nullptr, 0}; s_cov[x] = Row<W>{nullptr, 0}; }
         if (W) {
-            s_all.p = a.out[0] + (a.offs[0 * stride + jj] - a.offs[0 * stride]);
-            if (!a.packed) s_aln.p = a.out[1] + (a.offs[1 * stride + jj] - a.offs[1 * stride]);
+            s_all.p = a.out[0] + (offs[0 * stride + jj] - offs[0 * stride]);
+            if (!a.packed) s_aln.p = a.out[1] + (offs[1 * stride + jj] - offs[1 * stride]);
 #pragma unroll
             for (int x = 0; x < 4; ++x) {
-                s_fre[x].p = a.out[2 + x] + (a.offs[(2 + x) * stride + jj] - a.offs[(2 + x) * stride]);
-                s_cov[x].p = a.out[6 + x] + (a.offs[(6 + x) * stride + jj] - a.offs[(6 + x) * stride]);
-            }
-            if (staged[0] && !a.packed) s_aln.p = stage[0] + (a.offs[1 * stride + jj] - span0[0]);
-            if (staged[1]) s_all.p = stage[1] + (a.offs[0 * stride + jj] - span0[1]);
-            if (staged[2]) s_fre[0].p = stage[2] + (a.offs[2 * stride + jj] - span0[2]);
-            if (staged[3]) s_cov[0].p = stage[3] + (a.offs[6 * stride + jj] - span0[3]);
+                s_fre[x].p = a.out[2 + x] + (offs[(2 + x) * stride + jj] - offs[(2 + x) * stride]);
+                s_cov[x].p = a.out[6 + x] + (offs[(6 + x) * stride + jj] - offs[(6 + x) * stride]);
+            }
+            if (staged[0] && !a.packed) s_aln.p = stage[0] + (offs[1 * stride + jj] - span0[0]);
+            if (staged[1]) s_all.p = stage[1] + (offs[0 * stride + jj] - span0[1]);
+            if (staged[2]) s_fre[0].p = stage[2] + (offs[2 * stride + jj] - span0[2]);
+            if (staged[3]) s_cov[0].p = stage[3] + (offs[6 * stride + jj] - span0[3]);
         }
         const pf_bubble_result r = a.res[j];
         if (r.n_rows != 0 && r.n_rows != 0xFFFFFFFFu) {
@@ -119,8 +120,8 @@
             char *fre_start[4] = {s_fre[0].p, s_fre[1].p, s_fre[2].p, s_fre[3].p};
             const uint32_t fre_n0[4] = {s_fre[0].n, s_fre[1].n, s_fre[2].n, s_fre[3].n};
             if (W && a.packed) {
-                char *rec = staged[0] ? stage[0] + (a.offs[(size_t)S_PACK * stride + jj] - span0[0])
-                                      : a.out[S_PACK] + alnpack_index_bytes(a.nb) + (a.offs[(size_t)S_PACK * stride + jj] - a.offs[(size_t)S_PACK * stride]);
+                char *rec = staged[0] ? stage[0] + (offs[(size_t)S_PACK * stride + jj] - span0[0])
+                                      : a.out[S_PACK] + alnpack_index_bytes(a.nb) + (offs[(size_t)S_PACK * stride + jj] - offs[(size_t)S_PACK * stride]);
                 const uint64_t vc64 = my_vc;
                 const uint32_t h[4] = {t.u + 1, (t.exit_ov >> 1) + 1, L, R | (t.strict ? 0x80000000u : 0u)};
                 __builtin_memcpy(rec, &vc64, 8);
@@ -304,13 +305,13 @@
             }
         }
         if (!W) {
-            a.sizes[0 * stride + jj] = s_all.n;
-            a.sizes[1 * stride + jj] = s_aln.n;
-            a.sizes[(size_t)S_PACK * stride + jj] = (a.packed && s_aln.n) ? ALNPACK_HEADER + r.n_rows * alnpack_row_bytes(r.n_cols) : 0u;
+            sizes[0 * stride + jj] = s_all.n;
+            sizes[1 * stride + jj] = s_aln.n;
+            sizes[(size_t)S_PACK * stride + jj] = (a.packed && s_aln.n) ? ALNPACK_HEADER + r.n_rows * alnpack_row_bytes(r.n_cols) : 0u;
 #pragma unroll
             for (int x = 0; x < 4; ++x) {
-                a.sizes[(2 + x) * stride + jj] = s_fre[x].n;
-                a.sizes[(6 + x) * stride + jj] = s_cov[x].n;
+                sizes[(2 + x) * stride + jj] = s_fre[x].n;
+                sizes[(6 + x) * stride + jj] = s_cov[x].n;
             }
         }
     }
@@ -344,10 +345,9 @@
             }
         }
         if (a.packed && jj < a.nb && (jj % ALNPACK_GROUP == 0 || jj + 1 == a.nb)) {
-            const size_t stride = (size_t)a.nb + 1;
             char *idx = a.out[S_PACK];
             auto entry = [&](uint64_t g, uint32_t at) {
-                const uint64_t e[2] = {a.offs[1 * stride + at] - a.offs[1 * stride], a.offs[(size_t)S_PACK * stride + at] - a.offs[(size_t)S_PACK * stride]};
+                const uint64_t e[2] = {offs[1 * stride + at] - offs[1 * stride], offs[(size_t)S_PACK * stride + at] - offs[(size_t)S_PACK * stride]};
                 __builtin_memcpy(idx + 16 + 16 * g, e, 16);
             };
             if (jj % ALNPACK_GROUP == 0) entry(jj / ALNPACK_GROUP, jj);
@@ -360,13 +360,12 @@
         }
         __builtin_amdgcn_fence(__ATOMIC_SEQ_CST, "workgroup");
         __builtin_amdgcn_wave_barrier();
-        const size_t stride = (size_t)a.nb + 1;
 #pragma unroll
         for (int q = 0; q < 4; ++q) {
             if (!staged[q]) continue;
             const bool pk = q == 0 && a.packed;
             const int st_ = pk ? S_PACK : FMT_STAGED_STREAM[q];
-            char *dst = a.out[st_] + (pk ? alnpack_index_bytes(a.nb) : 0) + (span0[q] - a.offs[st_ * stride]);
+            char *dst = a.out[st_] + (pk ? alnpack_index_bytes(a.nb) : 0) + (span0[q] - offs[st_ * stride]);
             const uint32_t n_words = span_len[q] >> 2;
             for (uint32_t x = lane_id(); x < n_words; x += WAVE) {
                 const uint32_t w = reinterpret_cast<const uint32_t *>(stage[q])[x];
@@ -382,8 +381,7 @@
             if (lane_id() == 0 && s) atomicAdd(reinterpret_cast<unsigned long long *>(reinterpret_cast<char *>(a.cnt) + offsetof(CallCounters, allele)) + x, s);
         }
         if (jj == a.nb) {
-            const size_t stride = (size_t)a.nb + 1;
-            for (int s = 0; s < N_INT; ++s) a.sizes[s * stride + a.nb] = 0;
+            for (int s = 0; s < N_INT; ++s) sizes[s * stride + a.nb] = 0;
         }
     }
 }
@@ -393,6 +391,15 @@
     const size_t stride = (size_t)nb + 1;
     if (s < N_INT) totals[s] = offs[s * stride + nb] - offs[s * stride];
     (void)sizes;
+}
+
+__global__ void k_call_bounds(const uint64_t *__restrict__ offs, const uint32_t *__restrict__ vc, uint32_t nb, uint32_t piece, uint32_t n_rows,
+                              uint64_t *__restrict__ rows) {
+    const uint32_t i = blockIdx.x * blockDim.x + threadIdx.x;
+    if (i >= n_rows * (uint32_t)(N_INT + 1)) return;
+    const uint32_t b = i / (N_INT + 1), s = i % (N_INT + 1);
+    const uint64_t at = (uint64_t)b * piece < nb ? (uint64_t)b * piece : nb;
+    rows[i] = s < (uint32_t)N_INT ? offs[(size_t)s * ((size_t)nb + 1) + at] : (at ? (uint64_t)vc[at - 1] : 0);
 }
 
 
diff --git a/ploidyfrost_amd/csrc/pf_nibble.hpp b/ploidyfrost_amd/csrc/pf_nibble.hpp
--- a/ploidyfrost_amd/csrc/pf_nibble.hpp
+++ b/ploidyfrost_amd/csrc/pf_nibble.hpp
@@ -1,6 +1,10 @@
 #pragma once
 #include <stdint.h>
 #include <string.h>
+#if defined(__x86_64__) && !defined(__HIPCC__)
+#include <immintrin.h>
+#define PF_EXPAND_AVX2 1
+#endif
 
 namespace pf {
 
@@ -12,7 +16,16 @@
     return 16;
 }
 
-inline void nibble_expand(char *dst, const uint8_t *src, uint64_t n) {
+inline bool expand_simd_available() {
+#ifdef PF_EXPAND_AVX2
+    static const bool has = __builtin_cpu_supports("avx2");
+    return has;
+#else
+    return false;
+#endif
+}
+
+inline void nibble_expand_scalar(char *dst, const uint8_t *src, uint64_t n) {
     static const struct Lut {
         uint16_t two[256];
         Lut() {
@@ -34,4 +47,39 @@
     if (i < n) dst[i] = (char)(lut.two[src[i >> 1]] & 0xFF);
 }
 
+#ifdef PF_EXPAND_AVX2
+__attribute__((target("avx2"))) inline void nibble_expand_avx2(char *dst, const uint8_t *src, uint64_t n) {
+    const __m128i alpha128 = _mm_loadu_si128(reinterpret_cast<const __m128i *>(kNibbleAlphabet));
+    const __m256i alpha = _mm256_broadcastsi128_si256(alpha128);
+    const __m256i low4 = _mm256_set1_epi8(0x0F);
+    uint64_t i = 0;
+    for (; i + 64 <= n; i += 64) {
+        const __m256i in = _mm256_loadu_si256(reinterpret_cast<const __m256i *>(src + (i >> 1)));
+        const __m256i first = _mm256_shuffle_epi8(alpha, _mm256_and_si256(in, low4));
+        const __m256i second = _mm256_shuffle_epi8(alpha, _mm256_and_si256(_mm256_srli_epi16(in, 4), low4));
+        const __m256i a = _mm256_unpacklo_epi8(first, second), b = _mm256_unpackhi_epi8(first, second);
+        _mm256_storeu_si256(reinterpret_cast<__m256i *>(dst + i), _mm256_permute2x128_si256(a, b, 0x20));
+        _mm256_storeu_si256(reinterpret_cast<__m256i *>(dst + i + 32), _mm256_permute2x128_si256(a, b, 0x31));
+    }
+    if (i + 32 <= n) {
+        const __m128i in = _mm_loadu_si128(reinterpret_cast<const __m128i *>(src + (i >> 1)));
+        const __m128i m = _mm256_castsi256_si128(low4);
+        const __m128i first = _mm_shuffle_epi8(alpha128, _mm_and_si128(in, m));
+        const __m128i second = _mm_shuffle_epi8(alpha128, _mm_and_si128(_mm_srli_epi16(in, 4), m));
+        _mm_storeu_si128(reinterpret_cast<__m128i *>(dst + i), _mm_unpacklo_epi8(first, second));
+        _mm_storeu_si128(reinterpret_cast<__m128i *>(dst + i + 16), _mm_unpackhi_epi8(first, second));
+        i += 32;
+    }
+    nibble_expand_scalar(dst + i, src + (i >> 1), n - i);
 }
+#endif
+
+inline void nibble_expand(char *dst, const uint8_t *src, uint64_t n, bool simd = expand_simd_available()) {
+#ifdef PF_EXPAND_AVX2
+    if (simd && expand_simd_available()) return nibble_expand_avx2(dst, src, n);
+#endif
+    (void)simd;
+    nibble_expand_scalar(dst, src, n);
+}
+
+}
diff --git a/ploidyfrost_amd/hipapi.py b/ploidyfrost_amd/hipapi.py
--- a/ploidyfrost_amd/hipapi.py
+++ b/ploidyfrost_amd/hipapi.py
@@ -192,6 +192,8 @@
         "pf_call_align_lane": (i, [vp, i, u64, u64, u32, C.c_double, C.c_double, C.c_double, vp]),
         "pf_call_text_range_lane": (i, [vp, i, i, u64, u64, u64, vp]),
         "pf_call_text_sizes": (i, [vp, i, u64, u64, u64, vp]),
+        "pf_call_text_size_lane": (i, [vp, i, u64, u64, vp]),
+        "pf_call_text_write_lane": (i, [vp, i, i, u64, u64, vp]),
         "pf_bfs_live_deferred": (i, [vp, u64, vp]),
         "pf_bfs_live_count": (i, [vp, vp]),
         "pf_call_fetch": (i, [vp, i, i, vp, u64]),
@@ -261,7 +263,7 @@
                     "pf_gmm_upload", "pf_gmm_count", "pf_gmm_fit", "pf_kmc_decode", "pf_device_free", "pf_copy_to_host",
                     "pf_minimizer_table_slots", "pf_minimizer_crowding", "pf_minimizer_replay_inputs", "pf_bfs_candidates_split", "pf_unitig_cov_exact", "pf_unitig_cov_probe", "pf_unitig_cov_colored_probe",
                     "pf_call_set_state", "pf_call_set_format", "pf_superbubble_rows", "pf_superbubble_fetch", "pf_call_coverage", "pf_call_scan", "pf_call_sides", "pf_call_resolve", "pf_call_select", "pf_call_run", "pf_call_align",
-                    "pf_call_text", "pf_call_set_alignseq_packed", "pf_comm_unique_id", "pf_comm_init", "pf_gather", "pf_comm_destroy", "pf_call_reserve", "pf_call_reserve_lanes", "pf_timing_select", "pf_kernel_busy", "pf_call_reserve_text", "pf_selftest_scan", "pf_call_set_numeric_packed", "pf_call_fetch_text", "pf_find_reserve", "pf_call_set_colours", "pf_call_set_cutoffs", "pf_call_peek", "pf_call_text_range", "pf_call_align_lane", "pf_call_text_range_lane", "pf_call_text_sizes", "pf_call_fetch", "pf_call_fetch_slab", "pf_call_fetch_range", "pf_call_fetch_wait", "pf_format_doubles",
+                    "pf_call_text", "pf_call_set_alignseq_packed", "pf_comm_unique_id", "pf_comm_init", "pf_gather", "pf_comm_destroy", "pf_call_reserve", "pf_call_reserve_lanes", "pf_timing_select", "pf_kernel_busy", "pf_call_reserve_text", "pf_selftest_scan", "pf_call_set_numeric_packed", "pf_call_fetch_text", "pf_find_reserve", "pf_call_set_colours", "pf_call_set_cutoffs", "pf_call_peek", "pf_call_text_range", "pf_call_align_lane", "pf_call_text_range_lane", "pf_call_text_sizes", "pf_call_text_size_lane", "pf_call_text_write_lane", "pf_call_fetch","pf_call_fetch_slab", "pf_call_fetch_range", "pf_call_fetch_wait", "pf_format_doubles",
                     "pf_gmm_values", "pf_call_model_begin", "pf_call_model_take", "pf_call_model_finish", "pf_call_fetched_bytes",
                     "pf_call_model_filter", "pf_call_model_take_text",
                     "pf_call_model_filter_multi", "pf_call_model_color_count", "pf_call_model_color_select",
```
